# sloisel/MultiGridBarrierMPI.jl

Hardware: AMD Instinct MI355X
Metric: fem2d p-Laplace DoF/s per Newton step (higher is better)
Workload: dtype f64; 1 GPU; fem2d p-Laplace L=7 p=1 (n=57344 rows, N_L=49154 Newton unknowns), amgb main phase, tol=sqrt(eps); parallelism=single GPU

## Files before the change

### include/mgb_hip.h

```cpp
#ifndef MGB_HIP_H
#define MGB_HIP_H

#include <stdint.h>

#ifdef __cplusplus
extern "C" {
#endif

#define MGB_OK 0
#define MGB_E_ARG (-1)
#define MGB_E_HIP (-2)
#define MGB_E_NUMERIC (-3)
#define MGB_E_INTERNAL (-4)

typedef struct mgb_ctx_s* mgb_ctx;
typedef struct mgb_geo_s* mgb_geo;
typedef struct mgb_amg_s* mgb_amg;
typedef struct mgb_vec_s* mgb_vec;
typedef struct mgb_csr_s* mgb_csr;
typedef struct mgb_locator_s* mgb_locator;

const char* mgb_last_error(void);
int mgb_version(void);
int mgb_device_count(void);

int mgb_ctx_create(int device_id, mgb_ctx* out);
int mgb_ctx_destroy(mgb_ctx ctx);
int mgb_ctx_synchronize(mgb_ctx ctx);
typedef int (*mgb_allreduce_fn)(void* user, double* dev_ptr, long long count);
int mgb_ctx_set_comm(mgb_ctx ctx, int rank, int world, mgb_allreduce_fn fn, void* user);
int mgb_rccl_unique_id(char* out128);
int mgb_ctx_set_comm_rccl(mgb_ctx ctx, const char* unique_id128, int rank, int world);
int mgb_ctx_comm_stats(mgb_ctx ctx, long long* calls, double* bytes);
int mgb_shard_rows(int rank, int world, int n, int block, int* r0, int* r1);

int mgb_fem1d_native(int L, mgb_geo* out);
int mgb_fem2d_native(int L, const double* K, int nK_rows, mgb_geo* out);
int mgb_fem3d_native(int L, int k, mgb_geo* out);
int mgb_geo_create(int n, int dim, int L, int block, const double* x, const double* w, mgb_geo* out);
int mgb_geo_set_matrix(mgb_geo g, const char* name, int rows, int cols, const int32_t* rowptr,
                       const int32_t* colidx, const double* vals);
int mgb_geo_destroy(mgb_geo g);
int mgb_geo_dims(mgb_geo g, int* n, int* dim, int* L, int* block);
int mgb_geo_get_xw(mgb_geo g, double* x, double* w);
int mgb_geo_matrix_info(mgb_geo g, const char* name, int* rows, int* cols, int* nnz);
int mgb_geo_matrix_get(mgb_geo g, const char* name, int32_t* rowptr, int32_t* colidx, double* vals);

int mgb_vec_create(mgb_ctx ctx, int n, const double* host_or_null, mgb_vec* out);
int mgb_vec_free(mgb_vec v);
int mgb_vec_len(mgb_vec v, int* n);
int mgb_vec_upload(mgb_vec v, const double* host);
int mgb_vec_download(mgb_vec v, double* host);
int mgb_csr_create(mgb_ctx ctx, int rows, int cols, const int32_t* rowptr, const int32_t* colidx,
                   const double* vals, mgb_csr* out);
int mgb_csr_free(mgb_csr A);
int mgb_csr_dims(mgb_csr A, int* rows, int* cols, int* nnz);
int mgb_csr_get(mgb_csr A, int32_t* rowptr, int32_t* colidx, double* vals);
int mgb_csr_spgemm(mgb_csr A, mgb_csr B, mgb_csr* out);
int mgb_csr_transpose(mgb_csr A, mgb_csr* out);
int mgb_csr_add(mgb_csr A, double alpha, mgb_csr B, mgb_csr* out);
int mgb_csr_hcat(int count, const mgb_csr* mats, mgb_csr* out);
int mgb_csr_blockdiag(int count, const mgb_csr* mats, mgb_csr* out);
int mgb_diag(mgb_ctx ctx, mgb_vec z, int m, int n, mgb_csr* out);
int mgb_spmv(mgb_csr A, mgb_vec x, mgb_vec y);
int mgb_spmv_add(mgb_csr A, mgb_vec x, mgb_vec y0, mgb_vec y);
int mgb_dot(mgb_vec x, mgb_vec y, double* out);
int mgb_norm(mgb_vec x, double* out);
int mgb_sum(mgb_vec x, double* out);
int mgb_col_extract(mgb_vec M, int n, int K, int k, mgb_vec out);
int mgb_map_rows_barrier(int which, int K, int nterms, const int* kind, const int* nq, const int* idx_q, const int* idx_s,
                         const int* idx_s2, const double* p, const double* coef, const double* off, int n, mgb_vec Dz,
                         mgb_vec out);
int mgb_mul(mgb_vec x, mgb_vec y, mgb_vec out);
int mgb_axpy(mgb_vec x, double alpha, mgb_vec y, mgb_vec out);
int mgb_vec_allreduce_sum(mgb_vec x);
int mgb_all_isfinite(mgb_vec x, int* out);

int mgb_amg_create(mgb_ctx ctx, mgb_geo g, int S, const char* const* state_vars, int K, const char* const* D,
                   int nq, const int* idx_q, int idx_s, double p, mgb_amg* out);
int mgb_amg_create_cones(mgb_ctx ctx, mgb_geo g, int S, const char* const* state_vars, int K, const char* const* D,
                         int ncones, const int* nq, const int* idx_q, const int* idx_s, const int* idx_s2,
                         const double* p, mgb_amg* out);
int mgb_amg_create_terms(mgb_ctx ctx, mgb_geo g, int S, const char* const* state_vars, int K, const char* const* D,
                         int nterms, const int* kind, const int* nq, const int* idx_q, const int* idx_s, const int* idx_s2,
                         const double* p, const double* coef, const double* off, mgb_amg* out);
int mgb_amg_set_exponents(mgb_amg a, int term, const double* p_nodes);
int mgb_amg_set_term_mask(mgb_amg a, const unsigned char* mask);
int mgb_amg_destroy(mgb_amg a);
int mgb_amg_dims(mgb_amg a, int* n, int* S, int* K, int* L, int* nY);
int mgb_amg_local_rows(mgb_amg a, int* n_global, int* row0, int* n_local);
int mgb_amg_prepare(mgb_amg a, int level);
int mgb_amg_level_size(mgb_amg a, int level, int* N, int* nnz_lower);
int mgb_amg_f0_f32(mgb_amg a, int level, const float* s, float t, double* f0);
int mgb_amg_f1_f32(mgb_amg a, int level, const float* s, float t, float* g);
int mgb_amg_f2_f32(mgb_amg a, int level, const float* s, float t, float* lower_vals);
int mgb_amg_f1_template_f64(mgb_amg a, int level, const double* s, double t, double* g);
int mgb_amg_f2_template_f64(mgb_amg a, int level, const double* s, double t, double* lower_vals);
int mgb_amg_chol_info(mgb_amg a, int level, int* split_world, double* exchange_doubles, int* launches);
int mgb_amg_chol_schedule(mgb_amg a, int level, int cap, int* nlaunch, int* kind, int* workgroups, int* unknown_node,
                          int* unknown_col);
int mgb_amg_chol_tree(mgb_amg a, int level, int cap, int* nnodes, int* ns, int* nf, int* parent);
int mgb_amg_chol_values_local(mgb_amg a, int level, int* yes);
int mgb_amg_hessian_pattern(mgb_amg a, int level, int32_t* rowptr, int32_t* colidx);
int mgb_amg_set_c(mgb_amg a, const double* c);
int mgb_amg_set_z(mgb_amg a, const double* z);
int mgb_amg_get_z(mgb_amg a, double* z);
int mgb_amg_apply_D(mgb_amg a, int level, const double* s, double* Dz );
int mgb_amg_f0(mgb_amg a, int level, const double* s, double t, double* y, double* parts2);
int mgb_amg_f0_trial(mgb_amg a, int level, const double* s_ref, const double* s, double t, double* y);
int mgb_amg_f1(mgb_amg a, int level, const double* s, double t, double* g);
int mgb_amg_f2(mgb_amg a, int level, const double* s, double t, double* lower_vals);
int mgb_amg_solve_linear(mgb_amg a, int level, const double* lower_vals, const double* g, double* x);
int mgb_amg_solve_linear_gpu(mgb_amg a, int level, const double* lower_vals, const double* g, double* x);
int mgb_amg_set_solver(mgb_amg a, int solver);
int mgb_amg_set_schedule(mgb_amg a, int all_levels);
int mgb_amg_set_stop_rule(mgb_amg a, int upstream);
int mgb_amg_set_centering(mgb_amg a, int exact);
int mgb_amg_solve(mgb_amg a, double tol, double t0, double kappa, int maxit, int max_newton, int verbose);
int mgb_amg_set_early_stop(mgb_amg a, int col);
int mgb_amg_sol_info(mgb_amg a, int* nt, double* t_elapsed, double* time_factor, long long* counts4);
int mgb_amg_sol_get(mgb_amg a, long long* its , double* ts, double* c_dot_Dz);
int mgb_amg_sol_kernels(mgb_amg a, double* ms11, double* bytes11, long long* launches11);
int mgb_amg_time_kernels(mgb_amg a, int level, int reps, int nrot, double* ms8, double* bytes8);

int mgb_hessian_apply(mgb_amg a, int level, const double* s, const double* v, double* Hv, int matrix_free);
int mgb_smooth(mgb_amg a, int level, const double* s, const double* b, double* x, int degree, int sweeps, double lmax,
               int matrix_free, double* lmax_used);
int mgb_prolong(mgb_amg a, int level, const double* xc, double* xf);
int mgb_restrict(mgb_amg a, int level, const double* rf, double* rc);
int mgb_amg_prolongation(mgb_amg a, int level, int* rows, int* cols, int* nnz, int32_t* rowptr, int32_t* colidx, double* vals);
int mgb_amg_pcg_solve_linear(mgb_amg a, int level, const double* s, const double* g, double* x, int* iters, double* relres,
                             int* converged);
int mgb_amg_set_pcg(mgb_amg a, double rtol, int maxit, int degree, int power_its, double lo_frac, double hi_frac, int chunk,
                    int fallback, int assembled_top, int giveup);
int mgb_amg_sol_pcg(mgb_amg a, long long* counts4, double* time_s);
int mgb_amg_time_mg_kernels(mgb_amg a, int level, int reps, int nrot, double* ms6, double* bytes6, double* alg6);
int mgb_amg_mg_info(mgb_amg a, int top, int* coarsest);

int mgb_locator_create(mgb_ctx ctx, mgb_geo g, mgb_locator* out);
int mgb_locator_destroy(mgb_locator loc);
int mgb_interpolate(mgb_locator loc, int m, mgb_vec pts, int S, mgb_vec z, mgb_vec vals, mgb_vec grads_or_null,
                    int32_t* elem_host_or_null);
int mgb_geo_interpolate_host(mgb_geo g, int m, const double* pts, int S, const double* z, double* vals,
                             double* grads_or_null, int32_t* elem_or_null);


typedef struct mgb_plan_s* mgb_plan;
int mgb_plan_create(mgb_geo g, int S, const char* const* state_vars, int K, const char* const* D, int nq,
                    const int* idx_q, int idx_s, int level, mgb_plan* out);
int mgb_reduction_scratch_doubles(int n_local, int max_level_unknowns, long long* out);
int mgb_plan_destroy(mgb_plan p);
int mgb_plan_prolongation(mgb_plan fine, mgb_plan coarse, int* rows, int* cols, int* nnz, int32_t* rowptr, int32_t* colidx,
                          double* vals);
int mgb_plan_sizes(mgb_plan p, int* N, int* nnz_lower, int* nnz_T, int* nnz_B);
int mgb_plan_pattern(mgb_plan p, int32_t* rowptr, int32_t* colidx);
int mgb_plan_eval_host(mgb_plan p, const double* Y , double* lower_vals);
int mgb_plan_shard(mgb_plan p, int S, int K, int rank, int world, int block, mgb_plan* out, int* r0, int* r1);
int mgb_plan_apply_B_host(mgb_plan p, const double* s , double* Bs );
int mgb_plan_apply_BT_host(mgb_plan p, const double* v , double* g );
int mgb_plan_chol_bench(mgb_plan p, const double* Y, int dim, int reps, double* seconds_per_factor,
                        double* seconds_per_solve, double* flops, double* front_doubles, double* residual);
typedef struct mgb_hostchol_s* mgb_hostchol;
int mgb_plan_hostchol_create(mgb_plan p, int dim, mgb_hostchol* out);
int mgb_hostchol_destroy(mgb_hostchol c);
int mgb_hostchol_info(mgb_hostchol c, int* n, int* threads, double* flops);
int mgb_hostchol_factor_solve(mgb_hostchol c, const double* lower_vals, const double* g, double* x);
int mgb_hostchol_partition(mgb_hostchol c, int world, int* split_world, int cap, int* nnodes, int* owner);
int mgb_hostchol_factor_solve_dist(mgb_hostchol c, int rank, int world, mgb_allreduce_fn fn, void* user,
                                   const double* lower_vals, const double* g, double* x);
int mgb_plan_hostchol_create_ranked(mgb_plan p, int dim, int K, int world, int block, mgb_hostchol* out);
int mgb_hostchol_rank_aligned(mgb_hostchol c, int world, int* aligned, int* top_values);
int mgb_hostchol_factor_solve_dist_local(mgb_hostchol c, int rank, int world, mgb_allreduce_fn fn, void* user,
                                         const double* local_lower_vals, const double* g, double* x);
int mgb_plan_chol_tree(mgb_plan p, int dim, int cap, int* nnodes, int* ns, int* nf, int* parent);
int mgb_plan_chol_bwd_fused(mgb_plan p, int dim, int cut, int top_nf, int threads, int* info, int cap_wg, int* wg, int cap_bdry,
                            int* bdry, int* slots, int cap_nodes, int* bofs, int* first);
int mgb_chol_selftest(int nx, int ny, double* max_residual, double* flops, double* seconds);

#ifdef __cplusplus
}
#endif
#endif
```

### multigridbarriermpi.jl_amd/__init__.py

```python
from __future__ import annotations

import math
from dataclasses import dataclass, field
from typing import Callable, Dict, List, Optional, Sequence

import numpy as np
import scipy.sparse as sp

from . import _lib
from ._lib import MGBError, call, dptr, f64, i32, iptr

import ctypes as C

__all__ = [
    "fem1d", "fem2d", "fem3d", "fem1d_mpi", "fem2d_mpi", "fem3d_mpi", "fem1d_mpi_solve", "fem2d_mpi_solve",
    "fem3d_mpi_solve", "parabolic_solve", "ParabolicSOL", "native_to_mpi",
    "mpi_to_native", "amgb", "Geometry", "AMGBSOL", "HPCVector", "HPCMatrix", "HPCSparseMatrix",
    "backend_hip", "amgb_zeros", "amgb_all_isfinite", "amgb_diag", "amgb_blockdiag", "map_rows", "map_rows_gpu",
    "_raw_array", "_to_cpu_array", "MGBError", "device_count", "AMG", "amg", "hcat", "BarrierFn", "barrier_functions",
    "interpolate", "sample_grid",
]


def device_count() -> int:
# ... 533 lines not shown
    call("mgb_geo_create", n, dim, L, int(g_native.discretization.get("block", 1)), dptr(x), dptr(w), C.byref(h))

    def put(name, S):
        S = sp.csr_matrix(S, dtype=np.float64)
        S.sort_indices()
        S.sum_duplicates()
        rp, ci, va = i32(S.indptr), i32(S.indices), f64(S.data)
        call("mgb_geo_set_matrix", h, name.encode(), S.shape[0], S.shape[1], iptr(rp), iptr(ci), dptr(va))
        return HPCSparseMatrix(S, backend)

    try:
        operators = {k: put("op:" + k, g_native.operators[k]) for k in sorted(g_native.operators)}
        subspaces = {k: [put("sub:%s:%d" % (k, l), S) for l, S in enumerate(g_native.subspaces[k])]
                     for k in sorted(g_native.subspaces)}
        refine = [put("refine:%d" % l, S) for l, S in enumerate(g_native.refine)]
        coarsen = [put("coarsen:%d" % l, S) for l, S in enumerate(g_native.coarsen)]
    except Exception:
        call("mgb_geo_destroy", h)
        raise
    return Geometry(dict(g_native.discretization), HPCMatrix(x, backend), HPCVector(w, backend), subspaces,
                    operators, refine, coarsen, _geo=h)


def _mpi_from_native_handle(h, kind, ops, backend: Optional[HPCBackend], extra=None) -> Geometry:
    backend = backend or backend_hip()
    ref = _GeoRef(h)
    n, dim, L, block = C.c_int(), C.c_int(), C.c_int(), C.c_int()
    call("mgb_geo_dims", h, C.byref(n), C.byref(dim), C.byref(L), C.byref(block))
    x = np.empty((n.value, dim.value))
    w = np.empty(n.value)
    call("mgb_geo_get_xw", h, dptr(x), dptr(w))
    lazy = lambda name: _GeoMatrix(ref, name, backend)
    operators = {k: lazy("op:" + k) for k in sorted(ops)}
    subspaces = {k: [lazy("sub:%s:%d" % (k, l)) for l in range(L.value)] for k in ("dirichlet", "full")}
    refine = [lazy("refine:%d" % l) for l in range(L.value)]
    coarsen = [lazy("coarsen:%d" % l) for l in range(L.value)]
    disc = dict(kind=kind, L=L.value, dim=dim.value, block=block.value, **(extra or {}))
    return Geometry(disc, HPCMatrix(x, backend), HPCVector(w, backend), subspaces, operators, refine, coarsen, _geo=h,
                    _geo_ref=ref)


def _check_ti(Ti):
    if np.dtype(Ti) != np.dtype(np.int32):
        raise ValueError("only Ti=Int32 is supported by the HIP path")


def fem1d_mpi(L: int = 4, Ti=np.int32, backend=None) -> Geometry:
    _check_ti(Ti)
    h = C.c_void_p()
    call("mgb_fem1d_native", int(L), C.byref(h))
    return _mpi_from_native_handle(h, "fem1d", ("id", "dx"), backend)


def fem3d(L: int = 2, k: int = 3) -> Geometry:
    h = C.c_void_p()
    call("mgb_fem3d_native", int(L), int(k), C.byref(h))
    try:
        g = _native_from_handle(h, "fem3d", ("id", "dx", "dy", "dz"))
        g.discretization["k"] = int(k)
        return g
    finally:
        call("mgb_geo_destroy", h)


def fem3d_mpi(L: int = 2, k: int = 3, Ti=np.int32, backend=None) -> Geometry:
    _check_ti(Ti)
    h = C.c_void_p()
    call("mgb_fem3d_native", int(L), int(k), C.byref(h))
    return _mpi_from_native_handle(h, "fem3d", ("id", "dx", "dy", "dz"), backend, extra=dict(k=int(k)))


def fem2d_mpi(L: int = 2, K=None, Ti=np.int32, backend=None) -> Geometry:
    _check_ti(Ti)
    h = C.c_void_p()
    if K is None:
        call("mgb_fem2d_native", int(L), None, 0, C.byref(h))
    else:
        Kc = f64(K)
        call("mgb_fem2d_native", int(L), dptr(Kc), int(Kc.shape[0]), C.byref(h))
    return _mpi_from_native_handle(h, "fem2d", ("id", "dx", "dy"), backend)



DEFAULT_STATE = (("u", "dirichlet"), ("s", "full"))
DEFAULT_D = {1: (("u", "id"), ("u", "dx"), ("s", "id")),
             2: (("u", "id"), ("u", "dx"), ("u", "dy"), ("s", "id")),
             3: (("u", "id"), ("u", "dx"), ("u", "dy"), ("u", "dz"), ("s", "id"))}
class _RowFn:

    def __init__(self, row, grid):
        self._row, self.grid = row, grid

    def __call__(self, x):
        return self._row(x)


def _rows(fn, x) -> np.ndarray:
    if hasattr(fn, "grid"):
        return np.ascontiguousarray(fn.grid(x), dtype=np.float64)
    return np.vstack([np.asarray(fn(xi), dtype=np.float64) for xi in x])


def _const_rows(v):
    v = np.asarray(v, dtype=np.float64)
    return _RowFn(lambda x: v.copy(), lambda x: np.tile(v, (x.shape[0], 1)))


DEFAULT_F = {1: _const_rows([0.5, 0.0, 1.0]), 2: _const_rows([0.5, 0.0, 0.0, 1.0]), 3: _const_rows([0.5, 0.0, 0.0, 0.0, 1.0])}
DEFAULT_G = {1: _RowFn(lambda x: np.array([x[0], 2.0]), lambda x: np.column_stack([x[:, 0], np.full(x.shape[0], 2.0)])),
             2: _RowFn(lambda x: np.array([x[0] ** 2 + x[1] ** 2, 100.0]),
                       lambda x: np.column_stack([x[:, 0] ** 2 + x[:, 1] ** 2, np.full(x.shape[0], 100.0)])),
             3: _RowFn(lambda x: np.array([x[0] ** 2 + x[1] ** 2 + x[2] ** 2, 100.0]),
                       lambda x: np.column_stack([x[:, 0] ** 2 + x[:, 1] ** 2 + x[:, 2] ** 2, np.full(x.shape[0], 100.0)]))}


def _encode_terms(cones):
    kind, nq, iq, isl, is2, pp, coef, off = [], [], [], [], [], [], [], []
    for c in cones:
        if c[0] == "linear":
            _, cidx, ccoef, coff = c
            if not 1 <= len(cidx) <= 3 or len(ccoef) != len(cidx):
                raise ValueError("linear barrier term: 1..3 columns with one coefficient each")
            kind.append(1); nq.append(len(cidx)); iq += (list(cidx) + [0, 0, 0])[:3]; isl.append(0); is2.append(-1)
            pp.append(1.0); coef += (list(map(float, ccoef)) + [0.0, 0.0, 0.0])[:3]; off.append(float(coff))
        else:
            kind.append(0); nq.append(len(c[0]) - 1); iq += (list(c[0][:-1]) + [0, 0, 0])[:3]; isl.append(int(c[0][-1]))
            is2.append(int(c[2]) if len(c) > 2 else -1); pp.append(float(c[1])); coef += [0.0, 0.0, 0.0]; off.append(0.0)
    arr_i = lambda v: (C.c_int * len(v))(*v)
    arr_d = lambda v: (C.c_double * len(v))(*v)
    return (len(cones), arr_i(kind), arr_i(nq), arr_i(iq), arr_i(isl), arr_i(is2), arr_d(pp), arr_d(coef), arr_d(off))


class BarrierFn:

    def __init__(self, cones, K: int, which: int):
        self.cones, self.K, self.which = list(cones), int(K), int(which)

    def rows(self, Dz: "HPCMatrix"):
        n, K = Dz.shape
        if K != self.K:
            raise ValueError("BarrierFn: Dz has %d columns, the barrier was built for %d" % (K, self.K))
        width = (1, K, K * K)[self.which]
        out = HPCVector(n * width, Dz.backend)
        call("mgb_map_rows_barrier", self.which, K, *_encode_terms(self.cones), n, Dz._v.handle, out.handle)
        if self.which == 0:
            return out
        M_ = HPCMatrix.__new__(HPCMatrix)
        M_.shape, M_.backend, M_._v = (n, width), Dz.backend, out
        return M_

    def __call__(self, x_row, dz_row):
        r = self.rows(HPCMatrix(np.asarray(dz_row, dtype=np.float64).reshape(1, -1))).to_numpy()
        return float(r[0]) if self.which == 0 else r[0]


def barrier_functions(cones, K: int):
    return tuple(BarrierFn(cones, K, w) for w in (0, 1, 2))


class AMG:

    def __init__(self, geometry: Geometry, state_variables=DEFAULT_STATE, D=None, p: float = 1.0, idx=None,
                 cones=None, select=None):
        if geometry._geo is None:
            raise TypeError("AMG needs an MPI geometry (use native_to_mpi / fem*d_mpi)")
        dim = geometry.discretization["dim"]
        D = DEFAULT_D[dim] if D is None else D
        K = len(D)
        if cones is None:
            if idx is None:
                idx = list(range(K - dim - 1, K))
            cones = [(list(idx), float(p) if np.isscalar(p) else p)]
        self.geometry = geometry
        node_p, cones = {}, list(cones)
        for ti, c in enumerate(cones):
            if c[0] != "linear" and not np.isscalar(c[1]):
                pv = c[1]
                pn = (np.array([float(pv(xi)) for xi in geometry.x.to_numpy()]) if callable(pv) else f64(pv).reshape(-1))
                if pn.size != geometry.x.shape[0] or not np.all(pn >= 1.0):
                    raise ValueError("p(x) must give one value >= 1 per node")
                node_p[ti] = pn
                cones[ti] = (c[0], float(pn[0])) + tuple(c[2:])
        p = float(p) if np.isscalar(p) else (float(node_p[0][0]) if 0 in node_p else 1.0)
        self.p_nodes = node_p.get(0)
        self.state_variables, self.D, self.p, self.cones = tuple(state_variables), tuple(D), float(p), list(cones)
        power = [c for c in cones if c[0] != "linear"]
        self.idx = list(power[0][0]) if power else []
        backend = geometry.x.backend
        h = C.c_void_p()
        call("mgb_amg_create_terms", backend.handle, geometry._geo, len(state_variables), _lib.str_array(state_variables), K,
             _lib.str_array(D), *_encode_terms(cones), C.byref(h))
        self.handle = h
        n, S, K_, L, nY = (C.c_int() for _ in range(5))
        call("mgb_amg_dims", h, C.byref(n), C.byref(S), C.byref(K_), C.byref(L), C.byref(nY))
        self.S, self.K, self.L, self.nY = S.value, K_.value, L.value, nY.value
        ng, r0, nl = C.c_int(), C.c_int(), C.c_int()
        call("mgb_amg_local_rows", h, C.byref(ng), C.byref(r0), C.byref(nl))
        self.n, self.row0, self.n_local = ng.value, r0.value, nl.value
        for ti, pn in node_p.items():
            call("mgb_amg_set_exponents", h, int(ti), dptr(pn))
        if select is not None:
            mask = np.ascontiguousarray([[1 if b else 0 for b in select(xi)] for xi in geometry.x.to_numpy()], dtype=np.uint8)
            if mask.shape != (self.n, len(cones)):
                raise ValueError("select(x) must give one flag per barrier term")
            call("mgb_amg_set_term_mask", h, mask.ctypes.data_as(C.POINTER(C.c_ubyte)))

    def prepare(self, l=-1):
        call("mgb_amg_prepare", self.handle, int(l))

    def level_size(self, l):
        N, nz = C.c_int(), C.c_int()
        call("mgb_amg_level_size", self.handle, l, C.byref(N), C.byref(nz))
        return N.value, nz.value

    def chol_info(self, l=None):
        sw, ex, la = C.c_int(), C.c_double(), C.c_int()
        call("mgb_amg_chol_info", self.handle, self.L - 1 if l is None else int(l), C.byref(sw), C.byref(ex), C.byref(la))
        vl = C.c_int()
        call("mgb_amg_chol_values_local", self.handle, self.L - 1 if l is None else int(l), C.byref(vl))
        return dict(split_world=sw.value, exchange_doubles=ex.value, launches=la.value, values_local=bool(vl.value))

    CHOL_KINDS = ("Leaf", "Single", "SingleNarrow", "SingleDense", "SingleDenseNarrow", "Start", "Step", "Step2", "Panel2",
                  "Update2", "BwdRect", "Bwd256", "Bwd1024", "BwdFused")

    def chol_schedule(self, l=None):
        l = self.L - 1 if l is None else int(l)
        N = self.level_size(l)[0]
        nl = C.c_int()
        call("mgb_amg_chol_schedule", self.handle, l, 0, C.byref(nl), None, None, None, None)
        kind, wg = np.empty(nl.value, dtype=np.int32), np.empty(nl.value, dtype=np.int32)
        node, col = np.empty(N, dtype=np.int32), np.empty(N, dtype=np.int32)
        call("mgb_amg_chol_schedule", self.handle, l, nl.value, C.byref(nl), iptr(kind), iptr(wg), iptr(node), iptr(col))
        nn = C.c_int()
        call("mgb_amg_chol_tree", self.handle, l, 0, C.byref(nn), None, None, None)
        ns, nf, par = (np.empty(nn.value, dtype=np.int32) for _ in range(3))
        call("mgb_amg_chol_tree", self.handle, l, nn.value, C.byref(nn), iptr(ns), iptr(nf), iptr(par))
        height = np.zeros(nn.value, dtype=np.int32)
        for t in range(nn.value):
            if par[t] >= 0:
                height[par[t]] = max(height[par[t]], height[t] + 1)
        return dict(kinds=[self.CHOL_KINDS[k] for k in kind], workgroups=wg, unknown_node=node, unknown_col=col, ns=ns, nf=nf,
                    parent=par, height=height)

    def hessian_pattern(self, l):
        N, nz = self.level_size(l)
        rp = np.empty(N + 1, dtype=np.int32)
        ci = np.empty(nz, dtype=np.int32)
        call("mgb_amg_hessian_pattern", self.handle, l, iptr(rp), iptr(ci))
        return rp, ci

    def set_c(self, c):
        c = f64(c)
        assert c.shape == (self.n, self.K)
        call("mgb_amg_set_c", self.handle, dptr(c))

    def set_z(self, z):
        z = f64(np.asarray(z).reshape(-1))
        assert z.size == self.n * self.S
        call("mgb_amg_set_z", self.handle, dptr(z))

    def get_z(self):
        z = np.empty(self.n * self.S)
        call("mgb_amg_get_z", self.handle, dptr(z))
        return z

    def apply_D(self, l, s):
        s = f64(s)
        out = np.empty((self.n_local, self.K))
        call("mgb_amg_apply_D", self.handle, l, dptr(s), dptr(out))
        return out

    def apply_D_global(self, l, s):
        loc = self.apply_D(l, s)
        backend = self.geometry.x.backend
        if backend.world == 1:
            return loc
        full = np.zeros((self.n, self.K))
        full[self.row0:self.row0 + self.n_local] = loc
        v = HPCVector(full.reshape(-1), backend)
        call("mgb_vec_allreduce_sum", v.handle)
        return v.to_numpy().reshape(self.n, self.K)

    def f0(self, l, s, t, parts=False):
        s = f64(s)
        y = C.c_double()
        pr = np.empty(2)
        call("mgb_amg_f0", self.handle, l, dptr(s), float(t), C.byref(y), dptr(pr))
        return (y.value, pr) if parts else y.value

    def f0_trial(self, l, s_ref, s, t):
        s_ref, s = f64(s_ref), f64(s)
        y = C.c_double()
        call("mgb_amg_f0_trial", self.handle, l, dptr(s_ref), dptr(s), float(t), C.byref(y))
        return y.value

    def f1(self, l, s, t):
        s = f64(s)
        g = np.empty(self.level_size(l)[0])
        call("mgb_amg_f1", self.handle, l, dptr(s), float(t), dptr(g))
        return g

    def f2(self, l, s, t):
        s = f64(s)
        N, nz = self.level_size(l)
        vals = np.empty(nz)
        call("mgb_amg_f2", self.handle, l, dptr(s), float(t), dptr(vals))
# ... 531 lines not shown
```

### multigridbarriermpi.jl_amd/_lib.py

```python
from __future__ import annotations

import ctypes as C
import os

import numpy as np

_HERE = os.path.dirname(os.path.abspath(__file__))
LIB_PATH = os.path.join(_HERE, "lib", "libmgb_hip.so")

c_int_p = C.POINTER(C.c_int)
c_i32_p = C.POINTER(C.c_int32)
c_dbl_p = C.POINTER(C.c_double)
c_flt_p = C.POINTER(C.c_float)
c_ll_p = C.POINTER(C.c_longlong)
c_str_arr = C.POINTER(C.c_char_p)
H = C.c_void_p
ALLREDUCE_FN = C.CFUNCTYPE(C.c_int, C.c_void_p, C.c_void_p, C.c_longlong)


class MGBError(RuntimeError):
    def __init__(self, code, msg):
        super().__init__("mgb error %d: %s" % (code, msg))
        self.code = code


PROTOTYPES = {
    "mgb_ctx_create": [C.c_int, C.POINTER(H)],
    "mgb_ctx_destroy": [H],
    "mgb_ctx_synchronize": [H],
    "mgb_ctx_set_comm": [H, C.c_int, C.c_int, ALLREDUCE_FN, C.c_void_p],
    "mgb_rccl_unique_id": [C.c_char_p],
    "mgb_ctx_set_comm_rccl": [H, C.c_char_p, C.c_int, C.c_int],
    "mgb_ctx_comm_stats": [H, c_ll_p, c_dbl_p],
    "mgb_shard_rows": [C.c_int, C.c_int, C.c_int, C.c_int, c_int_p, c_int_p],
    "mgb_fem1d_native": [C.c_int, C.POINTER(H)],
    "mgb_fem2d_native": [C.c_int, c_dbl_p, C.c_int, C.POINTER(H)],
    "mgb_fem3d_native": [C.c_int, C.c_int, C.POINTER(H)],
    "mgb_geo_create": [C.c_int, C.c_int, C.c_int, C.c_int, c_dbl_p, c_dbl_p, C.POINTER(H)],
    "mgb_geo_set_matrix": [H, C.c_char_p, C.c_int, C.c_int, c_i32_p, c_i32_p, c_dbl_p],
    "mgb_geo_destroy": [H],
    "mgb_geo_dims": [H, c_int_p, c_int_p, c_int_p, c_int_p],
    "mgb_geo_get_xw": [H, c_dbl_p, c_dbl_p],
    "mgb_geo_matrix_info": [H, C.c_char_p, c_int_p, c_int_p, c_int_p],
    "mgb_geo_matrix_get": [H, C.c_char_p, c_i32_p, c_i32_p, c_dbl_p],
    "mgb_vec_create": [H, C.c_int, c_dbl_p, C.POINTER(H)],
    "mgb_vec_free": [H],
    "mgb_vec_len": [H, c_int_p],
    "mgb_vec_upload": [H, c_dbl_p],
    "mgb_vec_download": [H, c_dbl_p],
    "mgb_csr_create": [H, C.c_int, C.c_int, c_i32_p, c_i32_p, c_dbl_p, C.POINTER(H)],
    "mgb_csr_free": [H],
    "mgb_csr_dims": [H, c_int_p, c_int_p, c_int_p],
    "mgb_csr_get": [H, c_i32_p, c_i32_p, c_dbl_p],
    "mgb_csr_spgemm": [H, H, C.POINTER(H)],
    "mgb_csr_transpose": [H, C.POINTER(H)],
    "mgb_csr_add": [H, C.c_double, H, C.POINTER(H)],
    "mgb_csr_hcat": [C.c_int, C.POINTER(H), C.POINTER(H)],
    "mgb_csr_blockdiag": [C.c_int, C.POINTER(H), C.POINTER(H)],
    "mgb_diag": [H, H, C.c_int, C.c_int, C.POINTER(H)],
    "mgb_spmv": [H, H, H],
    "mgb_spmv_add": [H, H, H, H],
    "mgb_dot": [H, H, c_dbl_p],
    "mgb_norm": [H, c_dbl_p],
    "mgb_sum": [H, c_dbl_p],
    "mgb_col_extract": [H, C.c_int, C.c_int, C.c_int, H],
    "mgb_map_rows_barrier": [C.c_int, C.c_int, C.c_int, c_int_p, c_int_p, c_int_p, c_int_p, c_int_p, c_dbl_p, c_dbl_p, c_dbl_p,
                             C.c_int, H, H],
    "mgb_mul": [H, H, H],
    "mgb_axpy": [H, C.c_double, H, H],
    "mgb_vec_allreduce_sum": [H],
    "mgb_all_isfinite": [H, c_int_p],
    "mgb_amg_create": [H, H, C.c_int, c_str_arr, C.c_int, c_str_arr, C.c_int, c_int_p, C.c_int, C.c_double,
                       C.POINTER(H)],
    "mgb_amg_create_cones": [H, H, C.c_int, c_str_arr, C.c_int, c_str_arr, C.c_int, c_int_p, c_int_p, c_int_p, c_int_p,
                             c_dbl_p, C.POINTER(H)],
    "mgb_amg_create_terms": [H, H, C.c_int, c_str_arr, C.c_int, c_str_arr, C.c_int, c_int_p, c_int_p, c_int_p, c_int_p, c_int_p,
                             c_dbl_p, c_dbl_p, c_dbl_p, C.POINTER(H)],
    "mgb_amg_set_exponents": [H, C.c_int, c_dbl_p],
    "mgb_amg_set_term_mask": [H, C.POINTER(C.c_ubyte)],
    "mgb_amg_destroy": [H],
    "mgb_amg_dims": [H, c_int_p, c_int_p, c_int_p, c_int_p, c_int_p],
    "mgb_amg_local_rows": [H, c_int_p, c_int_p, c_int_p],
    "mgb_amg_prepare": [H, C.c_int],
    "mgb_amg_chol_info": [H, C.c_int, c_int_p, c_dbl_p, c_int_p],
    "mgb_amg_chol_schedule": [H, C.c_int, C.c_int, c_int_p, c_int_p, c_int_p, c_int_p, c_int_p],
    "mgb_amg_chol_tree": [H, C.c_int, C.c_int, c_int_p, c_int_p, c_int_p, c_int_p],
    "mgb_amg_chol_values_local": [H, C.c_int, c_int_p],
    "mgb_amg_level_size": [H, C.c_int, c_int_p, c_int_p],
    "mgb_amg_hessian_pattern": [H, C.c_int, c_i32_p, c_i32_p],
    "mgb_amg_set_c": [H, c_dbl_p],
    "mgb_amg_set_z": [H, c_dbl_p],
    "mgb_amg_get_z": [H, c_dbl_p],
    "mgb_amg_apply_D": [H, C.c_int, c_dbl_p, c_dbl_p],
    "mgb_amg_f0": [H, C.c_int, c_dbl_p, C.c_double, c_dbl_p, c_dbl_p],
    "mgb_amg_f0_trial": [H, C.c_int, c_dbl_p, c_dbl_p, C.c_double, c_dbl_p],
    "mgb_amg_f1": [H, C.c_int, c_dbl_p, C.c_double, c_dbl_p],
    "mgb_amg_f2": [H, C.c_int, c_dbl_p, C.c_double, c_dbl_p],
    "mgb_amg_set_early_stop": [H, C.c_int],
    "mgb_amg_f0_f32": [H, C.c_int, c_flt_p, C.c_float, c_dbl_p],
    "mgb_amg_f1_f32": [H, C.c_int, c_flt_p, C.c_float, c_flt_p],
    "mgb_amg_f2_f32": [H, C.c_int, c_flt_p, C.c_float, c_flt_p],
    "mgb_amg_f1_template_f64": [H, C.c_int, c_dbl_p, C.c_double, c_dbl_p],
    "mgb_amg_f2_template_f64": [H, C.c_int, c_dbl_p, C.c_double, c_dbl_p],
    "mgb_amg_solve_linear": [H, C.c_int, c_dbl_p, c_dbl_p, c_dbl_p],
    "mgb_amg_solve_linear_gpu": [H, C.c_int, c_dbl_p, c_dbl_p, c_dbl_p],
    "mgb_amg_set_solver": [H, C.c_int],
    "mgb_amg_set_schedule": [H, C.c_int],
    "mgb_amg_set_stop_rule": [H, C.c_int],
    "mgb_amg_set_centering": [H, C.c_int],
    "mgb_amg_set_pcg": [H, C.c_double, C.c_int, C.c_int, C.c_int, C.c_double, C.c_double, C.c_int, C.c_int, C.c_int, C.c_int],
    "mgb_amg_sol_pcg": [H, c_ll_p, c_dbl_p],
    "mgb_hessian_apply": [H, C.c_int, c_dbl_p, c_dbl_p, c_dbl_p, C.c_int],
    "mgb_smooth": [H, C.c_int, c_dbl_p, c_dbl_p, c_dbl_p, C.c_int, C.c_int, C.c_double, C.c_int, c_dbl_p],
    "mgb_prolong": [H, C.c_int, c_dbl_p, c_dbl_p],
    "mgb_restrict": [H, C.c_int, c_dbl_p, c_dbl_p],
    "mgb_amg_prolongation": [H, C.c_int, c_int_p, c_int_p, c_int_p, c_i32_p, c_i32_p, c_dbl_p],
    "mgb_amg_pcg_solve_linear": [H, C.c_int, c_dbl_p, c_dbl_p, c_dbl_p, c_int_p, c_dbl_p, c_int_p],
    "mgb_amg_mg_info": [H, C.c_int, c_int_p],
    "mgb_amg_time_mg_kernels": [H, C.c_int, C.c_int, C.c_int, c_dbl_p, c_dbl_p, c_dbl_p],
    "mgb_locator_create": [H, H, C.POINTER(H)],
    "mgb_locator_destroy": [H],
    "mgb_interpolate": [H, C.c_int, H, C.c_int, H, H, H, c_i32_p],
    "mgb_geo_interpolate_host": [H, C.c_int, c_dbl_p, C.c_int, c_dbl_p, c_dbl_p, c_dbl_p, c_i32_p],
    "mgb_plan_prolongation": [H, H, c_int_p, c_int_p, c_int_p, c_i32_p, c_i32_p, c_dbl_p],
    "mgb_amg_solve": [H, C.c_double, C.c_double, C.c_double, C.c_int, C.c_int, C.c_int],
    "mgb_amg_sol_info": [H, c_int_p, c_dbl_p, c_dbl_p, c_ll_p],
    "mgb_amg_sol_get": [H, c_ll_p, c_dbl_p, c_dbl_p],
    "mgb_amg_sol_kernels": [H, c_dbl_p, c_dbl_p, c_ll_p],
    "mgb_amg_time_kernels": [H, C.c_int, C.c_int, C.c_int, c_dbl_p, c_dbl_p],
    "mgb_plan_create": [H, C.c_int, c_str_arr, C.c_int, c_str_arr, C.c_int, c_int_p, C.c_int, C.c_int,
                        C.POINTER(H)],
    "mgb_reduction_scratch_doubles": [C.c_int, C.c_int, c_ll_p],
    "mgb_plan_destroy": [H],
    "mgb_plan_sizes": [H, c_int_p, c_int_p, c_int_p, c_int_p],
    "mgb_plan_pattern": [H, c_i32_p, c_i32_p],
    "mgb_plan_eval_host": [H, c_dbl_p, c_dbl_p],
    "mgb_plan_shard": [H, C.c_int, C.c_int, C.c_int, C.c_int, C.c_int, C.POINTER(C.c_void_p), c_int_p, c_int_p],
    "mgb_plan_apply_B_host": [H, c_dbl_p, c_dbl_p],
    "mgb_plan_apply_BT_host": [H, c_dbl_p, c_dbl_p],
    "mgb_plan_chol_bench": [H, c_dbl_p, C.c_int, C.c_int, c_dbl_p, c_dbl_p, c_dbl_p, c_dbl_p, c_dbl_p],
    "mgb_plan_hostchol_create": [H, C.c_int, C.POINTER(H)],
    "mgb_hostchol_destroy": [H],
    "mgb_hostchol_info": [H, c_int_p, c_int_p, c_dbl_p],
    "mgb_hostchol_factor_solve": [H, c_dbl_p, c_dbl_p, c_dbl_p],
    "mgb_hostchol_partition": [H, C.c_int, c_int_p, C.c_int, c_int_p, c_int_p],
    "mgb_hostchol_factor_solve_dist": [H, C.c_int, C.c_int, ALLREDUCE_FN, C.c_void_p, c_dbl_p, c_dbl_p, c_dbl_p],
    "mgb_plan_hostchol_create_ranked": [H, C.c_int, C.c_int, C.c_int, C.c_int, C.POINTER(H)],
    "mgb_hostchol_rank_aligned": [H, C.c_int, c_int_p, c_int_p],
    "mgb_hostchol_factor_solve_dist_local": [H, C.c_int, C.c_int, ALLREDUCE_FN, C.c_void_p, c_dbl_p, c_dbl_p, c_dbl_p],
    "mgb_plan_chol_tree": [H, C.c_int, C.c_int, c_int_p, c_int_p, c_int_p, c_int_p],
    "mgb_plan_chol_bwd_fused": [H, C.c_int, C.c_int, C.c_int, C.c_int, c_int_p, C.c_int, c_int_p, C.c_int, c_int_p, c_int_p, C.c_int,
                                c_int_p, c_int_p],
    "mgb_chol_selftest": [C.c_int, C.c_int, c_dbl_p, c_dbl_p, c_dbl_p],
}
_SPECIAL = {"mgb_last_error": ([], C.c_char_p), "mgb_version": ([], C.c_int), "mgb_device_count": ([], C.c_int)}

_lib = None


def load():
    global _lib
    if _lib is not None:
        return _lib
    if not os.path.exists(LIB_PATH):
        raise ImportError("libmgb_hip.so not built: run `python -c 'import __graft_entry__ as g; g.build()'` "
                          "or multigridbarriermpi.jl_amd/csrc/build.sh (expected at %s)" % LIB_PATH)
    lib = C.CDLL(LIB_PATH)
    for name, args in PROTOTYPES.items():
        fn = getattr(lib, name)
        fn.argtypes = args
        fn.restype = C.c_int
    for name, (args, res) in _SPECIAL.items():
        fn = getattr(lib, name)
        fn.argtypes = args
        fn.restype = res
    _lib = lib
    return lib


def call(name, *args):
    lib = load()
    rc = getattr(lib, name)(*args)
    if rc != 0:
        raise MGBError(rc, lib.mgb_last_error().decode("utf-8", "replace"))
    return rc


def dptr(a):
    return None if a is None else a.ctypes.data_as(c_dbl_p)


def iptr(a):
    return None if a is None else a.ctypes.data_as(c_i32_p)


def f64(a):
    return np.ascontiguousarray(a, dtype=np.float64)


def i32(a):
    return np.ascontiguousarray(a, dtype=np.int32)


def str_array(pairs):
    flat = []
    for a, b in pairs:
        flat += [str(a).encode(), str(b).encode()]
    return (C.c_char_p * len(flat))(*flat)
```

### multigridbarriermpi.jl_amd/csrc/amg.cpp

```cpp
#include "amg.hpp"


#include <chrono>
#include <cmath>
#include <thread>
#include <string>
#include <cstdlib>
#include <cstdio>

namespace mgb {

void hip_check(hipError_t e, const char* what) {
  if (e != hipSuccess) throw HipError(std::string("HIP error in ") + what + ": " + hipGetErrorString(e));
}

static inline void cpu_relax() {
#if defined(__x86_64__) || defined(__i386__)
  __builtin_ia32_pause();
#elif defined(__aarch64__)
  asm volatile("yield" ::: "memory");
#else
  std::this_thread::yield();
#endif
}
// ... 309 lines not shown
  const int K = P.K, nY = P.nY();
  auto gather = [&](int q, const ConeSpec& S, RowU& u) { gather_row(pl.B, K, q, S, u); };
  auto structural = [&](const RowU& u, int nc, int a, int b, int i, int j) { return structural_pair(u, nc, a, b, i, j); };
  const int nthr = std::max(1, std::min(MfChol::threads(), n / 2048));
  auto chunks = [&](auto&& fn) { node_chunks(n, nthr, fn); };
  auto phase = [](const char*) {};
  auto entry = [&](int r, int c) {
    const int* b0 = pl.Apat.colidx.data() + pl.Apat.rowptr[r];
    const int* e0 = pl.Apat.colidx.data() + pl.Apat.rowptr[r + 1];
    return (int)(std::lower_bound(b0, e0, c) - pl.Apat.colidx.data());
  };
  const int nnzA = pl.Apat.nnz();
  pl.T = Csr(nnzA, n * nY);
  struct Term {
    int e, col;
    double coef;
  };
  std::vector<std::vector<Term>> tterms(nthr);
  std::vector<std::vector<int>> tcnt(nthr);
  chunks([&](int q0, int q1, int tI) {
    std::vector<Term>& terms = tterms[tI];
    std::vector<int>& cnt = tcnt[tI];
    cnt.assign(nnzA, 0);
    terms.reserve((size_t)(q1 - q0) * 80);
    RowU u;
    for (int q = q0; q < q1; ++q) {
      int base = 0;
      for (int ci = 0; ci < P.ncones; ++ci) {
        const ConeSpec& S = P.cone[ci];
        const int nact = S.nact();
        gather(q, S, u);
        const int nc = (int)u.cols.size();
        for (int i = 0; i < nc; ++i)
          for (int j = 0; j <= i; ++j) {
            int e = -1;
            int slot = base;
            for (int a = 0; a < nact; ++a)
              for (int b = a; b < nact; ++b, ++slot) {
                if (!structural(u, nc, a, b, i, j)) continue;
                if (e < 0) e = entry(u.cols[i], u.cols[j]);
                double coef = u.val[(size_t)a * nc + i] * u.val[(size_t)b * nc + j];
                if (a != b) coef += u.val[(size_t)b * nc + i] * u.val[(size_t)a * nc + j];
                terms.push_back({e, q * nY + slot, coef});
                cnt[e]++;
              }
          }
        base += S.nY();
      }
    }
  });
  phase("list terms");
  {
    long long tot = 0;
    for (int e = 0; e < nnzA; ++e) {
      pl.T.rowptr[e] = (int)tot;
      for (int t = 0; t < nthr; ++t) {
        const int c0 = tcnt[t][e];
        tcnt[t][e] = (int)tot;
        tot += c0;
      }
      if (tot > 2000000000LL) throw ArgError("amg: Hessian plan exceeds Int32 indexing");
    }
    pl.T.rowptr[nnzA] = (int)tot;
    pl.T.colidx.resize((size_t)tot);
    pl.T.vals.resize((size_t)tot);
  }
  chunks([&](int, int, int tI) {
    std::vector<int>& pos = tcnt[tI];
    for (const Term& tm : tterms[tI]) {
      const int pp = pos[tm.e]++;
      pl.T.colidx[pp] = tm.col;
      pl.T.vals[pp] = tm.coef;
    }
    std::vector<Term>().swap(tterms[tI]);
  });
  phase("fill terms");
}


Amg::Amg(Ctx& ctx, const GeometryHost& g, const AmgSpec& spec, const BarrierParams& P)
    : ctx_(ctx), n_(g.n), S_((int)spec.state_variables.size()), P_(P), spec_(spec) {
  hip_check(hipSetDevice(ctx_.device), "hipSetDevice");
  if (const char* e = std::getenv("MGB_FUSED_TRIAL_ROWS")) fused_trial_rows_ = std::atoi(e);
  if (P.K != (int)spec.D.size()) throw ArgError("amg: barrier K != number of D rows");
  if (P.ncones < 1 || P.ncones > kMaxCones) throw ArgError("amg: barrier supports 1 to 3 terms");
  if (P.K > 8) throw ArgError("amg: the barrier kernels support at most 8 rows of D");
  for (int ci = 0; ci < P.ncones; ++ci) {
    const ConeSpec& S = P.cone[ci];
    if (S.kind != 0 && S.kind != 1) throw ArgError("amg: unknown barrier term kind");
    if (S.nq < 1 || S.nq > 3) throw ArgError("amg: barrier supports 1..3 gradient components");
    for (int a = 0; a < S.nact(); ++a)
      if (S.col(a) < 0 || S.col(a) >= P.K) throw ArgError("amg: barrier index out of range");
  }
  if ((int)g.w.size() != n_ || (int)g.x.size() != n_ * g.dim) throw ArgError("amg: geometry x/w size mismatch");
  ng_ = g.n;
  Csr Dstack = build_dstack(g, spec);
  w_min_ = *std::min_element(g.w.begin(), g.w.end());
  if (ctx_.world > 1) {
    int r1 = 0;
    shard_rows(ctx_.rank, ctx_.world, ng_, g.block, &r0_, &r1);
    n_ = r1 - r0_;
    Dstack_.upload(shard_dstack(Dstack, ng_, S_, P.K, r0_, r1));
  } else {
    Dstack_.upload(Dstack);
  }
  w_.upload(g.w.data() + r0_, n_);
  const int K = P.K, nY = P.nY();
  c_.alloc((size_t)n_ * K);
  z_.alloc((size_t)n_ * S_);
  z_save_.alloc((size_t)n_ * S_);
  Dz0_.alloc((size_t)n_ * K);
  Dz0_save_.alloc((size_t)n_ * K);
  Dz_.alloc((size_t)n_ * K);
  DzA_.alloc((size_t)n_ * K);
  DzB_.alloc((size_t)n_ * K);
  DzC_.alloc((size_t)n_ * K);
  v_.alloc((size_t)n_ * K);
  Y_.alloc((size_t)n_ * nY);
  phi_cur_.alloc((size_t)n_ * P.ncones);
  phi_trial_.alloc((size_t)n_ * P.ncones);
  phi_trial2_.alloc((size_t)n_ * P.ncones);
  phi_trial3_.alloc((size_t)n_ * P.ncones);
  h_flag_.alloc(4);
  scal_.alloc(12);
  h_scal_.alloc(12);
  seq_dev_.alloc(1);
  hip_check(hipMemset(seq_dev_.p, 0, sizeof(unsigned long long)), "memset seq");
  h_seq_.alloc(1);
  h_seq_.p[0] = 0;
  hip_check(hipMemsetAsync(c_.p, 0, c_.n * sizeof(double), ctx_.stream), "memset");
  hip_check(hipMemsetAsync(z_.p, 0, z_.n * sizeof(double), ctx_.stream), "memset");
  hip_check(hipStreamSynchronize(ctx_.stream), "sync");
  geo_ = g;
  dstack_host_ = std::move(Dstack);
  for (int l = 0; l < g.L; ++l) {
    levels_.emplace_back(new Level);
    int N = 0;
    for (auto& sv : spec.state_variables) {
      if (sv.second == "fixed") continue;
      auto it = g.subspaces.find(sv.second);
      if (it == g.subspaces.end() || l >= (int)it->second.size())
        throw ArgError("amg: unknown subspace '" + sv.second + "'");
      N += it->second[l].cols;
    }
    levels_[l]->plan.N = N;
  }
  int maxN = 0;
  for (auto& lv : levels_) maxN = std::max(maxN, lv->plan.N);
  partials_.alloc(reduction_scratch_doubles(n_, maxN));
  hip_check(hipMemset(partials_.p, 0, partials_.n * sizeof(double)), "memset scratch");
}

size_t reduction_scratch_doubles(int n_local, int max_level_unknowns) {
  return (size_t)6 * std::max(f0_blocks(n_local), f0_blocks(max_level_unknowns)) + 8 + kReductionHeader;
}

int Amg::level_index(const Level& lv) const {
  for (size_t l = 0; l < levels_.size(); ++l)
    if (levels_[l].get() == &lv) return (int)l;
  throw InternalError("amg: level not found");
}

Amg::Level& Amg::level(int l) {
  Level& lv = *levels_.at(l);
  if (lv.built) return lv;
  if (lv.chol_analysis.joinable()) lv.chol_analysis.join();
  lv.chol_analyzed = false;
  lv.chol_analysis_error = nullptr;
  hip_check(hipSetDevice(ctx_.device), "hipSetDevice");
  static const bool use_elasm = !(std::getenv("MGB_ASSEMBLE") && std::string(std::getenv("MGB_ASSEMBLE")) == "plan");
  const bool try_elasm = use_elasm && ctx_.world == 1 && geo_.block > 1 && n_ % geo_.block == 0;
  lv.plan = build_level_plan(geo_, spec_, dstack_host_, l, P_, !try_elasm);
  lv.T_built = !try_elasm;
  if (ctx_.world > 1) {
    std::vector<unsigned long long> mask = dof_rank_masks(lv.plan.B, ng_, P_.K, ctx_.world, geo_.block);
    lv.plan = shard_level_plan(lv.plan, ng_, S_, P_.K, P_.nY(), r0_, r0_ + n_);
    lv.plan.rank_mask = std::move(mask);
  }
  if (!pcg_ && lv.plan.N > 0) {
    lv.chol_analysis = std::thread([this, &lv] {
      try {
        analyze_chol(lv);
      } catch (...) {
        lv.chol_analysis_error = std::current_exception();
      }
    });
  }
  const double t_up = now_s();
  lv.R.upload(lv.plan.R);
  lv.B.upload(lv.plan.B);
  if (n_ > fused_trial_rows_ && geo_.block > 1 && n_ % geo_.block == 0) lv.Bel.build(lv.plan.B, geo_.block * P_.K);
  lv.BT.upload(lv.plan.BT);
  if (lv.T_built) lv.T.upload(lv.plan.T);
  if (try_elasm && lv.plan.N > 0) {
    mg_of(lv);
    if (mg_ensure_elop(lv)) lv.elasm.build(lv.mg->elop, lv.plan.Apat, P_);
    if (!lv.elasm.view.valid()) ensure_T(lv);
  }
  const int N = lv.plan.N, nnzA = lv.plan.Apat.nnz();
  lv.s.alloc(N);
  lv.s_trial.alloc(N);
  lv.s_trial2.alloc(N);
  lv.s_trial3.alloc(N);
  lv.g_trial.alloc(N);
  lv.g.alloc(N);
  lv.nstep.alloc(N);
  lv.avals.alloc(nnzA);
  lv.h_avals.alloc(nnzA);
  lv.h_g.alloc(N);
  lv.h_n.alloc(N);
  lv.h_s.alloc(N);
  if (std::getenv("MGB_VERBOSE_SETUP")) std::fprintf(stderr, "[mgb setup] level upload + buffers       %.3f s\n", now_s() - t_up);
  lv.built = true;
  return lv;
}

void Amg::analyze_chol(Level& lv) {
  static const bool aligned_on = !(std::getenv("MGB_RANK_ALIGNED") && std::atoi(std::getenv("MGB_RANK_ALIGNED")) == 0);
  const bool ranked = aligned_on && ctx_.world > 1 && (int)lv.plan.rank_mask.size() == lv.plan.N;
  lv.chol.analyze(lv.plan.Apat, lv.plan.coords.data(), geo_.dim, 64, ranked ? lv.plan.rank_mask.data() : nullptr, ctx_.world);
  lv.chol_analyzed = true;
}

void Amg::ensure_chol(Level& lv) {
  if (lv.chol_built) return;
  hip_check(hipSetDevice(ctx_.device), "hipSetDevice");
  static const bool vt = std::getenv("MGB_VERBOSE_SETUP") != nullptr;
  double t0 = now_s();
  if (lv.chol_analysis.joinable()) lv.chol_analysis.join();
  if (lv.chol_analysis_error) {
    std::exception_ptr e = lv.chol_analysis_error;
    lv.chol_analysis_error = nullptr;
    std::rethrow_exception(e);
  }
  if (!lv.chol_analyzed) analyze_chol(lv);
  if (vt) std::fprintf(stderr, "[mgb setup] chol analyze (rest)         %.3f s\n", now_s() - t0);
  t0 = now_s();
  lv.gchol.build(lv.chol, &ctx_);
  if (vt) std::fprintf(stderr, "[mgb setup] gpuchol build + upload      %.3f s\n", now_s() - t0);
  lv.chol_built = true;
}

static double csr_bytes(const DevCsr& A, bool y0);

void Amg::ensure_T(Level& lv) {
  if (!lv.T_built) {
    build_plan_terms(lv.plan, ng_, P_);
    lv.T_built = true;
  }
  if (lv.T.view.rows == 0 && lv.plan.T.rows > 0) {
    hip_check(hipSetDevice(ctx_.device), "hipSetDevice");
    lv.T.upload(lv.plan.T);
  }
}

double Amg::assemble_bytes(Level& lv) {
  if (!lv.elasm.view.valid()) return csr_bytes(lv.T.view, false);
  const DevElOp& E = lv.mg->elop.view;
  return (double)lv.B.view.nnz * 8 + (double)n_ * P_.nY() * 8 + E.nel * 4.0 + 2.0 * E.nel * lv.elasm.view.npm * 8 +
         (double)E.nel * lv.elasm.view.npm * 4 + lv.plan.Apat.nnz() * 12.0;
}

void Amg::assemble_values(Level& lv) {
  if (lv.elasm.view.valid()) {
    launch_elop_assemble(ctx_.stream, lv.mg->elop.view, lv.elasm.view, P_, Y_.p, lv.elasm.elmat.p, lv.avals.p);
    return;
  }
  ensure_T(lv);
  launch_spmv(ctx_.stream, lv.T.view, Y_.p, nullptr, lv.avals.p);
}

const LevelPlan& Amg::plan(int l) { return level(l).plan; }

void Amg::chol_info(int l, int* split_world, double* exchange_doubles, int* launches) {
  Level& lv = level(l);
  ensure_chol(lv);
  if (split_world) *split_world = lv.gchol.split() ? ctx_.world : 1;
  if (exchange_doubles) *exchange_doubles = lv.gchol.split() ? lv.gchol.exchange_doubles() : 0.0;
  if (launches) *launches = lv.gchol.launches_per_solve();
}

void Amg::chol_schedule(int l, int cap, int* nlaunch, int* kind, int* workgroups, int* unknown_node, int* unknown_col) {
  Level& lv = level(l);
  ensure_chol(lv);
  lv.gchol.schedule_info(cap, nlaunch, kind, workgroups);
  GpuChol::unknown_columns(lv.chol, unknown_node, unknown_col);
}

void Amg::chol_tree(int l, int cap, int* nnodes, int* ns, int* nf, int* parent) {
  Level& lv = level(l);
  ensure_chol(lv);
  std::vector<int> a, b, c;
  lv.chol.tree(a, b, c);
  if (nnodes) *nnodes = (int)a.size();
  const size_t m = std::min<size_t>(std::max(cap, 0), a.size());
  if (ns) std::copy(a.begin(), a.begin() + m, ns);
  if (nf) std::copy(b.begin(), b.begin() + m, nf);
  if (parent) std::copy(c.begin(), c.begin() + m, parent);
}

void Amg::prepare(int l) {
  const int L = (int)levels_.size();
  for (int J = (l >= 0 ? l : (schedule_all_ ? 0 : L - 1)); J <= (l >= 0 ? l : L - 1); ++J) {
    Level& lv = level(J);
    if (lv.plan.N == 0) continue;
    if (pcg_) mg_prepare(J);
    else ensure_chol(lv);
// ... 55 lines not shown
  hip_check(hipStreamSynchronize(ctx_.stream), "sync");
  if (ctx_.world <= 1) {
    z_.download(z_host, (size_t)n_ * S_);
    return;
  }
  DevBuf<double> zg;
  zg.alloc((size_t)ng_ * S_);
  hip_check(hipMemsetAsync(zg.p, 0, zg.n * sizeof(double), ctx_.stream), "memset zg");
  for (int sv = 0; sv < S_; ++sv)
    hip_check(hipMemcpyAsync(zg.p + (size_t)sv * ng_ + r0_, z_.p + (size_t)sv * n_, (size_t)n_ * sizeof(double),
                             hipMemcpyDeviceToDevice, ctx_.stream), "D2D z");
  ctx_.allreduce_sum(zg.p, (long long)zg.n);
  hip_check(hipStreamSynchronize(ctx_.stream), "sync");
  zg.download(z_host, zg.n);
}

static double csr_bytes(const DevCsr& A, bool y0) {
  return (double)A.nnz * 12.0 + (A.rows + 1) * 4.0 + A.cols * 8.0 + A.rows * 8.0 * (y0 ? 2 : 1);
}

KernelTimer::~KernelTimer() {
  for (auto* v : {&free_, &pending_})
    for (auto& p : *v) {
      (void)hipEventDestroy(p.a);
      (void)hipEventDestroy(p.b);
    }
}

void KernelTimer::begin(hipStream_t st, int cls, double bytes) {
  if (!on_ || !sampling_) return;
  if (free_.empty()) {
    Pair p{};
    hip_check(hipEventCreate(&p.a), "hipEventCreate");
    hip_check(hipEventCreate(&p.b), "hipEventCreate");
    free_.push_back(p);
  }
  cur_ = free_.back();
  free_.pop_back();
  cur_.cls = cls;
  cur_.bytes = bytes;
  hip_check(hipEventRecord(cur_.a, st), "hipEventRecord");
  open_ = true;
}

void KernelTimer::end(hipStream_t st) {
  if (!on_ || !open_) return;
  hip_check(hipEventRecord(cur_.b, st), "hipEventRecord");
  pending_.push_back(cur_);
  open_ = false;
}

void KernelTimer::collect(SolveStats& st) {
  for (auto& p : pending_) {
    float ms = 0;
    if (hipEventElapsedTime(&ms, p.a, p.b) == hipSuccess) {
      st.kern_ms[p.cls] += ms;
      st.kern_bytes[p.cls] += p.bytes;
      st.kern_launches[p.cls]++;
    }
    free_.push_back(p);
  }
  pending_.clear();
}

void Amg::sync_collect(const char* what) {
  hip_check(hipStreamSynchronize(ctx_.stream), what);
  if (live_) timer_.collect(*live_);
}

void Amg::resync_signals() {
  hip_check(hipStreamSynchronize(ctx_.stream), "resync signals");
  seq_expected_ = *h_seq_.p;
}

HostSignal Amg::next_signal() {
  HostSignal sig;
  if (ctx_.world != 1) return sig;
  sig.seq_dev = seq_dev_.p;
  sig.seq_host = h_seq_.p;
  ++seq_expected_;
  return sig;
}

void Amg::wait_signal(const char* what) {
  if (ctx_.world != 1 || host_solve_ || (live_ && timer_.sampling())) {
    sync_collect(what);
    return;
  }
  const volatile unsigned long long* q = h_seq_.p;
  const double t0 = now_s();
  for (unsigned long spins = 0; __atomic_load_n(q, __ATOMIC_ACQUIRE) < seq_expected_; ++spins) {
    cpu_relax();
    if ((spins & 0xfffff) == 0xfffff && now_s() - t0 > 10.0) {
      hip_check(hipStreamSynchronize(ctx_.stream), what);
      if (__atomic_load_n(q, __ATOMIC_ACQUIRE) < seq_expected_) throw InternalError(std::string("mgb: completion signal lost in ") + what);
    }
  }
}

void Amg::refresh_dz0() { launch_spmv(ctx_.stream, Dstack_.view, z_.p, nullptr, Dz0_.p); }

void Amg::dev_apply(Level& lv, const double* s_dev, double* dz) {
  timer_.begin(ctx_.stream, KC_APPLY, csr_bytes(lv.B.view, true));
  if (lv.Bel.view.valid()) launch_spmv_el(ctx_.stream, lv.B.view, lv.Bel.view, s_dev, Dz0_.p, dz);
  else launch_spmv(ctx_.stream, lv.B.view, s_dev, Dz0_.p, dz);
  timer_.end(ctx_.stream);
}

double Amg::trial_bytes(const Level& lv, bool with_ref) const {
  return csr_bytes(lv.B.view, true) + (double)n_ * (P_.K + 1 + P_.ncones * (with_ref ? 2 : 1)) * 8;
}

void Amg::enqueue_f0(Level& lv, const double* s_dev, double alpha, const double* nstep, double* s_out, double* dz,
                     const double* phi_ref, double* phi_out, double* out2, HostSignal sig) {
  if (n_ <= fused_trial_rows_) {
    timer_.begin(ctx_.stream, KC_F0, trial_bytes(lv, phi_ref != nullptr));
    launch_trial_f0(ctx_.stream, lv.B.view, n_, P_, s_dev, alpha, nstep, s_out, Dz0_.p, dz, w_.p, c_.p, phi_ref,
                    kFracToBoundary, phi_out, partials_.p, out2, host_scal(out2), sig);
    timer_.end(ctx_.stream);
    return;
  }
  const double* x = s_dev;
  if (nstep) {
    launch_waxpby(ctx_.stream, lv.plan.N, s_dev, alpha, nstep, s_out);
    x = s_out;
  }
  dev_apply(lv, x, dz);
  timer_.begin(ctx_.stream, KC_F0, (double)n_ * (2 * P_.K + 2 + (phi_ref ? 1 : 0)) * 8);
  launch_barrier_f0(ctx_.stream, n_, P_, dz, w_.p, c_.p, phi_ref, kFracToBoundary, phi_out, partials_.p, out2, host_scal(out2), sig);
  timer_.end(ctx_.stream);
}

double Amg::dev_f0(Level& lv, const double* s_dev, double t, double* parts, const double* phi_ref, double* phi_out,
                   double* dz, double alpha, const double* nstep, double* s_out) {
  enqueue_f0(lv, s_dev, alpha, nstep, s_out, dz, phi_ref, phi_out, scal_.p, next_signal());
  if (ctx_.world > 1) {
    ctx_.allreduce_sum(scal_.p, 2);
    hip_check(hipMemcpyAsync(h_scal_.p, scal_.p, 2 * sizeof(double), hipMemcpyDeviceToHost, ctx_.stream), "D2H scal");
  }
  wait_signal("sync f0");
  if (parts) {
    parts[0] = h_scal_.p[0];
    parts[1] = h_scal_.p[1];
  }
  return h_scal_.p[0] + t * h_scal_.p[1];
}

bool Amg::values_stay_local(Level& lv) {
  if (ctx_.world <= 1 || host_solve_) return false;
  ensure_chol(lv);
  return lv.gchol.values_local();
}

void Amg::enqueue_f2_assemble(Level& lv, const double* dz, SolveStats& st) {
  timer_.begin(ctx_.stream, KC_F2, (double)n_ * (P_.K + 1 + P_.nY()) * 8);
  launch_barrier_f2(ctx_.stream, n_, P_, dz, w_.p, Y_.p);
  timer_.end(ctx_.stream);
  if (pcg_) {
    mg_values(level_index(lv));
    st.n_f2++;
    return;
  }
  timer_.begin(ctx_.stream, KC_ASSEMBLE, assemble_bytes(lv));
  assemble_values(lv);
  timer_.end(ctx_.stream);
  if (!values_stay_local(lv)) ctx_.allreduce_sum(lv.avals.p, lv.plan.Apat.nnz());
  st.n_f2++;
}

double Amg::dev_f1(Level& lv, const double* dz, double t, double* g_out, SolveStats* st, const double** pre) {
  timer_.begin(ctx_.stream, KC_F1, (double)n_ * (3 * P_.K + 1) * 8);
  launch_barrier_f1(ctx_.stream, n_, P_, dz, w_.p, c_.p, t, v_.p);
  timer_.end(ctx_.stream);
  timer_.begin(ctx_.stream, KC_RESTRICT, csr_bytes(lv.BT.view, false));
  launch_spmv(ctx_.stream, lv.BT.view, v_.p, nullptr, g_out);
  timer_.end(ctx_.stream);
  if (owner_local(lv)) {
    const int ntop = lv.gchol.ntop_unknowns();
    if (gtop_.n < (size_t)ntop + 1) gtop_.alloc((size_t)ntop + 1);
    launch_gather_top(ctx_.stream, ntop, lv.gchol.top_unknowns(), g_out, gtop_.p);
    launch_dot_owned(ctx_.stream, lv.plan.N, g_out, g_out, lv.gchol.unknown_kind(), 0, partials_.p, gtop_.p + ntop);
    ctx_.allreduce_sum(gtop_.p, ntop + 1);
    launch_scatter_top_norm(ctx_.stream, ntop, lv.gchol.top_unknowns(), gtop_.p, g_out, scal_.p + 2);
  } else {
    ctx_.allreduce_sum(g_out, lv.plan.N);
    launch_dot(ctx_.stream, lv.plan.N, g_out, g_out, partials_.p, scal_.p + 2, host_scal(scal_.p + 2), nullptr, nullptr, next_signal());
  }
  if (ctx_.world > 1)
    hip_check(hipMemcpyAsync(h_scal_.p + 2, scal_.p + 2, sizeof(double), hipMemcpyDeviceToHost, ctx_.stream), "D2H gg");
  if (host_solve_)
    hip_check(hipMemcpyAsync(lv.h_g.p, g_out, (size_t)lv.plan.N * sizeof(double), hipMemcpyDeviceToHost, ctx_.stream),
              "D2H g");
  if (pre && st && !host_solve_) {
    if (!pcg_) ensure_chol(lv);
    if (ctx_.world > 1) {
      if (!ev_f1_) hip_check(hipEventCreateWithFlags(&ev_f1_, hipEventDisableTiming), "event");
      hip_check(hipEventRecord(ev_f1_, ctx_.stream), "record f1");
    }
    enqueue_f2_assemble(lv, dz, *st);
    *pre = dz;
    if (ctx_.world == 1) wait_signal("sync f1");
    else hip_check(hipEventSynchronize(ev_f1_), "sync f1 event");
  } else {
    wait_signal("sync f1");
  }
  return std::sqrt(h_scal_.p[2]);
}

static const double kBeta = 0.5, kArmijo = 0.1, kMinStep = 1e-8;

void Amg::enqueue_trial(Level& lv, Trial& T, double step, int slot, HostSignal sig) {
  double* out = scal_.p + 4 + 2 * slot;
  enqueue_f0(lv, lv.s.p, -step, lv.nstep.p, T.s, T.dz, phi_cur_.p, T.phi, out, sig);
  T.step = step;
}

static const double kSpecSteps[3] = {1.0, kBeta, kBeta * kBeta};

void Amg::enqueue_spec_trials(Level& lv, Trial* spec, HostSignal sig) {
  const int ns = spec_count();
  if (ns == 3) {
    TrialSet T;
    T.na = 3;
    for (int q = 0; q < 3; ++q) {
      T.alpha[q] = -kSpecSteps[q];
      T.s_out[q] = spec[q].s;
      T.dz[q] = spec[q].dz;
      T.phi_out[q] = spec[q].phi;
      spec[q].step = kSpecSteps[q];
    }
    T.out_dev = scal_.p + 4;
    T.out_host = host_scal(scal_.p + 4);
    timer_.begin(ctx_.stream, KC_F0, trial_bytes(lv, true) + 2.0 * n_ * (P_.K + P_.ncones) * 8);
    launch_trial_set(ctx_.stream, lv.B.view, n_, P_, lv.s.p, lv.nstep.p, T, Dz0_.p, w_.p, c_.p, phi_cur_.p, kFracToBoundary,
                     partials_.p, sig);
    timer_.end(ctx_.stream);
  } else {
    enqueue_trial(lv, spec[0], kSpecSteps[0], 0);
    enqueue_trial(lv, spec[1], kSpecSteps[1], 1, sig);
  }
}

void Amg::launch_step_graph(Level& lv, Trial* spec) {
  const void* key[15] = {lv.avals.p, lv.g.p, lv.nstep.p, lv.s.p, spec[0].s, spec[0].phi, spec[0].dz, spec[1].s, spec[1].phi,
                         spec[1].dz, spec[2].s,  spec[2].phi, spec[2].dz, phi_cur_.p, Dz0_.p};
  for (const auto& g : lv.step_graphs)
    if (std::equal(key, key + 15, g.key)) {
      hip_check(hipGraphLaunch(g.exec, ctx_.stream), "hipGraphLaunch");
      ++seq_expected_;
      for (int q = 0; q < spec_count(); ++q) spec[q].step = kSpecSteps[q];
      return;
    }
  hipGraph_t graph = nullptr;
  hip_check(hipStreamBeginCapture(ctx_.stream, hipStreamCaptureModeThreadLocal), "hipStreamBeginCapture");
  try {
    lv.gchol.enqueue_chain(ctx_.stream, lv.avals.p, lv.g.p, lv.nstep.p);
    launch_dot(ctx_.stream, lv.plan.N, lv.g.p, lv.nstep.p, partials_.p, scal_.p + 3, host_scal(scal_.p + 3), lv.gchol.fail_flag(),
               h_flag_.p);
    HostSignal sig;
    sig.seq_dev = seq_dev_.p;
    sig.seq_host = h_seq_.p;
    enqueue_spec_trials(lv, spec, sig);
  } catch (...) {
    (void)hipStreamEndCapture(ctx_.stream, &graph);
    if (graph) (void)hipGraphDestroy(graph);
    throw;
  }
  hip_check(hipStreamEndCapture(ctx_.stream, &graph), "hipStreamEndCapture");
  Level::StepGraph sg{};
  std::copy(key, key + 15, sg.key);
  hipError_t e = hipGraphInstantiate(&sg.exec, graph, nullptr, nullptr, 0);
  (void)hipGraphDestroy(graph);
  hip_check(e, "hipGraphInstantiate");
  lv.step_graphs.push_back(sg);
  hip_check(hipGraphLaunch(sg.exec, ctx_.stream), "hipGraphLaunch");
  ++seq_expected_;
}

bool Amg::dev_f2_solve(Level& lv, const double* dz, double t, SolveStats& st, double* inc, Trial* spec,
                       const double* pre_assembled) {
  const int N = lv.plan.N, nnzA = lv.plan.Apat.nnz();
  if (!pcg_) ensure_chol(lv);
  if (pre_assembled != dz) enqueue_f2_assemble(lv, dz, st);
  st.n_factor++;
  timer_.sample((st.n_factor % 8) == 1);
  if (pcg_) {
    const int top = level_index(lv);
    bool ok = pcg_run(lv, top, lv.g.p, lv.nstep.p, &st, nullptr, nullptr);
    if (!ok && pcg_last_code_ == 2.0) {
      for (int l = mg_coarsest(top); l <= top; ++l)
        if (level(l).mg) level(l).mg->ev_warm = false;
      mg_values(top);
      ok = pcg_run(lv, top, lv.g.p, lv.nstep.p, &st, nullptr, nullptr);
    }
    h_flag_.p[0] = 0;
    if (ok) pcg_bad_streak_ = 0;
    if (!ok) {
      if (!pcg_opt.fallback) return false;
      st.pcg_fallbacks++;
      if (pcg_opt.giveup > 0 && ++pcg_bad_streak_ >= pcg_opt.giveup) {
        pcg_ = false;
        st.pcg_gaveup_at = st.n_factor;
      }
      ensure_chol(lv);
      assemble_values(lv);
      lv.gchol.factor_solve(ctx_.stream, lv.avals.p, lv.g.p, lv.nstep.p, nullptr, false);
      lv.flag_armed = false;
      hip_check(hipMemcpyAsync(h_flag_.p, lv.gchol.fail_flag(), sizeof(int), hipMemcpyDeviceToHost, ctx_.stream), "D2H flag");
    }
    launch_dot(ctx_.stream, N, lv.g.p, lv.nstep.p, partials_.p, scal_.p + 3, host_scal(scal_.p + 3), nullptr, nullptr,
               spec ? HostSignal() : next_signal());
    if (spec) {
      enqueue_spec_trials(lv, spec, next_signal());
      st.n_f0 += spec_count();
    }
    wait_signal("sync pcg solve");
    if (!ok) hip_check(hipStreamSynchronize(ctx_.stream), "sync fallback flag");
    if (spec)
      for (int q = 0; q < spec_count(); ++q) {
        spec[q].y = h_scal_.p[4 + 2 * q] + t * h_scal_.p[5 + 2 * q];
        spec[q].valid = true;
      }
    *inc = h_scal_.p[3];
    return h_flag_.p[0] == 0;
  }
  if (!host_solve_) {
    const bool use_graph = GpuChol::knobs().graph;
    KernelTimer* tm = (live_ && timer_.sampling()) ? &timer_ : nullptr;
    const bool flag_rides = ctx_.world == 1;
    hipEvent_t e0 = nullptr, e1 = nullptr;
    const bool time_chain = live_ && timer_.enabled() && (st.n_factor % 8) == 5;
    if (flag_rides && spec && !tm && !time_chain && use_graph && lv.flag_armed) {
      launch_step_graph(lv, spec);
      st.n_f0 += spec_count();
    } else {
      if (time_chain) {
        hip_check(hipEventCreate(&e0), "event");
        hip_check(hipEventCreate(&e1), "event");
        hip_check(hipEventRecord(e0, ctx_.stream), "record");
      }
      const bool olocal = owner_local(lv);
      lv.gchol.factor_solve(ctx_.stream, lv.avals.p, lv.g.p, lv.nstep.p, tm, flag_rides && lv.flag_armed, false, olocal);
      if (time_chain) hip_check(hipEventRecord(e1, ctx_.stream), "record");
      if (olocal) {
        launch_dot_owned(ctx_.stream, N, lv.g.p, lv.nstep.p, lv.gchol.unknown_kind(), ctx_.rank == 0, partials_.p, scal_.p + 3);
        launch_flag_to_double(ctx_.stream, lv.gchol.fail_flag(), scal_.p + 10);
      } else if (flag_rides) {
        launch_dot(ctx_.stream, N, lv.g.p, lv.nstep.p, partials_.p, scal_.p + 3, host_scal(scal_.p + 3), lv.gchol.fail_flag(),
                   h_flag_.p, spec ? HostSignal() : next_signal());
        lv.flag_armed = true;
      } else {
        launch_dot(ctx_.stream, N, lv.g.p, lv.nstep.p, partials_.p, scal_.p + 3);
        hip_check(hipMemcpyAsync(h_flag_.p, lv.gchol.fail_flag(), sizeof(int), hipMemcpyDeviceToHost, ctx_.stream), "D2H flag");
      }
      if (spec) {
        enqueue_spec_trials(lv, spec, next_signal());
        if (!olocal) ctx_.allreduce_sum(scal_.p + 4, 2 * spec_count());
        st.n_f0 += spec_count();
      }
      if (olocal) {
        if (!spec) hip_check(hipMemsetAsync(scal_.p + 4, 0, 6 * sizeof(double), ctx_.stream), "zero trial slots");
        ctx_.allreduce_sum(scal_.p + 3, 8);
        hip_check(hipMemcpyAsync(h_scal_.p + 3, scal_.p + 3, 8 * sizeof(double), hipMemcpyDeviceToHost, ctx_.stream), "D2H inc + trials + flag");
      } else if (ctx_.world > 1)
        hip_check(hipMemcpyAsync(h_scal_.p + 3, scal_.p + 3, (spec ? 1 + 2 * spec_count() : 1) * sizeof(double),
                                 hipMemcpyDeviceToHost, ctx_.stream), "D2H inc + trials");
    }
    wait_signal("sync solve");
    if (owner_local(lv)) h_flag_.p[0] = h_scal_.p[10] != 0.0 ? 1 : 0;
    if (spec)
      for (int q = 0; q < spec_count(); ++q) {
        spec[q].y = h_scal_.p[4 + 2 * q] + t * h_scal_.p[5 + 2 * q];
        spec[q].valid = true;
      }
    if (e0) {
      float ms = 0;
      hip_check(hipEventSynchronize(e1), "sync chain event");
      if (hipEventElapsedTime(&ms, e0, e1) == hipSuccess) st.time_factor += 8.0 * ms * 1e-3;
      (void)hipEventDestroy(e0);
      (void)hipEventDestroy(e1);
    }
    *inc = h_scal_.p[3];
    if (h_flag_.p[0] != 0 && h_flag_.p[0] != 1)
      throw InternalError("gpuchol: pivot flag holds " + std::to_string(h_flag_.p[0]) + " (only 0 / 1 are ever written)");
    return h_flag_.p[0] == 0;
  }
  hip_check(hipMemcpyAsync(lv.h_avals.p, lv.avals.p, (size_t)nnzA * sizeof(double), hipMemcpyDeviceToHost, ctx_.stream),
            "D2H avals");
  sync_collect("sync f2");
  const double t0 = now_s();
  bool ok = lv.chol.factor(lv.h_avals.p);
  double acc = 0;
  if (ok) {
    std::copy(lv.h_g.p, lv.h_g.p + N, lv.h_n.p);
    lv.chol.solve(lv.h_n.p);
    for (int i = 0; i < N; ++i) acc += lv.h_g.p[i] * lv.h_n.p[i];
    hip_check(hipMemcpyAsync(lv.nstep.p, lv.h_n.p, (size_t)N * sizeof(double), hipMemcpyHostToDevice, ctx_.stream),
              "H2D n");
  }
  st.time_factor += now_s() - t0;
  *inc = acc;
  return ok;
}


Amg::NewtonResult Amg::newton(int l, double t, bool finest, bool final, double lam_tol, int maxit, SolveStats& st, int verbose) {
  Level& lv = level(l);
  const int N = lv.plan.N;
  NewtonResult res;
  if (N == 0) {
    res.converged = true;
    return res;
  }
  hip_check(hipMemsetAsync(lv.s.p, 0, (size_t)N * sizeof(double), ctx_.stream), "memset s");
  double y = dev_f0(lv, lv.s.p, t, nullptr, nullptr, phi_cur_.p, Dz_.p);
  st.n_f0++;
  if (!std::isfinite(y)) {
    std::vector<double> hdz((size_t)n_ * P_.K);
    Dz_.download(hdz.data(), hdz.size());
    int bad = 0, worst = -1;
    double minphi = INFINITY;
    for (int q = 0; q < n_; ++q) {
      const double* d = hdz.data() + (size_t)q * P_.K;
      double phi = INFINITY, sv = INFINITY;
      for (int ci = 0; ci < P_.ncones; ++ci) {
        const ConeSpec& S = P_.cone[ci];
        if (S.kind == 1) {
          double ph = S.off;
          for (int i = 0; i < S.nq; ++i) ph += S.coef[i] * d[S.iq[i]];
          phi = std::min(phi, ph);
          continue;
        }
        double qq = 0;
        for (int i = 0; i < S.nq; ++i) qq += d[S.iq[i]] * d[S.iq[i]];
        const double sc = d[S.is] + (S.is2 >= 0 ? d[S.is2] : 0.0);
        phi = std::min(phi, (sc > 0 ? std::pow(sc, S.a) : -1.0) - qq);
        sv = std::min(sv, sc);
      }
      if (!(phi > 0) || !(sv > 0)) bad++;
      if (!(phi >= minphi)) {
        minphi = phi;
        worst = q;
      }
    }
    char buf[256];
    snprintf(buf, sizeof buf, "newton: infeasible start (level %d, t=%g, %d of %d rows outside the cone, min phi=%g at row %d, y=%g)",
             l, t, bad, n_, minphi, worst, y);
    throw NumericError(buf);
  }
  double gnorm = dev_f1(lv, Dz_.p, t, lv.g.p);
  st.n_f1++;
  double ymin = y, gmin = gnorm, incmin = INFINITY;
  const double theta = finest ? 0.1 : 0.5;
  Trial T[3];
  T[0].s = lv.s_trial.p;
  T[0].phi = phi_trial_.p;
  T[1].s = lv.s_trial2.p;
  T[1].phi = phi_trial2_.p;
  T[2].s = lv.s_trial3.p;
  T[2].phi = phi_trial3_.p;
  T[0].dz = DzA_.p;
  T[1].dz = DzB_.p;
  T[2].dz = DzC_.p;
  auto eval = [&](int pos, double step) {
    if (!(T[pos].valid && T[pos].step == step))
      for (int q = 0; q < 3; ++q)
        if (q != pos && T[q].valid && T[q].step == step) {
          std::swap(T[pos], T[q]);
          break;
        }
    Trial& X = T[pos];
    if (X.valid && X.step == step) return X.y;
    X.y = dev_f0(lv, lv.s.p, t, nullptr, phi_cur_.p, X.phi, X.dz, -step, lv.nstep.p, X.s);
    st.n_f0++;
    X.step = step;
    X.valid = true;
    return X.y;
  };
  const double* pre = nullptr;
  const bool speculate = !host_solve_;
  while (res.k < maxit && !res.converged) {
    res.k++;
    double inc = 0;
    T[0].valid = T[1].valid = T[2].valid = false;
    const double* have = pre;
    pre = nullptr;
    if (!dev_f2_solve(lv, Dz_.p, t, st, &inc, speculate ? T : nullptr, have)) {
      if (verbose > 1) fprintf(stderr, "    [mgb] level %d k=%d: Hessian not numerically SPD (pivot flag %d)\n", l, res.k, h_flag_.p[0]);
      break;
    }
    if (!std::isfinite(inc)) {
      if (verbose > 1) fprintf(stderr, "    [mgb] level %d k=%d: non-finite Newton decrement\n", l, res.k);
      break;
    }
    if (inc <= 0) {
      res.converged = true;
      break;
    }
    double step = 1.0, ynext = y, gnext = gnorm;
    bool accepted = false;
    while (step >= kMinStep) {
      double yA = eval(0, step);
      if (std::isfinite(yA) && yA <= y - kArmijo * step * inc) {
        while (step * kBeta >= kMinStep) {
          const double yB = eval(1, step * kBeta);
          if (!(std::isfinite(yB) && yB < yA)) break;
          std::swap(T[0], T[1]);
          yA = yB;
          step *= kBeta;
// ... 445 lines not shown
```

### multigridbarriermpi.jl_amd/csrc/amg.hpp

```cpp
#pragma once
#include <memory>
#include <string>
#include <utility>
#include <thread>
#include <exception>
#include <vector>

#include "geometry.hpp"
#include "gpuchol.hpp"
#include "kernels.hpp"
#include "mfchol.hpp"
#include "mg.hpp"

namespace mgb {

void hip_check(hipError_t e, const char* what);

typedef int (*AllreduceFn)(void* user, double* dev_ptr, long long count);

struct Ctx {
  int device = 0;
  hipStream_t stream = nullptr;
  int rank = 0, world = 1;
  AllreduceFn allreduce = nullptr;
// ... 149 lines not shown
  bool schedule_all = false;
  bool time_kernels = true;
  bool upstream_stop = false;
  bool exact_centering = true;
  double tol = 1.4901161193847656e-08;
  double t0 = 0.1;
  double kappa = 10.0;
  int maxit = 10000;
  int max_newton = 48;
  int verbose = 0;
};

struct SolveStats {
  int L = 0;
  std::vector<long long> its;
  std::vector<double> ts, c_dot_Dz;
  double t_elapsed = 0, t_setup = 0;
  double time_factor = 0, time_device = 0;
  long long n_factor = 0, n_f0 = 0, n_f1 = 0, n_f2 = 0;
  long long pcg_solves = 0, pcg_iters = 0, pcg_fallbacks = 0;
  long long pcg_gaveup_at = -1;
  double time_pcg = 0;
  double kern_ms[KC_COUNT] = {};
  double kern_bytes[KC_COUNT] = {};
  long long kern_launches[KC_COUNT] = {};
};

class KernelTimer {
 public:
  ~KernelTimer();
  void enable(bool on) { on_ = on; sampling_ = true; }
  void sample(bool now) { sampling_ = now; }
  bool sampling() const { return on_ && sampling_; }
  bool enabled() const { return on_; }
  void begin(hipStream_t st, int cls, double bytes);
  void end(hipStream_t st);
  void collect(SolveStats& st);
 private:
  struct Pair {
    hipEvent_t a, b;
    int cls;
    double bytes;
  };
  std::vector<Pair> free_, pending_;
  Pair cur_{};
  bool on_ = false, open_ = false, sampling_ = true;
};

class Amg {
 public:
  Amg(Ctx& ctx, const GeometryHost& g, const AmgSpec& spec, const BarrierParams& P);
  int n() const { return n_; }
  int n_global() const { return ng_; }
  int row0() const { return r0_; }
  int S() const { return S_; }
  int K() const { return P_.K; }
  int L() const { return (int)levels_.size(); }
  int level_size(int l) const { return levels_[l]->plan.N; }
  const LevelPlan& plan(int l);
  void prepare(int l);
  const BarrierParams& params() const { return P_; }
  void chol_info(int l, int* split_world, double* exchange_doubles, int* launches);
  void chol_schedule(int l, int cap, int* nlaunch, int* kind, int* workgroups, int* unknown_node, int* unknown_col);
  void chol_tree(int l, int cap, int* nnodes, int* ns, int* nf, int* parent);
  bool chol_values_local(int l) { return values_stay_local(level(l)); }
  void set_early_stop(int col) { early_stop_col_ = col; }
  void set_exponents(int term, const double* p_nodes_global);
  void set_term_mask(const unsigned char* mask_global);
  void set_pcg(bool on) { pcg_ = on; }

  void set_c(const double* c_host);
  void set_z(const double* z_host);
  void get_z(double* z_host);

  double f0(int l, const double* s_host, double t, double* parts);
  double f0_trial(int l, const double* s_ref_host, const double* s_host, double t);
  void f1(int l, const double* s_host, double t, double* g_host);
  void f2(int l, const double* s_host, double t, double* avals_host);
  double f0_f32(int l, const float* s_host, float t);
  void f1_f32(int l, const float* s_host, float t, float* g_host);
  void f2_f32(int l, const float* s_host, float t, float* avals_host);
  void f1_tpl64(int l, const double* s_host, double t, double* g_host);
  void f2_tpl64(int l, const double* s_host, double t, double* avals_host);
  void apply_D(int l, const double* s_host, double* Dz_host);
  bool solve_host(int l, const double* avals, const double* g, double* nstep);
  bool solve_device(int l, const double* avals, const double* g, double* nstep);

  void solve(const SolveOptions& opt, SolveStats& st);

  struct KernelTimes {
    double apply_ms, f2_ms, assemble_ms, f1_ms, restrict_ms, f0_ms, trial_ms, apply_csr_ms, apply_el;
    double apply_bytes, f2_bytes, assemble_bytes, f1_bytes, restrict_bytes, f0_bytes, trial_bytes;
  };
  KernelTimes time_kernels(int l, int reps, int nrot = 1);

 private:
  struct Level {
    bool built = false, chol_built = false, T_built = false;
    DevElAsmOwned elasm;
    bool flag_armed = false;
    struct StepGraph {
      const void* key[15];
      hipGraphExec_t exec;
    };
    std::vector<StepGraph> step_graphs;
    std::thread chol_analysis;
    std::exception_ptr chol_analysis_error;
    bool chol_analyzed = false;
    ~Level() {
      if (chol_analysis.joinable()) chol_analysis.join();
      for (auto& g : step_graphs) (void)hipGraphExecDestroy(g.exec);
    }
    LevelPlan plan;
    DevCsrOwned R, B, BT, T;
    DevElCsrOwned Bel;
    DevBuf<float> B32, BT32, T32, s32, g32, avals32;
    bool f32_built = false;
    MfChol chol;
    GpuChol gchol;
    DevBuf<double> s, s_trial, s_trial2, s_trial3, g, g_trial, nstep, avals;
    PinnedBuf<double> h_avals, h_g, h_n, h_s;
    struct Mg {
      bool elop_tried = false, assembled = false, transfer = false, vectors = false;
      DevElOpOwned elop;
      DevBuf<double> elbuf;
      DevCsrOwned A;
      DevBuf<int> amap, diagpos, lo_rowptr, lo_colidx;
      DevCsrOwned P, PT;
      DevBuf<double> dinv, x, b, r, d0, d1, ev0, ev1, coef, Ainv;
      bool ev_warm = false;
    };
    std::unique_ptr<Mg> mg;
  };
  struct NewtonResult {
    int k = 0;
    bool converged = false;
  };
  Level& level(int l);
  int level_index(const Level& lv) const;
  void ensure_chol(Level& lv);
  void analyze_chol(Level& lv);
  void ensure_T(Level& lv);
  void assemble_values(Level& lv);
  double assemble_bytes(Level& lv);
  void refresh_dz0();
  void dev_apply(Level& lv, const double* s_dev, double* dz);
  double dev_f0(Level& lv, const double* s_dev, double t, double* parts, const double* phi_ref, double* phi_out,
                double* dz, double alpha = 0.0, const double* nstep = nullptr, double* s_out = nullptr);
  double trial_bytes(const Level& lv, bool with_ref) const;
  int fused_trial_rows_ = 64 * 2048;
  void enqueue_f0(Level& lv, const double* s_dev, double alpha, const double* nstep, double* s_out, double* dz,
                  const double* phi_ref, double* phi_out, double* out2, HostSignal sig = HostSignal());
  double dev_f1(Level& lv, const double* dz, double t, double* g_out, SolveStats* st = nullptr, const double** pre = nullptr);
  void enqueue_f2_assemble(Level& lv, const double* dz, SolveStats& st);
  bool values_stay_local(Level& lv);
  bool owner_local(Level& lv) { return in_solve_ && values_stay_local(lv); }
  bool in_solve_ = false;
  DevBuf<double> gtop_;
  struct EventHolder {
    hipEvent_t e = nullptr;
    ~EventHolder() {
      if (e) (void)hipEventDestroy(e);
    }
  } ev_f1_holder_;
  hipEvent_t& ev_f1_ = ev_f1_holder_.e;
  struct Trial {
    double* s = nullptr;
    double* phi = nullptr;
    double* dz = nullptr;
    double step = 0, y = 0;
    bool valid = false;
  };
  bool dev_f2_solve(Level& lv, const double* dz, double t, SolveStats& st, double* inc, Trial* spec = nullptr,
                    const double* pre_assembled = nullptr);
  void enqueue_trial(Level& lv, Trial& T, double step, int slot, HostSignal sig = HostSignal());
  int spec_count() const { return n_ <= fused_trial_rows_ ? 3 : 2; }
  void enqueue_spec_trials(Level& lv, Trial* spec, HostSignal sig);
  void launch_step_graph(Level& lv, Trial* spec);
  NewtonResult newton(int l, double t, bool finest, bool final, double lam_tol, int maxit, SolveStats& st, int verbose);
  bool amgb_step(double t, bool final, double lam_tol, int max_newton, std::vector<long long>& its, SolveStats& st, int verbose);
  double c_dot_dz();

 public:
  PcgOptions pcg_opt;
  void hessian_apply(int l, const double* s_host, const double* v_host, double* out_host, bool matrix_free);
  double mg_smooth(int l, const double* s_host, const double* b_host, double* x_host, int degree, int sweeps, double lmax,
                   bool matrix_free);
  void mg_prolong(int l, const double* xc_host, double* xf_host);
  void mg_restrict(int l, const double* rf_host, double* rc_host);
  int mg_coarsest(int top);
  bool pcg_solve_linear(int l, const double* s_host, const double* g_host, double* x_host, int* iters, double* relres);
  const Csr& prolongation_host(int l);
  struct MgKernelTimes {
    double ms[6], bytes[6], alg[6];
  };
  MgKernelTimes time_mg_kernels(int l, int reps, int nrot);

 private:
  Level::Mg& mg_of(Level& lv);
  void mg_ensure_vectors(Level& lv);
  bool mg_ensure_elop(Level& lv);
  void mg_ensure_assembled(Level& lv);
  void mg_ensure_transfer(int l);
  void mg_prepare(int top);
  bool mg_top_matrix_free(int top);
  void mg_values(int top);
  void mg_level_values(Level& lv, bool mf);
  void mg_estimate(Level& lv, bool mf, double lmax_given);
  void mg_apply(Level& lv, bool mf, const MgEpi& epi);
  void mg_smooth_pre(Level& lv, bool mf, const double* b, double* x, double* r, int degree, const double* done);
  void mg_smooth_post(Level& lv, bool mf, const double* b, double* x, double* r, int degree, const double* done);
  void mg_vcycle(int top, int l, const double* b, double* x, const double* done);
  bool pcg_run(Level& lv, int top, const double* g, double* x, SolveStats* st, int* iters, double* relres);
  void eval_Y_at(Level& lv, const double* s_host);
  std::vector<Csr> P_host_;
  DevBuf<double> mg_scal_, mg_scratch_, pcg_r_, pcg_z_, pcg_p_, pcg_Ap_;
  PinnedBuf<double> h_pcg_;
  DevBuf<int> mg_fail_;
  bool mg_inited_ = false;
  bool pcg_ = false;
  double pcg_last_code_ = 0;
  int pcg_bad_streak_ = 0;

  Ctx& ctx_;
  int n_ = 0, S_ = 0;
  int ng_ = 0, r0_ = 0;
  int early_stop_col_ = -1;
  bool slack_negative();
  DevBuf<float> w32_, c32_, Dz0_32_, Dz32_, v32_, Y32_;
  DevBuf<double> rowF_, rowC_, a_node_, mu_node_;
  DevBuf<unsigned char> term_mask_;
  void ensure_f32(Level& lv);
  BarrierParams P_;
  AmgSpec spec_;
  GeometryHost geo_;
  Csr dstack_host_;
  DevCsrOwned Dstack_;
  std::vector<std::unique_ptr<Level>> levels_;
  DevBuf<double> w_, c_, z_, z_save_, Dz0_, Dz0_save_, Dz_, DzA_, DzB_, DzC_, v_, Y_, partials_, scal_, phi_cur_, phi_trial_, phi_trial2_,
      phi_trial3_;
  PinnedBuf<int> h_flag_;
  bool host_solve_ = false;
  PinnedBuf<double> h_scal_;
  double w_min_ = 0;
  bool schedule_all_ = false;
  KernelTimer timer_;
  SolveStats* live_ = nullptr;
  void sync_collect(const char* what);
  DevBuf<unsigned long long> seq_dev_;
  PinnedBuf<unsigned long long> h_seq_;
  unsigned long long seq_expected_ = 0;
  void resync_signals();
  HostSignal next_signal();
  void wait_signal(const char* what);
  double* host_scal(double* dev_slot) const { return ctx_.world == 1 ? h_scal_.p + (dev_slot - scal_.p) : nullptr; }
};

}
```

### multigridbarriermpi.jl_amd/csrc/capi.cpp

```cpp
#include "../../include/mgb_hip.h"

#include <chrono>
#include <cmath>
#include <cstdlib>
#include <string>
#include <thread>

#include "amg.hpp"
#include "interp.hpp"

using namespace mgb;

struct mgb_ctx_s {
  Ctx ctx;
  explicit mgb_ctx_s(int dev) : ctx(dev) {}
};
struct mgb_geo_s {
  GeometryHost g;
};
struct mgb_vec_s {
  mgb_ctx_s* ctx;
  DevBuf<double> buf;
  int n;
};
// ... 442 lines not shown
  return guard([&] {
    need(ctx && out, "null argument");
    hip_check(hipSetDevice(ctx->ctx.device), "hipSetDevice");
    Csr A = make_csr(rows, cols, rowptr, colidx, vals, "mgb_csr_create");
    *out = new_csr(ctx, std::move(A));
  });
}
int mgb_csr_free(mgb_csr A) {
  return guard([&] { delete A; });
}
int mgb_csr_dims(mgb_csr A, int* rows, int* cols, int* nnz) {
  return guard([&] {
    need(A, "null argument");
    if (rows) *rows = A->host.rows;
    if (cols) *cols = A->host.cols;
    if (nnz) *nnz = A->host.nnz();
  });
}
int mgb_csr_get(mgb_csr A, int32_t* rowptr, int32_t* colidx, double* vals) {
  return guard([&] {
    need(A, "null argument");
    if (rowptr) std::copy(A->host.rowptr.begin(), A->host.rowptr.end(), rowptr);
    if (colidx) std::copy(A->host.colidx.begin(), A->host.colidx.end(), colidx);
    if (vals) std::copy(A->host.vals.begin(), A->host.vals.end(), vals);
  });
}
int mgb_csr_spgemm(mgb_csr A, mgb_csr B, mgb_csr* out) {
  return guard([&] {
    need(A && B && out, "null argument");
    *out = new_csr(A->ctx, spgemm(A->host, B->host));
  });
}
int mgb_csr_transpose(mgb_csr A, mgb_csr* out) {
  return guard([&] {
    need(A && out, "null argument");
    *out = new_csr(A->ctx, transpose(A->host));
  });
}
int mgb_csr_add(mgb_csr A, double alpha, mgb_csr B, mgb_csr* out) {
  return guard([&] {
    need(A && B && out, "null argument");
    *out = new_csr(A->ctx, add(A->host, alpha, B->host));
  });
}
static std::vector<const Csr*> host_list(int count, const mgb_csr* mats) {
  need(count >= 1 && mats, "empty matrix list");
  std::vector<const Csr*> v;
  for (int i = 0; i < count; ++i) {
    need(mats[i] != nullptr, "null matrix in list");
    v.push_back(&mats[i]->host);
  }
  return v;
}
int mgb_csr_hcat(int count, const mgb_csr* mats, mgb_csr* out) {
  return guard([&] {
    need(out, "null argument");
    auto v = host_list(count, mats);
    *out = new_csr(mats[0]->ctx, hcat(v));
  });
}
int mgb_csr_blockdiag(int count, const mgb_csr* mats, mgb_csr* out) {
  return guard([&] {
    need(out, "null argument");
    auto v = host_list(count, mats);
    *out = new_csr(mats[0]->ctx, blockdiag(v));
  });
}
int mgb_diag(mgb_ctx ctx, mgb_vec z, int m, int n, mgb_csr* out) {
  return guard([&] {
    need(ctx && z && out && m >= 0 && n >= 0, "diag: bad arguments");
    const int d = std::min(std::min(m, n), z->n);
    std::vector<double> h(z->n);
    hip_check(hipStreamSynchronize(ctx->ctx.stream), "sync");
    z->buf.download(h.data(), z->n);
    Csr A(m, n);
    for (int i = 0; i < m; ++i) {
      if (i < d) {
        A.colidx.push_back(i);
        A.vals.push_back(h[i]);
      }
      A.rowptr[i + 1] = (int)A.colidx.size();
    }
    *out = new_csr(ctx, std::move(A));
  });
}
int mgb_spmv_add(mgb_csr A, mgb_vec x, mgb_vec y0, mgb_vec y) {
  return guard([&] {
    need(A && x && y, "null argument");
    need(A->A.view.cols == x->n && A->A.view.rows == y->n && (!y0 || y0->n == y->n), "spmv: shape mismatch");
    launch_spmv(A->ctx->ctx.stream, A->A.view, x->buf.p, y0 ? y0->buf.p : nullptr, y->buf.p);
    hip_check(hipGetLastError(), "spmv launch");
  });
}
int mgb_spmv(mgb_csr A, mgb_vec x, mgb_vec y) { return mgb_spmv_add(A, x, nullptr, y); }
int mgb_dot(mgb_vec x, mgb_vec y, double* out) {
  return guard([&] {
    need(x && y && out && x->n == y->n, "dot: shape mismatch");
    *out = reduce_scalar(x, [&](hipStream_t st, double* parts, double* res) { launch_dot(st, x->n, x->buf.p, y->buf.p, parts, res); });
  });
}
int mgb_norm(mgb_vec x, double* out) {
  return guard([&] {
    need(x && out, "null argument");
    *out = std::sqrt(reduce_scalar(x, [&](hipStream_t st, double* parts, double* res) { launch_dot(st, x->n, x->buf.p, x->buf.p, parts, res); }));
  });
}
int mgb_sum(mgb_vec x, double* out) {
  return guard([&] {
    need(x && out, "null argument");
    *out = reduce_scalar(x, [&](hipStream_t st, double* parts, double* res) { launch_sum(st, x->n, x->buf.p, parts, res); });
  });
}
int mgb_col_extract(mgb_vec M, int n, int K, int k, mgb_vec out) {
  return guard([&] {
    need(M && out && n >= 0 && K >= 1 && k >= 0 && k < K, "col_extract: bad arguments");
    need((long long)n * K == M->n && out->n == n, "col_extract: shape mismatch");
    launch_col_extract(M->ctx->ctx.stream, n, K, k, M->buf.p, out->buf.p);
    hip_check(hipGetLastError(), "col_extract launch");
  });
}
int mgb_map_rows_barrier(int which, int K, int nterms, const int* kind, const int* nq, const int* idx_q, const int* idx_s,
                         const int* idx_s2, const double* p, const double* coef, const double* off, int n, mgb_vec Dz,
                         mgb_vec out) {
  return guard([&] {
    need(Dz && out && n >= 0 && K >= 1 && K <= 8 && which >= 0 && which <= 2, "map_rows_barrier: bad arguments");
    BarrierParams P = make_params_terms(K, nterms, kind, nq, idx_q, idx_s, idx_s2, p, coef, off);
    const long long want = which == 0 ? n : (which == 1 ? (long long)n * K : (long long)n * K * K);
    need((long long)n * K == Dz->n && out->n == want, "map_rows_barrier: shape mismatch");
    hipStream_t st = Dz->ctx->ctx.stream;
    hip_check(hipSetDevice(Dz->ctx->ctx.device), "hipSetDevice");
    if (which == 0) {
      launch_barrier_rows_F(st, n, P, Dz->buf.p, out->buf.p);
    } else {
      std::vector<double> ones((size_t)std::max(n, 1), 1.0);
      DevBuf<double> w;
      w.upload(ones.data(), ones.size());
      if (which == 1) {
        DevBuf<double> c;
        c.alloc((size_t)std::max(n, 1) * K);
        hip_check(hipMemsetAsync(c.p, 0, c.n * sizeof(double), st), "memset");
        if (n) launch_barrier_f1(st, n, P, Dz->buf.p, w.p, c.p, 0.0, out->buf.p);
        hip_check(hipStreamSynchronize(st), "sync");
      } else {
        DevBuf<double> Y;
        Y.alloc((size_t)std::max(n, 1) * P.nY());
        if (n) launch_barrier_f2(st, n, P, Dz->buf.p, w.p, Y.p);
        launch_expand_hessian_rows(st, n, P, Y.p, out->buf.p);
        hip_check(hipStreamSynchronize(st), "sync");
      }
    }
    hip_check(hipGetLastError(), "map_rows_barrier launch");
  });
}
int mgb_mul(mgb_vec x, mgb_vec y, mgb_vec out) {
  return guard([&] {
    need(x && y && out && x->n == y->n && x->n == out->n, "mul: shape mismatch");
    launch_mul(x->ctx->ctx.stream, x->n, x->buf.p, y->buf.p, out->buf.p);
  });
}
int mgb_axpy(mgb_vec x, double alpha, mgb_vec y, mgb_vec out) {
  return guard([&] {
    need(x && y && out && x->n == y->n && x->n == out->n, "axpy: shape mismatch");
    launch_waxpby(x->ctx->ctx.stream, x->n, x->buf.p, alpha, y->buf.p, out->buf.p);
  });
}
int mgb_vec_allreduce_sum(mgb_vec x) {
  return guard([&] {
    need(x, "null argument");
    x->ctx->ctx.allreduce_sum(x->buf.p, x->n, true);
    hip_check(hipStreamSynchronize(x->ctx->ctx.stream), "sync allreduce");
  });
}
int mgb_all_isfinite(mgb_vec x, int* out) {
  return guard([&] {
    need(x && out, "null argument");
    hipStream_t st = x->ctx->ctx.stream;
    DevBuf<int> flag;
    flag.alloc(1);
    launch_all_isfinite(st, x->n, x->buf.p, flag.p);
    hip_check(hipStreamSynchronize(st), "sync");
    int h = 0;
    flag.download(&h, 1);
    *out = h != 0;
  });
}

int mgb_amg_create(mgb_ctx ctx, mgb_geo g, int S, const char* const* state_vars, int K, const char* const* D, int nq,
                   const int* idx_q, int idx_s, double p, mgb_amg* out) {
  return guard([&] {
    need(ctx && g && out, "null argument");
    AmgSpec spec = make_spec(S, state_vars, K, D);
    BarrierParams P = make_params(K, nq, idx_q, idx_s, p);
    auto* a = new mgb_amg_s{ctx, nullptr, {}};
    try {
      const auto t0 = std::chrono::steady_clock::now();
      a->amg.reset(new Amg(ctx->ctx, g->g, spec, P));
      a->stats.t_setup = std::chrono::duration<double>(std::chrono::steady_clock::now() - t0).count();
    } catch (...) {
      delete a;
      throw;
    }
    *out = a;
  });
}
int mgb_amg_create_cones(mgb_ctx ctx, mgb_geo g, int S, const char* const* state_vars, int K, const char* const* D,
                         int ncones, const int* nq, const int* idx_q, const int* idx_s, const int* idx_s2,
                         const double* p, mgb_amg* out) {
  return guard([&] {
    need(ctx && g && out, "null argument");
    AmgSpec spec = make_spec(S, state_vars, K, D);
    BarrierParams P = make_params_cones(K, ncones, nq, idx_q, idx_s, idx_s2, p);
    auto* a = new mgb_amg_s{ctx, nullptr, {}};
    try {
      const auto t0 = std::chrono::steady_clock::now();
      a->amg.reset(new Amg(ctx->ctx, g->g, spec, P));
      a->stats.t_setup = std::chrono::duration<double>(std::chrono::steady_clock::now() - t0).count();
    } catch (...) {
      delete a;
      throw;
    }
    *out = a;
  });
}
int mgb_amg_create_terms(mgb_ctx ctx, mgb_geo g, int S, const char* const* state_vars, int K, const char* const* D, int nterms,
                         const int* kind, const int* nq, const int* idx_q, const int* idx_s, const int* idx_s2, const double* p,
                         const double* coef, const double* off, mgb_amg* out) {
  return guard([&] {
    need(ctx && g && out, "null argument");
    AmgSpec spec = make_spec(S, state_vars, K, D);
    BarrierParams P = make_params_terms(K, nterms, kind, nq, idx_q, idx_s, idx_s2, p, coef, off);
    auto* a = new mgb_amg_s{ctx, nullptr, {}};
    try {
      const auto t0 = std::chrono::steady_clock::now();
      a->amg.reset(new Amg(ctx->ctx, g->g, spec, P));
      a->stats.t_setup = std::chrono::duration<double>(std::chrono::steady_clock::now() - t0).count();
    } catch (...) {
      delete a;
      throw;
    }
    *out = a;
  });
}
int mgb_amg_destroy(mgb_amg a) {
  return guard([&] { delete a; });
}
int mgb_amg_dims(mgb_amg a, int* n, int* S, int* K, int* L, int* nY) {
  return guard([&] {
    need(a, "null amg");
    if (n) *n = a->amg->n();
    if (S) *S = a->amg->S();
    if (K) *K = a->amg->K();
    if (L) *L = a->amg->L();
    if (nY) *nY = a->amg->params().nY();
  });
}
int mgb_amg_local_rows(mgb_amg a, int* n_global, int* row0, int* n_local) {
  return guard([&] {
    need(a, "null amg");
    if (n_global) *n_global = a->amg->n_global();
    if (row0) *row0 = a->amg->row0();
    if (n_local) *n_local = a->amg->n();
  });
}
int mgb_amg_prepare(mgb_amg a, int level) {
  return guard([&] {
    need(a && level >= -1 && level < a->amg->L(), "level out of range");
    a->amg->prepare(level);
  });
}
int mgb_amg_set_exponents(mgb_amg a, int term, const double* p_nodes) {
  return guard([&] {
    need(a && p_nodes, "set_exponents: null argument");
    a->amg->set_exponents(term, p_nodes);
  });
}
int mgb_amg_set_term_mask(mgb_amg a, const unsigned char* mask) {
  return guard([&] {
    need(a && mask, "set_term_mask: null argument");
    a->amg->set_term_mask(mask);
  });
}
int mgb_amg_set_early_stop(mgb_amg a, int col) {
  return guard([&] {
    need(a && col >= -1, "set_early_stop: bad arguments");
    a->amg->set_early_stop(col);
  });
}
int mgb_amg_f0_f32(mgb_amg a, int level, const float* s, float t, double* f0) {
  return guard([&] {
    need(a && s && f0 && level >= 0 && level < a->amg->L(), "f0_f32: bad arguments");
    *f0 = a->amg->f0_f32(level, s, t);
  });
}
int mgb_amg_f1_f32(mgb_amg a, int level, const float* s, float t, float* g) {
  return guard([&] {
    need(a && s && g && level >= 0 && level < a->amg->L(), "f1_f32: bad arguments");
    a->amg->f1_f32(level, s, t, g);
  });
}
int mgb_amg_f2_f32(mgb_amg a, int level, const float* s, float t, float* lower_vals) {
  return guard([&] {
    need(a && s && lower_vals && level >= 0 && level < a->amg->L(), "f2_f32: bad arguments");
    a->amg->f2_f32(level, s, t, lower_vals);
  });
}
int mgb_amg_f1_template_f64(mgb_amg a, int level, const double* s, double t, double* g) {
// ... 675 lines not shown
```

### multigridbarriermpi.jl_amd/csrc/devutil.hpp

```cpp
#pragma once
#include <hip/hip_runtime.h>

#include "kernels.hpp"

namespace mgb {
namespace {

constexpr int kBlock = 256;
constexpr int kMaxBlocks = 2048;

inline int grid_for(long long work_items) {
  long long b = (work_items + kBlock - 1) / kBlock;
  if (b < 1) b = 1;
  if (b > kMaxBlocks) b = kMaxBlocks;
  return (int)b;
}

__device__ inline unsigned xcd_block(unsigned b, unsigned nb) {
  if (nb < 16u) return b;
  const unsigned per = nb >> 3, main = per << 3;
  return b < main ? (b & 7u) * per + (b >> 3) : b;
}

__device__ inline double wave_sum(double v) {
#pragma unroll
  for (int o = 32; o > 0; o >>= 1) v += __shfl_down(v, o, 64);
  return v;
}

__device__ inline double block_sum(double v, double* lds) {
  v = wave_sum(v);
  const int wave = threadIdx.x >> 6;
  if ((threadIdx.x & 63) == 0) lds[wave] = v;
  __syncthreads();
  double r = 0.0;
  if (threadIdx.x == 0)
    for (int i = 0; i < kBlock / 64; ++i) r += lds[i];
  __syncthreads();
  return r;
}

template <int N>
__device__ inline void block_sum_n(const double (&v)[N], double (&out)[N]) {
  __shared__ double red[N][kBlock / 64];
  const int wave = threadIdx.x >> 6;
#pragma unroll
  for (int o = 0; o < N; ++o) {
    const double w = wave_sum(v[o]);
    if ((threadIdx.x & 63) == 0) red[o][wave] = w;
  }
  __syncthreads();
#pragma unroll
  for (int o = 0; o < N; ++o) {
    double r = 0.0;
    if (threadIdx.x == 0)
      for (int i = 0; i < kBlock / 64; ++i) r += red[o][i];
    out[o] = r;
  }
  __syncthreads();
}

constexpr int kTicketDoubles = kReductionHeader;
constexpr int kTicketStride = 32;
static_assert(kReductionHeader * sizeof(double) >= 9 * kTicketStride * sizeof(unsigned), "ticket words");
template <int NOUT>
__device__ inline void grid_finish(const double (&r)[NOUT] , double* scratch, double* out_dev,
                                   double* out_host, double* lds, HostSignal sig = HostSignal(), unsigned slot = 0xffffffffu) {
  if (slot == 0xffffffffu) slot = blockIdx.x;
  __shared__ int is_last;
  unsigned* ticket = reinterpret_cast<unsigned*>(scratch);
  double* partials = scratch + kTicketDoubles;
  if (threadIdx.x == 0) {
#pragma unroll
    for (int o = 0; o < NOUT; ++o)
      __hip_atomic_store(&partials[(size_t)slot * NOUT + o], r[o], __ATOMIC_RELAXED, __HIP_MEMORY_SCOPE_AGENT);
    asm volatile("s_waitcnt vmcnt(0)" ::: "memory");
    const unsigned shard = blockIdx.x & 7u, nshards = gridDim.x < 8u ? gridDim.x : 8u;
    const unsigned in_shard = (gridDim.x - shard + 7u) / 8u;
    bool last = false;
    if (__hip_atomic_fetch_add(&ticket[kTicketStride * shard], 1u, __ATOMIC_RELAXED, __HIP_MEMORY_SCOPE_AGENT) == in_shard - 1) {
      __hip_atomic_store(&ticket[kTicketStride * shard], 0u, __ATOMIC_RELAXED, __HIP_MEMORY_SCOPE_AGENT);
      last = __hip_atomic_fetch_add(&ticket[kTicketStride * 8], 1u, __ATOMIC_RELAXED, __HIP_MEMORY_SCOPE_AGENT) == nshards - 1;
      if (last) __hip_atomic_store(&ticket[kTicketStride * 8], 0u, __ATOMIC_RELAXED, __HIP_MEMORY_SCOPE_AGENT);
    }
    is_last = last;
  }
  __syncthreads();
  if (!is_last) return;
  double acc[NOUT];
#pragma unroll
  for (int o = 0; o < NOUT; ++o) acc[o] = 0.0;
  for (int i0 = threadIdx.x; i0 < (int)gridDim.x; i0 += 4 * kBlock) {
    double v[4][NOUT];
#pragma unroll
    for (int u = 0; u < 4; ++u) {
      const int i = min(i0 + u * kBlock, (int)gridDim.x - 1);
#pragma unroll
      for (int o = 0; o < NOUT; ++o) v[u][o] = __hip_atomic_load(&partials[(size_t)i * NOUT + o], __ATOMIC_RELAXED, __HIP_MEMORY_SCOPE_AGENT);
    }
#pragma unroll
    for (int u = 0; u < 4; ++u)
#pragma unroll
      for (int o = 0; o < NOUT; ++o) acc[o] = (i0 + u * kBlock < (int)gridDim.x) ? acc[o] + v[u][o] : acc[o];
  }
  double tot[NOUT];
  block_sum_n<NOUT>(acc, tot);
  (void)lds;
  if (threadIdx.x == 0) {
#pragma unroll
    for (int o = 0; o < NOUT; ++o) {
      if (out_dev) out_dev[o] = tot[o];
      if (out_host) __hip_atomic_store(&out_host[o], tot[o], __ATOMIC_RELAXED, __HIP_MEMORY_SCOPE_SYSTEM);
    }
  }
  if (sig.seq_host && threadIdx.x == 0) {
    asm volatile("s_waitcnt vmcnt(0)" ::: "memory");
    const unsigned long long q = __hip_atomic_load(sig.seq_dev, __ATOMIC_RELAXED, __HIP_MEMORY_SCOPE_AGENT) + 1;
    __hip_atomic_store(sig.seq_dev, q, __ATOMIC_RELAXED, __HIP_MEMORY_SCOPE_AGENT);
    __hip_atomic_store(sig.seq_host, q, __ATOMIC_RELEASE, __HIP_MEMORY_SCOPE_SYSTEM);
  }
}
template <int NOUT, class Fn>
__device__ inline void grid_finish_fn(const double (&r)[NOUT] , double* scratch, double* lds, Fn&& fn) {
  __shared__ int is_last_fn;
  unsigned* ticket = reinterpret_cast<unsigned*>(scratch);
  double* partials = scratch + kTicketDoubles;
  if (threadIdx.x == 0) {
#pragma unroll
    for (int o = 0; o < NOUT; ++o)
      __hip_atomic_store(&partials[(size_t)blockIdx.x * NOUT + o], r[o], __ATOMIC_RELAXED, __HIP_MEMORY_SCOPE_AGENT);
    asm volatile("s_waitcnt vmcnt(0)" ::: "memory");
    const unsigned shard = blockIdx.x & 7u, nshards = gridDim.x < 8u ? gridDim.x : 8u;
    const unsigned in_shard = (gridDim.x - shard + 7u) / 8u;
    bool last = false;
    if (__hip_atomic_fetch_add(&ticket[kTicketStride * shard], 1u, __ATOMIC_RELAXED, __HIP_MEMORY_SCOPE_AGENT) == in_shard - 1) {
      __hip_atomic_store(&ticket[kTicketStride * shard], 0u, __ATOMIC_RELAXED, __HIP_MEMORY_SCOPE_AGENT);
      last = __hip_atomic_fetch_add(&ticket[kTicketStride * 8], 1u, __ATOMIC_RELAXED, __HIP_MEMORY_SCOPE_AGENT) == nshards - 1;
      if (last) __hip_atomic_store(&ticket[kTicketStride * 8], 0u, __ATOMIC_RELAXED, __HIP_MEMORY_SCOPE_AGENT);
    }
    is_last_fn = last;
  }
  __syncthreads();
  if (!is_last_fn) return;
  double tot[NOUT], acc[NOUT];
#pragma unroll
  for (int o = 0; o < NOUT; ++o) acc[o] = 0.0;
  for (int i0 = threadIdx.x; i0 < (int)gridDim.x; i0 += 4 * kBlock) {
    double v[4][NOUT];
#pragma unroll
    for (int u = 0; u < 4; ++u) {
      const int i = min(i0 + u * kBlock, (int)gridDim.x - 1);
#pragma unroll
      for (int o = 0; o < NOUT; ++o) v[u][o] = __hip_atomic_load(&partials[(size_t)i * NOUT + o], __ATOMIC_RELAXED, __HIP_MEMORY_SCOPE_AGENT);
    }
#pragma unroll
    for (int u = 0; u < 4; ++u)
#pragma unroll
      for (int o = 0; o < NOUT; ++o) acc[o] = (i0 + u * kBlock < (int)gridDim.x) ? acc[o] + v[u][o] : acc[o];
  }
  block_sum_n<NOUT>(acc, tot);
  (void)lds;
  if (threadIdx.x == 0) fn(tot);
}

}
}
```

### multigridbarriermpi.jl_amd/csrc/kernels.hip

```cpp
#include "kernels.hpp"
#include "kernels_tpl.hpp"

#include <algorithm>
#include <cmath>

namespace mgb {

namespace {


template <int G>
void spmv_launch(hipStream_t st, const DevCsr& A, const double* x, const double* y0, double* y) {
  const int grid = grid_for((long long)A.rows * G);
  hipLaunchKernelGGL((spmv_kernel_t<G, double>), dim3(grid), dim3(kBlock), 0, st, A.rows, A.rowptr, A.colidx, A.vals, x, y0, y);
}

template <int G>
__global__ __launch_bounds__(kBlock) void spmv_el_kernel(int rows, DevElCsr E, const int* __restrict__ rowptr,
                                                          const double* __restrict__ vals, const double* __restrict__ x,
                                                          const double* y0, double* y) {
  extern __shared__ double xs[];
  const int lane = threadIdx.x % G, grp = threadIdx.x / G;
  constexpr int GR = kBlock / G;
  const int rpe = E.rows_per_el;
  const int els = max(1, min(E.nel, (kBlock * 4) / rpe));
  const int npass = (E.nel + els - 1) / els;
  for (int ps = xcd_block(blockIdx.x, gridDim.x); ps < npass; ps += gridDim.x) {
    const int e0 = ps * els, ne = min(els, E.nel - e0);
    __syncthreads();
    for (int idx = threadIdx.x; idx < ne * E.cmax; idx += kBlock) xs[idx] = x[E.ecols[(long long)e0 * E.cmax + idx]];
    __syncthreads();
    const long long r0 = (long long)e0 * rpe;
    const int nrows = (int)min((long long)ne * rpe, (long long)rows - r0);
    for (int rr0 = grp; rr0 < nrows; rr0 += kSpmvU * GR) {
      int b[kSpmvU], e[kSpmvU];
      double acc[kSpmvU], base[kSpmvU];
#pragma unroll
      for (int u = 0; u < kSpmvU; ++u) {
        const int rr = rr0 + u * GR;
        const bool ok = rr < nrows;
        b[u] = ok ? rowptr[r0 + rr] : 0;
        e[u] = ok ? rowptr[r0 + rr + 1] : 0;
        base[u] = (ok && y0 && lane == 0) ? y0[r0 + rr] : 0.0;
      }
#pragma unroll
      for (int u = 0; u < kSpmvU; ++u) {
        const int rr = rr0 + u * GR;
        const double* xe = xs + (rr / rpe) * E.cmax;
        const int k = b[u] + lane;
        acc[u] = (k < e[u]) ? vals[k] * xe[E.lcol[k]] : 0.0;
        for (int kk = k + G; kk < e[u]; kk += G) acc[u] += vals[kk] * xe[E.lcol[kk]];
      }
#pragma unroll
      for (int u = 0; u < kSpmvU; ++u) {
        double a = acc[u];
#pragma unroll
        for (int o = G / 2; o > 0; o >>= 1) a += __shfl_down(a, o, G);
        const int rr = rr0 + u * GR;
        if (lane == 0 && rr < nrows) y[r0 + rr] = base[u] + a;
      }
    }
  }
}

template <int G>
void spmv_el_launch(hipStream_t st, const DevCsr& A, const DevElCsr& E, const double* x, const double* y0, double* y) {
  const int els = std::max(1, std::min(E.nel, (kBlock * 4) / E.rows_per_el));
  const int npass = (E.nel + els - 1) / els;
  const int grid = std::max(1, std::min(npass, kMaxBlocks * 4));
  hipLaunchKernelGGL(spmv_el_kernel<G>, dim3(grid), dim3(kBlock), (size_t)els * E.cmax * sizeof(double), st, A.rows, E, A.rowptr,
                     A.vals, x, y0, y);
}


using Cone = ConeT<double>;

__global__ __launch_bounds__(kBlock) void barrier_f0_kernel(int n, BarrierParams P, const double* __restrict__ Dz,
                                                             const double* __restrict__ w,
                                                             const double* __restrict__ c,
                                                             const double* __restrict__ phi_ref, double frac,
                                                             double* __restrict__ phi_out, double* scratch,
                                                             double* out_dev, double* out_host, HostSignal sig) {
  __shared__ double lds[kBlock / 64];
  double accF = 0.0, accL = 0.0;
  for (long long q = (long long)blockIdx.x * kBlock + threadIdx.x; q < n; q += (long long)gridDim.x * kBlock) {
    const double* dz = Dz + q * P.K;
    const double* cq = c + q * P.K;
    const double wq = w[q];
    double F = 0.0;
    for (int ci = 0; ci < P.ncones; ++ci) {
      if (!P.active(ci, q)) {
        if (phi_out) phi_out[q * P.ncones + ci] = INFINITY;
        continue;
      }
      const ConeAM<double> am = cone_am<double>(P, ci, q);
      Cone k = load_cone<double>(P.cone[ci], dz, am.a);
      if (phi_ref && !(k.phi >= frac * phi_ref[q * P.ncones + ci])) k.ok = false;
      if (phi_out) phi_out[q * P.ncones + ci] = k.phi;
      F += k.ok ? (-log(k.phi) - am.mu * log(k.s)) : INFINITY;
    }
    accF += wq * F;
    double lin = 0.0;
    for (int j = 0; j < P.K; ++j) lin += cq[j] * dz[j];
    accL += wq * lin;
  }
  const double r[2] = {block_sum(accF, lds), block_sum(accL, lds)};
  grid_finish<2>(r, scratch, out_dev, out_host, lds, sig);
}


constexpr int kTrialNodes = 64;
template <int G, int NA>
__global__ __launch_bounds__(kBlock) void trial_f0_kernel(int n, int N, BarrierParams P, const int* __restrict__ rowptr,
                                                           const int* __restrict__ colidx, const double* __restrict__ vals,
                                                           const double* __restrict__ s, const double* __restrict__ nstep,
                                                           TrialSet T, const double* __restrict__ Dz0,
                                                           const double* __restrict__ w, const double* __restrict__ c,
                                                           const double* __restrict__ phi_ref, double frac, double* scratch,
                                                           HostSignal sig) {
  __shared__ double lds[kBlock / 64];
  __shared__ double dzs[NA][kTrialNodes * kMaxK];
  constexpr int GR = kBlock / G;
  const int K = P.K, lane = threadIdx.x % G, grp = threadIdx.x / G;
#pragma unroll
  for (int a = 0; a < NA; ++a)
    if (T.s_out[a])
      for (long long i = (long long)blockIdx.x * kBlock + threadIdx.x; i < N; i += (long long)gridDim.x * kBlock)
        T.s_out[a][i] = s[i] + T.alpha[a] * nstep[i];
  auto xval = [&](int j, int a) { return nstep ? s[j] + T.alpha[a] * nstep[j] : s[j]; };
  double accF = 0.0, accL = 0.0;
  const int pa = threadIdx.x >> 6, pnode = threadIdx.x & 63;
  const int nchunks = (n + kTrialNodes - 1) / kTrialNodes;
  for (int ch = xcd_block(blockIdx.x, gridDim.x); ch < nchunks; ch += gridDim.x) {
    const int q0 = ch * kTrialNodes, nq = min(kTrialNodes, n - q0), nrows = nq * K;
    const long long r0 = (long long)q0 * K;
    for (int rr0 = grp; rr0 < nrows; rr0 += kSpmvU * GR) {
      int b[kSpmvU], e[kSpmvU], ci[kSpmvU];
      double acc[NA][kSpmvU], base[kSpmvU], va[kSpmvU];
#pragma unroll
      for (int u = 0; u < kSpmvU; ++u) {
        const int rr = rr0 + u * GR;
        const bool ok = rr < nrows;
        b[u] = ok ? rowptr[r0 + rr] : 0;
        e[u] = ok ? rowptr[r0 + rr + 1] : 0;
        base[u] = (ok && lane == 0) ? Dz0[r0 + rr] : 0.0;
      }
#pragma unroll
      for (int u = 0; u < kSpmvU; ++u) {
        const int k = b[u] + lane;
        const bool in = k < e[u];
        ci[u] = in ? colidx[k] : -1;
        va[u] = in ? vals[k] : 0.0;
      }
#pragma unroll
      for (int a = 0; a < NA; ++a)
#pragma unroll
        for (int u = 0; u < kSpmvU; ++u) acc[a][u] = (ci[u] >= 0) ? va[u] * xval(ci[u], a) : 0.0;
#pragma unroll
      for (int u = 0; u < kSpmvU; ++u)
        for (int k = b[u] + lane + G; k < e[u]; k += G) {
          const double vk = vals[k];
          const int ck = colidx[k];
#pragma unroll
          for (int a = 0; a < NA; ++a) acc[a][u] += vk * xval(ck, a);
        }
#pragma unroll
      for (int a = 0; a < NA; ++a)
#pragma unroll
        for (int u = 0; u < kSpmvU; ++u) {
          double t = acc[a][u];
#pragma unroll
          for (int o = G / 2; o > 0; o >>= 1) t += __shfl_down(t, o, G);
          const int rr = rr0 + u * GR;
          if (lane == 0 && rr < nrows) {
            const double v = base[u] + t;
            T.dz[a][r0 + rr] = v;
            dzs[a][rr] = v;
          }
        }
    }
    __syncthreads();
    if (pa < NA && pnode < nq) {
      const long long q = q0 + pnode;
      const double* dz = dzs[pa] + pnode * K;
      const double* cq = c + q * K;
      const double wq = w[q];
      double* phi_out = T.phi_out[pa];
      double F = 0.0;
      for (int ci2 = 0; ci2 < P.ncones; ++ci2) {
        if (!P.active(ci2, q)) {
          if (phi_out) phi_out[q * P.ncones + ci2] = INFINITY;
          continue;
        }
        const ConeAM<double> am = cone_am<double>(P, ci2, q);
        Cone k = load_cone<double>(P.cone[ci2], dz, am.a);
        if (phi_ref && !(k.phi >= frac * phi_ref[q * P.ncones + ci2])) k.ok = false;
        if (phi_out) phi_out[q * P.ncones + ci2] = k.phi;
        F += k.ok ? (-log(k.phi) - am.mu * log(k.s)) : INFINITY;
      }
      accF += wq * F;
      double lin = 0.0;
      for (int j = 0; j < K; ++j) lin += cq[j] * dz[j];
      accL += wq * lin;
    }
    __syncthreads();
  }
  double r[2 * NA], mine[2 * NA];
#pragma unroll
  for (int a = 0; a < NA; ++a) {
    mine[2 * a] = pa == a ? accF : 0.0;
    mine[2 * a + 1] = pa == a ? accL : 0.0;
  }
  block_sum_n<2 * NA>(mine, r);
  grid_finish<2 * NA>(r, scratch, T.out_dev, T.out_host, lds, sig, xcd_block(blockIdx.x, gridDim.x));
}

inline int trial_grid(int n) {
  const int b = (n + kTrialNodes - 1) / kTrialNodes;
  return b < 1 ? 1 : (b > kMaxBlocks ? kMaxBlocks : b);
}

template <int G>
void trial_launch(hipStream_t st, const DevCsr& B, int n, const BarrierParams& P, const double* s, const double* nstep,
                  const TrialSet& T, const double* Dz0, const double* w, const double* c, const double* phi_ref, double frac,
                  double* scratch, HostSignal sig) {
#define MGB_TRIAL_NA(NA)                                                                                                    \
  hipLaunchKernelGGL((trial_f0_kernel<G, NA>), dim3(trial_grid(n)), dim3(kBlock), 0, st, n, B.cols, P, B.rowptr, B.colidx,   \
                     B.vals, s, nstep, T, Dz0, w, c, phi_ref, frac, scratch, sig)
  switch (T.na) {
    case 1: MGB_TRIAL_NA(1); break;
    case 2: MGB_TRIAL_NA(2); break;
    default: MGB_TRIAL_NA(3); break;
  }
#undef MGB_TRIAL_NA
}

__global__ __launch_bounds__(kBlock) void barrier_rows_F_kernel(int n, BarrierParams P, const double* __restrict__ Dz,
                                                                 double* __restrict__ out) {
  for (long long q = (long long)blockIdx.x * kBlock + threadIdx.x; q < n; q += (long long)gridDim.x * kBlock) {
    const double* dz = Dz + q * P.K;
    double F = 0.0;
    for (int ci = 0; ci < P.ncones; ++ci) {
      if (!P.active(ci, q)) continue;
      const ConeAM<double> am = cone_am<double>(P, ci, q);
      Cone k = load_cone<double>(P.cone[ci], dz, am.a);
      F += k.ok ? (-log(k.phi) - am.mu * log(k.s)) : INFINITY;
    }
    out[q] = F;
  }
}

__global__ __launch_bounds__(kBlock) void expand_hessian_rows_kernel(int n, BarrierParams P, const double* __restrict__ Y,
                                                                      double* __restrict__ out) {
  const int K = P.K, nY = P.nY();
  for (long long q = (long long)blockIdx.x * kBlock + threadIdx.x; q < n; q += (long long)gridDim.x * kBlock) {
    double* o = out + q * K * K;
    for (int e = 0; e < K * K; ++e) o[e] = 0.0;
    const double* yq = Y + q * nY;
    int slot = 0;
    for (int ci = 0; ci < P.ncones; ++ci) {
      const ConeSpec& S = P.cone[ci];
      const int nact = S.nact();
      for (int a = 0; a < nact; ++a)
        for (int b = a; b < nact; ++b, ++slot) {
          const int ra = S.col(a), rb = S.col(b);
          o[ra * K + rb] += yq[slot];
          if (ra != rb) o[rb * K + ra] += yq[slot];
        }
    }
  }
}

__global__ __launch_bounds__(kBlock) void waxpby_kernel(int n, const double* __restrict__ x, double alpha,
                                                         const double* __restrict__ y, double* out) {
  for (long long i = (long long)blockIdx.x * kBlock + threadIdx.x; i < n; i += (long long)gridDim.x * kBlock)
    out[i] = x[i] + alpha * y[i];
}

__global__ __launch_bounds__(kBlock) void mul_kernel(int n, const double* __restrict__ x, const double* __restrict__ y,
                                                      double* out) {
  for (long long i = (long long)blockIdx.x * kBlock + threadIdx.x; i < n; i += (long long)gridDim.x * kBlock)
    out[i] = x[i] * y[i];
}

__global__ __launch_bounds__(kBlock) void col_extract_kernel(int n, int K, int k, const double* __restrict__ M,
                                                              double* out) {
  for (long long i = (long long)blockIdx.x * kBlock + threadIdx.x; i < n; i += (long long)gridDim.x * kBlock)
    out[i] = M[i * K + k];
}

__global__ __launch_bounds__(kBlock) void dot_kernel(int n, const double* __restrict__ x, const double* __restrict__ y,
                                                      double* scratch, double* out_dev, double* out_host, int* flag_dev,
                                                      int* flag_host, HostSignal sig) {
  __shared__ double lds[kBlock / 64];
  if (flag_dev && blockIdx.x == 0 && threadIdx.x == 0) {
    const int f = __hip_atomic_load(flag_dev, __ATOMIC_RELAXED, __HIP_MEMORY_SCOPE_AGENT);
    __hip_atomic_store(flag_host, f, __ATOMIC_RELAXED, __HIP_MEMORY_SCOPE_SYSTEM);
    __hip_atomic_store(flag_dev, 0, __ATOMIC_RELAXED, __HIP_MEMORY_SCOPE_AGENT);
  }
  double acc = 0.0;
  for (long long i = (long long)blockIdx.x * kBlock + threadIdx.x; i < n; i += (long long)gridDim.x * kBlock)
    acc += x[i] * y[i];
  const double r[1] = {block_sum(acc, lds)};
  grid_finish<1>(r, scratch, out_dev, out_host, lds, sig);
}

__global__ __launch_bounds__(kBlock) void dot_owned_kernel(int n, const double* __restrict__ x, const double* __restrict__ y,
                                                            const int* __restrict__ kind, int count_top, double* scratch,
                                                            double* out_dev) {
  __shared__ double lds[kBlock / 64];
  double acc = 0.0;
  for (long long i = (long long)blockIdx.x * kBlock + threadIdx.x; i < n; i += (long long)gridDim.x * kBlock) {
    const int k = kind[i];
    if (k == 1 || (k == 2 && count_top)) acc += x[i] * y[i];
  }
  const double r[1] = {block_sum(acc, lds)};
  grid_finish<1>(r, scratch, out_dev, nullptr, lds);
}

__global__ __launch_bounds__(kBlock) void gather_top_kernel(int ntop, const int* __restrict__ top, const double* __restrict__ g,
                                                             double* __restrict__ buf) {
  for (long long i = (long long)blockIdx.x * kBlock + threadIdx.x; i < ntop; i += (long long)gridDim.x * kBlock) buf[i] = g[top[i]];
}

__global__ __launch_bounds__(kBlock) void scatter_top_norm_kernel(int ntop, const int* __restrict__ top, const double* __restrict__ buf,
                                                                   double* __restrict__ g, double* out) {
  __shared__ double lds[kBlock / 64];
  double acc = 0.0;
  for (int i = threadIdx.x; i < ntop; i += kBlock) {
    const double v = buf[i];
    g[top[i]] = v;
    acc += v * v;
  }
  const double tot = block_sum(acc, lds);
  if (threadIdx.x == 0) out[0] = buf[ntop] + tot;
}

__global__ void flag_to_double_kernel(const int* flag_dev, double* out) {
  if (threadIdx.x == 0 && blockIdx.x == 0) out[0] = *flag_dev != 0 ? 1.0 : 0.0;
}

__global__ __launch_bounds__(kBlock) void sum_kernel(int n, const double* __restrict__ x, double* scratch, double* out_dev,
                                                      double* out_host) {
  __shared__ double lds[kBlock / 64];
  double acc = 0.0;
  for (long long i = (long long)blockIdx.x * kBlock + threadIdx.x; i < n; i += (long long)gridDim.x * kBlock) acc += x[i];
  const double r[1] = {block_sum(acc, lds)};
  grid_finish<1>(r, scratch, out_dev, out_host, lds);
}

__global__ __launch_bounds__(kBlock) void isfinite_kernel(int n, const double* __restrict__ x, int* flag) {
  int bad = 0;
  for (long long i = (long long)blockIdx.x * kBlock + threadIdx.x; i < n; i += (long long)gridDim.x * kBlock)
    bad |= !isfinite(x[i]);
  if (__any(bad) && (threadIdx.x & 63) == 0) atomicAnd(flag, 0);
}

}

void launch_spmv(hipStream_t st, const DevCsr& A, const double* x, const double* y0, double* y) {
  if (A.rows == 0) return;
  switch (A.group) {
    case 1: spmv_launch<1>(st, A, x, y0, y); break;
    case 2: spmv_launch<2>(st, A, x, y0, y); break;
    case 4: spmv_launch<4>(st, A, x, y0, y); break;
    case 8: spmv_launch<8>(st, A, x, y0, y); break;
    case 16: spmv_launch<16>(st, A, x, y0, y); break;
    case 32: spmv_launch<32>(st, A, x, y0, y); break;
    default: spmv_launch<64>(st, A, x, y0, y); break;
  }
}

void launch_spmv_el(hipStream_t st, const DevCsr& A, const DevElCsr& E, const double* x, const double* y0, double* y) {
  if (A.rows == 0) return;
  switch (A.group) {
    case 1: spmv_el_launch<1>(st, A, E, x, y0, y); break;
    case 2: spmv_el_launch<2>(st, A, E, x, y0, y); break;
    case 4: spmv_el_launch<4>(st, A, E, x, y0, y); break;
    case 8: spmv_el_launch<8>(st, A, E, x, y0, y); break;
    case 16: spmv_el_launch<16>(st, A, E, x, y0, y); break;
    case 32: spmv_el_launch<32>(st, A, E, x, y0, y); break;
    default: spmv_el_launch<64>(st, A, E, x, y0, y); break;
  }
}

void launch_waxpby(hipStream_t st, int n, const double* x, double alpha, const double* y, double* out) {
  if (n == 0) return;
  hipLaunchKernelGGL(waxpby_kernel, dim3(grid_for(n)), dim3(kBlock), 0, st, n, x, alpha, y, out);
}

int f0_blocks(int n) { return std::max(grid_for(n), trial_grid(n)); }

void launch_trial_set(hipStream_t st, const DevCsr& B, int n, BarrierParams P, const double* s, const double* nstep,
                      const TrialSet& T, const double* Dz0, const double* w, const double* c, const double* phi_ref, double frac,
                      double* scratch, HostSignal sig) {
#define MGB_TRIAL(G) trial_launch<G>(st, B, n, P, s, nstep, T, Dz0, w, c, phi_ref, frac, scratch, sig)
  switch (B.group) {
    case 1: MGB_TRIAL(1); break;
    case 2: MGB_TRIAL(2); break;
    case 4: MGB_TRIAL(4); break;
    case 8: MGB_TRIAL(8); break;
    case 16: MGB_TRIAL(16); break;
    case 32: MGB_TRIAL(32); break;
    default: MGB_TRIAL(64); break;
  }
#undef MGB_TRIAL
}

void launch_trial_f0(hipStream_t st, const DevCsr& B, int n, BarrierParams P, const double* s, double alpha,
                     const double* nstep, double* s_out, const double* Dz0, double* Dz, const double* w, const double* c,
                     const double* phi_ref, double frac, double* phi_out, double* scratch, double* out2, double* out2_host,
                     HostSignal sig) {
  TrialSet T;
  T.na = 1;
  T.alpha[0] = alpha;
  T.s_out[0] = s_out;
  T.dz[0] = Dz;
  T.phi_out[0] = phi_out;
  T.out_dev = out2;
  T.out_host = out2_host;
  launch_trial_set(st, B, n, P, s, nstep, T, Dz0, w, c, phi_ref, frac, scratch, sig);
}

void launch_barrier_f0(hipStream_t st, int n, BarrierParams P, const double* Dz, const double* w, const double* c,
                       const double* phi_ref, double frac, double* phi_out, double* scratch, double* out2, double* out2_host,
                       HostSignal sig) {
  hipLaunchKernelGGL(barrier_f0_kernel, dim3(grid_for(n)), dim3(kBlock), 0, st, n, P, Dz, w, c, phi_ref, frac, phi_out, scratch,
                     out2, out2_host, sig);
}

void launch_barrier_f1(hipStream_t st, int n, BarrierParams P, const double* Dz, const double* w, const double* c,
                       double t, double* v) {
  hipLaunchKernelGGL(barrier_f1_kernel_t<double>, dim3(grid_for(n)), dim3(kBlock), 0, st, n, P, Dz, w, c, t, v);
}

void launch_barrier_f2(hipStream_t st, int n, BarrierParams P, const double* Dz, const double* w, double* Y) {
  hipLaunchKernelGGL(barrier_f2_kernel_t<double>, dim3(grid_for(n)), dim3(kBlock), 0, st, n, P, Dz, w, Y);
}

void launch_barrier_rows_F(hipStream_t st, int n, BarrierParams P, const double* Dz, double* out) {
  if (n == 0) return;
  hipLaunchKernelGGL(barrier_rows_F_kernel, dim3(grid_for(n)), dim3(kBlock), 0, st, n, P, Dz, out);
}

void launch_expand_hessian_rows(hipStream_t st, int n, BarrierParams P, const double* Y, double* out) {
  if (n == 0) return;
  hipLaunchKernelGGL(expand_hessian_rows_kernel, dim3(grid_for(n)), dim3(kBlock), 0, st, n, P, Y, out);
}

void launch_dot(hipStream_t st, int n, const double* x, const double* y, double* scratch, double* out, double* out_host,
                int* flag_dev, int* flag_host, HostSignal sig) {
  hipLaunchKernelGGL(dot_kernel, dim3(grid_for(n)), dim3(kBlock), 0, st, n, x, y, scratch, out, out_host, flag_dev, flag_host, sig);
}

void launch_dot_owned(hipStream_t st, int n, const double* x, const double* y, const int* kind, int count_top, double* scratch,
                      double* out) {
  hipLaunchKernelGGL(dot_owned_kernel, dim3(grid_for(n)), dim3(kBlock), 0, st, n, x, y, kind, count_top, scratch, out);
}

void launch_gather_top(hipStream_t st, int ntop, const int* top, const double* g, double* buf) {
  if (ntop > 0) hipLaunchKernelGGL(gather_top_kernel, dim3(grid_for(ntop)), dim3(kBlock), 0, st, ntop, top, g, buf);
}

void launch_scatter_top_norm(hipStream_t st, int ntop, const int* top, const double* buf, double* g, double* out) {
  hipLaunchKernelGGL(scatter_top_norm_kernel, dim3(1), dim3(kBlock), 0, st, ntop, top, buf, g, out);
}

void launch_flag_to_double(hipStream_t st, const int* flag_dev, double* out) {
  hipLaunchKernelGGL(flag_to_double_kernel, dim3(1), dim3(64), 0, st, flag_dev, out);
}

void launch_sum(hipStream_t st, int n, const double* x, double* scratch, double* out, double* out_host) {
  hipLaunchKernelGGL(sum_kernel, dim3(grid_for(n)), dim3(kBlock), 0, st, n, x, scratch, out, out_host);
}

void launch_all_isfinite(hipStream_t st, int n, const double* x, int* flag) {
  (void)hipMemsetAsync(flag, 0xFF, sizeof(int), st);
  if (n == 0) return;
  hipLaunchKernelGGL(isfinite_kernel, dim3(grid_for(n)), dim3(kBlock), 0, st, n, x, flag);
}

void launch_mul(hipStream_t st, int n, const double* x, const double* y, double* out) {
  if (n == 0) return;
  hipLaunchKernelGGL(mul_kernel, dim3(grid_for(n)), dim3(kBlock), 0, st, n, x, y, out);
}

void launch_col_extract(hipStream_t st, int n, int K, int k, const double* M, double* out) {
  if (n == 0) return;
  hipLaunchKernelGGL(col_extract_kernel, dim3(grid_for(n)), dim3(kBlock), 0, st, n, K, k, M, out);
}

}
```

### multigridbarriermpi.jl_amd/csrc/kernels.hpp

```cpp
#pragma once
#include <hip/hip_runtime.h>

namespace mgb {

struct DevCsr {
  int rows = 0, cols = 0, nnz = 0, group = 1;
  int* rowptr = nullptr;
  int* colidx = nullptr;
  double* vals = nullptr;
};

struct DevElCsr {
  int rows_per_el = 0, cmax = 0, nel = 0;
  const int* ecols = nullptr;
  const unsigned char* lcol = nullptr;
  bool valid() const { return nel > 0; }
};

struct ConeSpec {
  int kind = 0;
  int nq = 0;
  int iq[3] = {0, 0, 0};
  int is = 0;
  int is2 = -1;
  double a = 2.0;
  double mu = 1.0;
  double coef[3] = {0.0, 0.0, 0.0};
  double off = 0.0;
  __host__ __device__ int nact() const { return kind == 1 ? nq : nq + 1 + (is2 >= 0 ? 1 : 0); }
  __host__ __device__ int nY() const { return nact() * (nact() + 1) / 2; }
  __host__ __device__ int col(int a) const { return a < nq ? iq[a] : (a == nq ? is : is2); }
};

constexpr int kMaxCones = 3;
struct BarrierParams {
  int K = 0;
  int ncones = 1;
  ConeSpec cone[kMaxCones];
  const double* a_node = nullptr;
  const double* mu_node = nullptr;
  const unsigned char* term_mask = nullptr;
  __host__ __device__ bool active(int ci, long long q) const { return !term_mask || term_mask[q * ncones + ci]; }
  __host__ __device__ int nY() const {
    int s = 0;
    for (int c = 0; c < ncones; ++c) s += cone[c].nY();
    return s;
  }
};

void launch_spmv(hipStream_t st, const DevCsr& A, const double* x, const double* y0, double* y);
void launch_spmv_el(hipStream_t st, const DevCsr& A, const DevElCsr& E, const double* x, const double* y0, double* y);
void launch_spmv_f32(hipStream_t st, const DevCsr& A, const float* vals, const float* x, const float* y0, float* y);
void launch_barrier_f0_rows_f32(hipStream_t st, int n, BarrierParams P, const float* Dz, const float* w, const float* c,
                                double* outF, double* outC);
void launch_barrier_f1_f32(hipStream_t st, int n, BarrierParams P, const float* Dz, const float* w, const float* c, float t, float* v);
void launch_barrier_f2_f32(hipStream_t st, int n, BarrierParams P, const float* Dz, const float* w, float* Y);
void launch_to_f32(hipStream_t st, long long n, const double* in, float* out);
void launch_spmv_tpl_f64(hipStream_t st, const DevCsr& A, const double* x, const double* y0, double* y);
void launch_barrier_f1_tpl_f64(hipStream_t st, int n, BarrierParams P, const double* Dz, const double* w, const double* c, double t,
                               double* v);
void launch_barrier_f2_tpl_f64(hipStream_t st, int n, BarrierParams P, const double* Dz, const double* w, double* Y);
void launch_waxpby(hipStream_t st, int n, const double* x, double alpha, const double* y, double* out);
constexpr int kReductionHeader = 144;
struct HostSignal {
  unsigned long long* seq_dev = nullptr;
  unsigned long long* seq_host = nullptr;
};
int f0_blocks(int n);
void launch_barrier_f0(hipStream_t st, int n, BarrierParams P, const double* Dz, const double* w, const double* c,
                       const double* phi_ref, double frac, double* phi_out, double* scratch, double* out2,
                       double* out2_host = nullptr, HostSignal sig = HostSignal());
void launch_trial_f0(hipStream_t st, const DevCsr& B, int n, BarrierParams P, const double* s, double alpha,
                     const double* nstep, double* s_out, const double* Dz0, double* Dz, const double* w, const double* c,
                     const double* phi_ref, double frac, double* phi_out, double* scratch, double* out2,
                     double* out2_host = nullptr, HostSignal sig = HostSignal());
struct TrialSet {
  int na = 0;
  double alpha[3] = {0.0, 0.0, 0.0};
  double* s_out[3] = {nullptr, nullptr, nullptr};
  double* dz[3] = {nullptr, nullptr, nullptr};
  double* phi_out[3] = {nullptr, nullptr, nullptr};
  double* out_dev = nullptr;
  double* out_host = nullptr;
};
void launch_trial_set(hipStream_t st, const DevCsr& B, int n, BarrierParams P, const double* s, const double* nstep,
                      const TrialSet& T, const double* Dz0, const double* w, const double* c, const double* phi_ref, double frac,
                      double* scratch, HostSignal sig = HostSignal());
void launch_barrier_f1(hipStream_t st, int n, BarrierParams P, const double* Dz, const double* w, const double* c,
                       double t, double* v);
void launch_barrier_f2(hipStream_t st, int n, BarrierParams P, const double* Dz, const double* w, double* Y);
void launch_barrier_rows_F(hipStream_t st, int n, BarrierParams P, const double* Dz, double* out);
void launch_expand_hessian_rows(hipStream_t st, int n, BarrierParams P, const double* Y, double* out);
void launch_dot(hipStream_t st, int n, const double* x, const double* y, double* scratch, double* out, double* out_host = nullptr,
                int* flag_dev = nullptr, int* flag_host = nullptr, HostSignal sig = HostSignal());
void launch_dot_owned(hipStream_t st, int n, const double* x, const double* y, const int* kind, int count_top, double* scratch,
                      double* out);
void launch_gather_top(hipStream_t st, int ntop, const int* top, const double* g, double* buf);
void launch_scatter_top_norm(hipStream_t st, int ntop, const int* top, const double* buf, double* g, double* out);
void launch_flag_to_double(hipStream_t st, const int* flag_dev, double* out);
void launch_sum(hipStream_t st, int n, const double* x, double* scratch, double* out, double* out_host = nullptr);
void launch_all_isfinite(hipStream_t st, int n, const double* x, int* flag);
void launch_mul(hipStream_t st, int n, const double* x, const double* y, double* out);
void launch_col_extract(hipStream_t st, int n, int K, int k, const double* M, double* out);

}
```

### multigridbarriermpi.jl_amd/csrc/kernels_tpl.hpp

```cpp
#pragma once
#include "devutil.hpp"

namespace mgb {
namespace {

constexpr int kMaxK = 8;

constexpr int kSpmvU = 2;
template <int G, class T>
__global__ __launch_bounds__(kBlock) void spmv_kernel_t(int rows, const int* __restrict__ rowptr, const int* __restrict__ colidx,
                                                         const T* __restrict__ vals, const T* __restrict__ x, const T* y0, T* y) {
  const int lane = threadIdx.x % G;
  const long long stride = (long long)gridDim.x * (kBlock / G);
  for (long long row0 = (long long)xcd_block(blockIdx.x, gridDim.x) * (kBlock / G) + threadIdx.x / G; row0 < rows;
       row0 += kSpmvU * stride) {
    int b[kSpmvU], e[kSpmvU];
    T acc[kSpmvU], base[kSpmvU];
#pragma unroll
    for (int u = 0; u < kSpmvU; ++u) {
      const long long row = row0 + u * stride;
      const bool ok = row < rows;
      b[u] = ok ? rowptr[row] : 0;
      e[u] = ok ? rowptr[row + 1] : 0;
      base[u] = (ok && y0 && lane == 0) ? y0[row] : T(0);
      acc[u] = T(0);
    }
    int ci[kSpmvU];
    T va[kSpmvU];
#pragma unroll
    for (int u = 0; u < kSpmvU; ++u) {
      const int k = b[u] + lane;
      const bool in = k < e[u];
      ci[u] = in ? colidx[k] : -1;
      va[u] = in ? vals[k] : T(0);
    }
#pragma unroll
    for (int u = 0; u < kSpmvU; ++u) acc[u] = (ci[u] >= 0) ? va[u] * x[ci[u]] : T(0);
#pragma unroll
    for (int u = 0; u < kSpmvU; ++u)
      for (int k = b[u] + lane + G; k < e[u]; k += G) acc[u] += vals[k] * x[colidx[k]];
#pragma unroll
    for (int u = 0; u < kSpmvU; ++u) {
      T a = acc[u];
#pragma unroll
      for (int o = G / 2; o > 0; o >>= 1) a += __shfl_down(a, o, G);
      const long long row = row0 + u * stride;
      if (lane == 0 && row < rows) y[row] = base[u] + a;
    }
  }
}

template <class T>
struct ConeT {
  T q[3];
  T s, phi, sa;
  bool ok;
};

template <class T>
__device__ inline T pow_a(T s, T a) {
  if (a == T(2)) return s * s;
  if (a == T(1)) return s;
  return pow(s, a);
}

template <class T>
struct ConeAM {
  T a, mu;
};
template <class T>
__device__ inline ConeAM<T> cone_am(const BarrierParams& P, int ci, long long q) {
  ConeAM<T> r;
  r.a = P.a_node ? T(P.a_node[q * P.ncones + ci]) : T(P.cone[ci].a);
  r.mu = P.mu_node ? T(P.mu_node[q * P.ncones + ci]) : T(P.cone[ci].mu);
  return r;
}

template <class T>
__device__ inline ConeT<T> load_cone(const ConeSpec& P, const T* dz, T a) {
  ConeT<T> c;
  if (P.kind == 1) {
    T phi = T(P.off);
#pragma unroll
    for (int i = 0; i < 3; ++i) {
      c.q[i] = (i < P.nq) ? dz[P.iq[i]] : T(0);
      phi += (i < P.nq) ? T(P.coef[i]) * c.q[i] : T(0);
    }
    c.s = T(1);
    c.sa = T(1);
    c.phi = phi;
    c.ok = phi > T(0);
    return c;
  }
  T qq = T(0);
#pragma unroll
  for (int i = 0; i < 3; ++i) {
    c.q[i] = (i < P.nq) ? dz[P.iq[i]] : T(0);
    qq += c.q[i] * c.q[i];
  }
  c.s = dz[P.is] + (P.is2 >= 0 ? dz[P.is2] : T(0));
  c.ok = c.s > T(0);
  c.sa = c.ok ? pow_a<T>(c.s, a) : T(-1);
  c.phi = c.sa - qq;
  c.ok = c.ok && (c.phi > T(0));
  return c;
}

template <class T>
__device__ inline T pick3(const T (&q)[3], int i) {
  return i == 0 ? q[0] : (i == 1 ? q[1] : q[2]);
}

template <class T>
__global__ __launch_bounds__(kBlock) void barrier_f0_rows_kernel_t(int n, BarrierParams P, const T* __restrict__ Dz,
                                                                    const T* __restrict__ w, const T* __restrict__ c,
                                                                    double* __restrict__ outF, double* __restrict__ outC) {
  for (long long q = (long long)blockIdx.x * kBlock + threadIdx.x; q < n; q += (long long)gridDim.x * kBlock) {
    const T* dz = Dz + q * P.K;
    T F = T(0);
    for (int ci = 0; ci < P.ncones; ++ci) {
      if (!P.active(ci, q)) continue;
      const ConeAM<T> am = cone_am<T>(P, ci, q);
      const ConeT<T> k = load_cone<T>(P.cone[ci], dz, am.a);
      F += k.ok ? (-log(k.phi) - am.mu * log(k.s)) : T(INFINITY);
    }
    T cd = T(0);
#pragma unroll
    for (int j = 0; j < kMaxK; ++j) cd += (j < P.K) ? c[q * P.K + j] * dz[j] : T(0);
    outF[q] = (double)(w[q] * F);
    outC[q] = (double)(w[q] * cd);
  }
}

template <class T>
__global__ __launch_bounds__(kBlock) void barrier_f1_kernel_t(int n, BarrierParams P, const T* __restrict__ Dz,
                                                               const T* __restrict__ w, const T* __restrict__ c, T t,
                                                               T* __restrict__ v) {
  for (long long q = (long long)blockIdx.x * kBlock + threadIdx.x; q < n; q += (long long)gridDim.x * kBlock) {
    const T* dz = Dz + q * P.K;
    const T* cq = c + q * P.K;
    const T wq = w[q];
    T vr[kMaxK];
#pragma unroll
    for (int j = 0; j < kMaxK; ++j) vr[j] = (j < P.K) ? wq * (t * cq[j]) : T(0);
    for (int ci = 0; ci < P.ncones; ++ci) {
      const ConeSpec& S = P.cone[ci];
      if (!P.active(ci, q)) continue;
      const ConeAM<T> am = cone_am<T>(P, ci, q);
      const ConeT<T> k = load_cone<T>(S, dz, am.a);
      if (S.kind == 1) {
#pragma unroll
        for (int j = 0; j < kMaxK; ++j) {
          T add = T(0);
#pragma unroll
          for (int i = 0; i < 3; ++i) add += (i < S.nq && S.iq[i] == j) ? -wq * (T(S.coef[i]) / k.phi) : T(0);
          vr[j] += add;
        }
        continue;
      }
      const T ds = am.a * pow_a<T>(k.s, am.a - T(1));
      const T gs = wq * (-ds / k.phi - am.mu / k.s);
#pragma unroll
      for (int j = 0; j < kMaxK; ++j) {
        T add = T(0);
#pragma unroll
        for (int i = 0; i < 3; ++i) add += (i < S.nq && S.iq[i] == j) ? wq * (T(2) * k.q[i] / k.phi) : T(0);
        add += (S.is == j) ? gs : T(0);
        add += (S.is2 == j) ? gs : T(0);
        vr[j] += add;
      }
    }
    T* vq = v + q * P.K;
#pragma unroll
    for (int j = 0; j < kMaxK; ++j)
      if (j < P.K) vq[j] = vr[j];
  }
}

template <class T>
__global__ __launch_bounds__(kBlock) void barrier_f2_kernel_t(int n, BarrierParams P, const T* __restrict__ Dz,
                                                               const T* __restrict__ w, T* __restrict__ Y) {
  const int nY = P.nY();
  for (long long q = (long long)blockIdx.x * kBlock + threadIdx.x; q < n; q += (long long)gridDim.x * kBlock) {
    const T* dz = Dz + q * P.K;
    T* yq = Y + q * nY;
    const T wq = w[q];
    int slot = 0;
    for (int ci = 0; ci < P.ncones; ++ci) {
      const ConeSpec& S = P.cone[ci];
      if (!P.active(ci, q)) {
        const int ns = S.nY();
        for (int i = 0; i < ns; ++i) yq[slot++] = T(0);
        continue;
      }
      const ConeAM<T> am = cone_am<T>(P, ci, q);
      const ConeT<T> k = load_cone<T>(S, dz, am.a);
      if (S.kind == 1) {
        const T ip2l = T(1) / (k.phi * k.phi);
#pragma unroll
        for (int i = 0; i < 3; ++i)
#pragma unroll
          for (int j = 0; j < 3; ++j)
            if (i < S.nq && j >= i && j < S.nq) yq[slot++] = wq * (T(S.coef[i]) * T(S.coef[j]) * ip2l);
        continue;
      }
      const T a = am.a;
      const T ds = a * pow_a<T>(k.s, a - T(1));
      const T dds = (a == T(1)) ? T(0) : a * (a - T(1)) * pow_a<T>(k.s, a - T(2));
      const T ip = T(1) / k.phi, ip2 = ip * ip;
      const T hss = -dds * ip + ds * ds * ip2 + am.mu / (k.s * k.s);
      const int nq = S.nq, nact = S.nact();
#pragma unroll
      for (int i = 0; i < 5; ++i)
#pragma unroll
        for (int j = 0; j < 5; ++j) {
          if (i < nact && j >= i && j < nact) {
            const int ai = min(i, nq), aj = min(j, nq);
            T h;
            if (aj < nq) h = T(4) * pick3<T>(k.q, ai) * pick3<T>(k.q, aj) * ip2 + (ai == aj ? T(2) * ip : T(0));
            else if (ai < nq) h = T(-2) * pick3<T>(k.q, ai) * ds * ip2;
            else h = hss;
            yq[slot++] = wq * h;
          }
        }
    }
  }
}


}
}
```

Measured before the change: 88.91 million DoF/s per Newton step.

## Fuse barrier f1/f2 kernels, SpMV with norm, and step dot into trial set

Adds three fusions, each switchable through an MGB_STEP_FUSE env mask that is all-on by default. The barrier gradient and Hessian rows are computed in one kernel so Dz and w are read once. The restriction SpMV also reduces the gradient norm, removing a separate dot pass. The Newton-step dot product is folded into the three-point trial-set kernel. The goal is fewer launches and fewer memory passes per Newton step, at the cost of more complex kernels that may use more registers, with each fusion applying only on a single rank under size limits.

Result: slower. 85.48 million DoF/s per Newton step (-3.9%).

```diff
diff --git a/include/mgb_hip.h b/include/mgb_hip.h
--- a/include/mgb_hip.h
+++ b/include/mgb_hip.h
@@ -71,6 +71,14 @@
 int mgb_map_rows_barrier(int which, int K, int nterms, const int* kind, const int* nq, const int* idx_q, const int* idx_s,
                          const int* idx_s2, const double* p, const double* coef, const double* off, int n, mgb_vec Dz,
                          mgb_vec out);
+int mgb_spmv_norm(mgb_csr A, mgb_vec x, mgb_vec y, double* out);
+int mgb_trial_dot(mgb_csr B, int K, int nterms, const int* kind, const int* nq, const int* idx_q, const int* idx_s,
+                  const int* idx_s2, const double* p, const double* coef, const double* off, int n, mgb_vec s, mgb_vec nstep,
+                  const double* alpha3, mgb_vec Dz0, mgb_vec w, mgb_vec c, mgb_vec g, int flag_in, int fused, mgb_vec out,
+                  double* sums7, int* flag_host, int* flag_dev, int* rode);
+int mgb_barrier_f12(int K, int nterms, const int* kind, const int* nq, const int* idx_q, const int* idx_s, const int* idx_s2,
+                    const double* p, const double* coef, const double* off, int n, mgb_vec Dz, mgb_vec w, mgb_vec c, double t,
+                    const double* a_node, const double* mu_node, const unsigned char* mask, int fused, mgb_vec v, mgb_vec Y);
 int mgb_mul(mgb_vec x, mgb_vec y, mgb_vec out);
 int mgb_axpy(mgb_vec x, double alpha, mgb_vec y, mgb_vec out);
 int mgb_vec_allreduce_sum(mgb_vec x);
diff --git a/multigridbarriermpi.jl_amd/__init__.py b/multigridbarriermpi.jl_amd/__init__.py
--- a/multigridbarriermpi.jl_amd/__init__.py
+++ b/multigridbarriermpi.jl_amd/__init__.py
@@ -709,6 +709,47 @@
     def __call__(self, x_row, dz_row):
         r = self.rows(HPCMatrix(np.asarray(dz_row, dtype=np.float64).reshape(1, -1))).to_numpy()
         return float(r[0]) if self.which == 0 else r[0]
+
+
+def spmv_norm(A: "HPCSparseMatrix", x: "HPCVector"):
+    y = HPCVector(A.shape[0], A.backend)
+    out = C.c_double()
+    call("mgb_spmv_norm", A.handle, x.handle, y.handle, C.byref(out))
+    return y, out.value
+
+
+def trial_dot(B: "HPCSparseMatrix", cones, K: int, s, nstep, alphas, Dz0, w, c, g, flag: int = 0, fused: bool = True):
+    n, N = B.shape[0] // K, B.shape[1]
+    nt = len(cones)
+    be = B.backend
+    vec = lambda a: HPCVector(np.asarray(a, dtype=np.float64), be)
+    per = N + n * K + n * nt
+    out = HPCVector(3 * per, be)
+    sums = np.zeros(7)
+    al = f64(np.asarray(alphas, dtype=np.float64))
+    fh, fd, rode = C.c_int(), C.c_int(), C.c_int()
+    hs, hn, hz, hw, hc, hg = vec(s), vec(nstep), vec(Dz0), vec(w), vec(c), vec(g)
+    call("mgb_trial_dot", B.handle, K, *_encode_terms(cones), n, hs.handle, hn.handle, dptr(al), hz.handle, hw.handle, hc.handle,
+         hg.handle, int(flag), int(bool(fused)), out.handle, dptr(sums), C.byref(fh), C.byref(fd), C.byref(rode))
+    o = out.to_numpy().reshape(3, per)
+    return dict(dot=sums[0], sums=sums[1:].reshape(3, 2), x=o[:, :N], dz=o[:, N:N + n * K].reshape(3, n, K),
+                phi=o[:, N + n * K:].reshape(3, n, nt), flag_host=fh.value, flag_dev=fd.value, rode=bool(rode.value))
+
+
+def barrier_f12(cones, K: int, Dz, w, c, t: float, a_node=None, mu_node=None, mask=None, fused: bool = True):
+    Dz = np.asarray(Dz, dtype=np.float64)
+    n = Dz.shape[0]
+    be = backend_hip()
+    nt, kind, nq, iq, isl, is2, pp, coef, off = _encode_terms(cones)
+    nY = sum((m * (m + 1)) // 2 for m in ((nq[i] if kind[i] == 1 else nq[i] + 1 + (1 if is2[i] >= 0 else 0)) for i in range(nt)))
+    hD, hw, hc = HPCVector(Dz, be), HPCVector(np.asarray(w, dtype=np.float64), be), HPCVector(np.asarray(c, dtype=np.float64), be)
+    v, Y = HPCVector(n * K, be), HPCVector(n * nY, be)
+    an = None if a_node is None else f64(np.asarray(a_node, dtype=np.float64).reshape(n, nt))
+    mn = None if mu_node is None else f64(np.asarray(mu_node, dtype=np.float64).reshape(n, nt))
+    mk = None if mask is None else np.ascontiguousarray(np.asarray(mask).reshape(n, nt), dtype=np.uint8)
+    call("mgb_barrier_f12", K, nt, kind, nq, iq, isl, is2, pp, coef, off, n, hD.handle, hw.handle, hc.handle, float(t), dptr(an),
+         dptr(mn), None if mk is None else mk.ctypes.data_as(C.POINTER(C.c_ubyte)), int(bool(fused)), v.handle, Y.handle)
+    return v.to_numpy().reshape(n, K), Y.to_numpy().reshape(n, nY)
 
 
 def barrier_functions(cones, K: int):
diff --git a/multigridbarriermpi.jl_amd/_lib.py b/multigridbarriermpi.jl_amd/_lib.py
--- a/multigridbarriermpi.jl_amd/_lib.py
+++ b/multigridbarriermpi.jl_amd/_lib.py
@@ -66,6 +66,11 @@
     "mgb_col_extract": [H, C.c_int, C.c_int, C.c_int, H],
     "mgb_map_rows_barrier": [C.c_int, C.c_int, C.c_int, c_int_p, c_int_p, c_int_p, c_int_p, c_int_p, c_dbl_p, c_dbl_p, c_dbl_p,
                              C.c_int, H, H],
+    "mgb_spmv_norm": [H, H, H, c_dbl_p],
+    "mgb_trial_dot": [H, C.c_int, C.c_int, c_int_p, c_int_p, c_int_p, c_int_p, c_int_p, c_dbl_p, c_dbl_p, c_dbl_p, C.c_int, H, H,
+                      c_dbl_p, H, H, H, H, C.c_int, C.c_int, H, c_dbl_p, c_int_p, c_int_p, c_int_p],
+    "mgb_barrier_f12": [C.c_int, C.c_int, c_int_p, c_int_p, c_int_p, c_int_p, c_int_p, c_dbl_p, c_dbl_p, c_dbl_p, C.c_int, H, H, H,
+                        C.c_double, c_dbl_p, c_dbl_p, C.POINTER(C.c_ubyte), C.c_int, H, H],
     "mgb_mul": [H, H, H],
     "mgb_axpy": [H, C.c_double, H, H],
     "mgb_vec_allreduce_sum": [H],
diff --git a/multigridbarriermpi.jl_amd/csrc/amg.cpp b/multigridbarriermpi.jl_amd/csrc/amg.cpp
--- a/multigridbarriermpi.jl_amd/csrc/amg.cpp
+++ b/multigridbarriermpi.jl_amd/csrc/amg.cpp
@@ -485,7 +485,7 @@
 }
 
 size_t reduction_scratch_doubles(int n_local, int max_level_unknowns) {
-  return (size_t)6 * std::max(f0_blocks(n_local), f0_blocks(max_level_unknowns)) + 8 + kReductionHeader;
+  return (size_t)7 * std::max(f0_blocks(n_local), f0_blocks(max_level_unknowns)) + 8 + kReductionHeader;
 }
 
 int Amg::level_index(const Level& lv) const {
@@ -847,10 +847,21 @@
   return lv.gchol.values_local();
 }
 
-void Amg::enqueue_f2_assemble(Level& lv, const double* dz, SolveStats& st) {
-  timer_.begin(ctx_.stream, KC_F2, (double)n_ * (P_.K + 1 + P_.nY()) * 8);
-  launch_barrier_f2(ctx_.stream, n_, P_, dz, w_.p, Y_.p);
-  timer_.end(ctx_.stream);
+enum { kFuseDot = 1, kFuseNorm = 2, kFuseF12 = 4 };
+static int step_fuse() {
+  static const int mask = [] {
+    const char* e = std::getenv("MGB_STEP_FUSE");
+    return e ? std::atoi(e) & 7 : 7;
+  }();
+  return mask;
+}
+
+void Amg::enqueue_f2_assemble(Level& lv, const double* dz, SolveStats& st, bool have_Y) {
+  if (!have_Y) {
+    timer_.begin(ctx_.stream, KC_F2, (double)n_ * (P_.K + 1 + P_.nY()) * 8);
+    launch_barrier_f2(ctx_.stream, n_, P_, dz, w_.p, Y_.p);
+    timer_.end(ctx_.stream);
+  }
   if (pcg_) {
     mg_values(level_index(lv));
     st.n_f2++;
@@ -864,11 +875,21 @@
 }
 
 double Amg::dev_f1(Level& lv, const double* dz, double t, double* g_out, SolveStats* st, const double** pre) {
-  timer_.begin(ctx_.stream, KC_F1, (double)n_ * (3 * P_.K + 1) * 8);
-  launch_barrier_f1(ctx_.stream, n_, P_, dz, w_.p, c_.p, t, v_.p);
+  const bool with_f2 = (step_fuse() & kFuseF12) && pre && st && !host_solve_ && !pcg_;
+  if (with_f2) {
+    timer_.begin(ctx_.stream, KC_F1, (double)n_ * (3 * P_.K + 1 + P_.nY()) * 8);
+    launch_barrier_f12(ctx_.stream, n_, P_, dz, w_.p, c_.p, t, v_.p, Y_.p);
+  } else {
+    timer_.begin(ctx_.stream, KC_F1, (double)n_ * (3 * P_.K + 1) * 8);
+    launch_barrier_f1(ctx_.stream, n_, P_, dz, w_.p, c_.p, t, v_.p);
+  }
   timer_.end(ctx_.stream);
+  const bool norm_rides = ctx_.world == 1 && (step_fuse() & kFuseNorm) && spmv_norm_fits(lv.BT.view.rows);
   timer_.begin(ctx_.stream, KC_RESTRICT, csr_bytes(lv.BT.view, false));
-  launch_spmv(ctx_.stream, lv.BT.view, v_.p, nullptr, g_out);
+  if (norm_rides)
+    launch_spmv_norm(ctx_.stream, lv.BT.view, v_.p, nullptr, g_out, partials_.p, scal_.p + 2, host_scal(scal_.p + 2), next_signal());
+  else
+    launch_spmv(ctx_.stream, lv.BT.view, v_.p, nullptr, g_out);
   timer_.end(ctx_.stream);
   if (owner_local(lv)) {
     const int ntop = lv.gchol.ntop_unknowns();
@@ -877,7 +898,7 @@
     launch_dot_owned(ctx_.stream, lv.plan.N, g_out, g_out, lv.gchol.unknown_kind(), 0, partials_.p, gtop_.p + ntop);
     ctx_.allreduce_sum(gtop_.p, ntop + 1);
     launch_scatter_top_norm(ctx_.stream, ntop, lv.gchol.top_unknowns(), gtop_.p, g_out, scal_.p + 2);
-  } else {
+  } else if (!norm_rides) {
     ctx_.allreduce_sum(g_out, lv.plan.N);
     launch_dot(ctx_.stream, lv.plan.N, g_out, g_out, partials_.p, scal_.p + 2, host_scal(scal_.p + 2), nullptr, nullptr, next_signal());
   }
@@ -892,7 +913,7 @@
       if (!ev_f1_) hip_check(hipEventCreateWithFlags(&ev_f1_, hipEventDisableTiming), "event");
       hip_check(hipEventRecord(ev_f1_, ctx_.stream), "record f1");
     }
-    enqueue_f2_assemble(lv, dz, *st);
+    enqueue_f2_assemble(lv, dz, *st, with_f2);
     *pre = dz;
     if (ctx_.world == 1) wait_signal("sync f1");
     else hip_check(hipEventSynchronize(ev_f1_), "sync f1 event");
@@ -912,7 +933,23 @@
 
 static const double kSpecSteps[3] = {1.0, kBeta, kBeta * kBeta};
 
-void Amg::enqueue_spec_trials(Level& lv, Trial* spec, HostSignal sig) {
+bool Amg::dot_rides(const Level& lv) const {
+  return (step_fuse() & kFuseDot) && ctx_.world == 1 && spec_count() == 3 && trial_dot_rides(n_, lv.plan.N);
+}
+
+TrialDot Amg::step_dot(Level& lv) {
+  TrialDot D;
+  D.x = lv.g.p;
+  D.y = lv.nstep.p;
+  D.N = lv.plan.N;
+  D.flag_dev = lv.gchol.fail_flag();
+  D.flag_host = h_flag_.p;
+  D.out_dev = scal_.p + 3;
+  D.out_host = host_scal(scal_.p + 3);
+  return D;
+}
+
+void Amg::enqueue_spec_trials(Level& lv, Trial* spec, HostSignal sig, const TrialDot* dot) {
   const int ns = spec_count();
   if (ns == 3) {
     TrialSet T;
@@ -926,11 +963,12 @@
     }
     T.out_dev = scal_.p + 4;
     T.out_host = host_scal(scal_.p + 4);
-    timer_.begin(ctx_.stream, KC_F0, trial_bytes(lv, true) + 2.0 * n_ * (P_.K + P_.ncones) * 8);
+    timer_.begin(ctx_.stream, KC_F0, trial_bytes(lv, true) + 2.0 * n_ * (P_.K + P_.ncones) * 8 + (dot ? 2.0 * dot->N * 8 : 0.0));
     launch_trial_set(ctx_.stream, lv.B.view, n_, P_, lv.s.p, lv.nstep.p, T, Dz0_.p, w_.p, c_.p, phi_cur_.p, kFracToBoundary,
-                     partials_.p, sig);
+                     partials_.p, sig, dot);
     timer_.end(ctx_.stream);
   } else {
+    if (dot) throw InternalError("enqueue_spec_trials: the dot rides with three points only");
     enqueue_trial(lv, spec[0], kSpecSteps[0], 0);
     enqueue_trial(lv, spec[1], kSpecSteps[1], 1, sig);
   }
@@ -950,12 +988,15 @@
   hip_check(hipStreamBeginCapture(ctx_.stream, hipStreamCaptureModeThreadLocal), "hipStreamBeginCapture");
   try {
     lv.gchol.enqueue_chain(ctx_.stream, lv.avals.p, lv.g.p, lv.nstep.p);
-    launch_dot(ctx_.stream, lv.plan.N, lv.g.p, lv.nstep.p, partials_.p, scal_.p + 3, host_scal(scal_.p + 3), lv.gchol.fail_flag(),
-               h_flag_.p);
+    const bool rides = dot_rides(lv);
+    if (!rides)
+      launch_dot(ctx_.stream, lv.plan.N, lv.g.p, lv.nstep.p, partials_.p, scal_.p + 3, host_scal(scal_.p + 3), lv.gchol.fail_flag(),
+                 h_flag_.p);
     HostSignal sig;
     sig.seq_dev = seq_dev_.p;
     sig.seq_host = h_seq_.p;
-    enqueue_spec_trials(lv, spec, sig);
+    const TrialDot D = step_dot(lv);
+    enqueue_spec_trials(lv, spec, sig, rides ? &D : nullptr);
   } catch (...) {
     (void)hipStreamEndCapture(ctx_.stream, &graph);
     if (graph) (void)hipGraphDestroy(graph);
@@ -1035,21 +1076,24 @@
         hip_check(hipEventRecord(e0, ctx_.stream), "record");
       }
       const bool olocal = owner_local(lv);
+      const bool rides = flag_rides && !olocal && spec && dot_rides(lv);
       lv.gchol.factor_solve(ctx_.stream, lv.avals.p, lv.g.p, lv.nstep.p, tm, flag_rides && lv.flag_armed, false, olocal);
       if (time_chain) hip_check(hipEventRecord(e1, ctx_.stream), "record");
       if (olocal) {
         launch_dot_owned(ctx_.stream, N, lv.g.p, lv.nstep.p, lv.gchol.unknown_kind(), ctx_.rank == 0, partials_.p, scal_.p + 3);
         launch_flag_to_double(ctx_.stream, lv.gchol.fail_flag(), scal_.p + 10);
       } else if (flag_rides) {
-        launch_dot(ctx_.stream, N, lv.g.p, lv.nstep.p, partials_.p, scal_.p + 3, host_scal(scal_.p + 3), lv.gchol.fail_flag(),
-                   h_flag_.p, spec ? HostSignal() : next_signal());
+        if (!rides)
+          launch_dot(ctx_.stream, N, lv.g.p, lv.nstep.p, partials_.p, scal_.p + 3, host_scal(scal_.p + 3), lv.gchol.fail_flag(),
+                     h_flag_.p, spec ? HostSignal() : next_signal());
         lv.flag_armed = true;
       } else {
         launch_dot(ctx_.stream, N, lv.g.p, lv.nstep.p, partials_.p, scal_.p + 3);
         hip_check(hipMemcpyAsync(h_flag_.p, lv.gchol.fail_flag(), sizeof(int), hipMemcpyDeviceToHost, ctx_.stream), "D2H flag");
       }
       if (spec) {
-        enqueue_spec_trials(lv, spec, next_signal());
+        const TrialDot D = step_dot(lv);
+        enqueue_spec_trials(lv, spec, next_signal(), rides ? &D : nullptr);
         if (!olocal) ctx_.allreduce_sum(scal_.p + 4, 2 * spec_count());
         st.n_f0 += spec_count();
       }
diff --git a/multigridbarriermpi.jl_amd/csrc/amg.hpp b/multigridbarriermpi.jl_amd/csrc/amg.hpp
--- a/multigridbarriermpi.jl_amd/csrc/amg.hpp
+++ b/multigridbarriermpi.jl_amd/csrc/amg.hpp
@@ -325,7 +325,7 @@
   void enqueue_f0(Level& lv, const double* s_dev, double alpha, const double* nstep, double* s_out, double* dz,
                   const double* phi_ref, double* phi_out, double* out2, HostSignal sig = HostSignal());
   double dev_f1(Level& lv, const double* dz, double t, double* g_out, SolveStats* st = nullptr, const double** pre = nullptr);
-  void enqueue_f2_assemble(Level& lv, const double* dz, SolveStats& st);
+  void enqueue_f2_assemble(Level& lv, const double* dz, SolveStats& st, bool have_Y = false);
   bool values_stay_local(Level& lv);
   bool owner_local(Level& lv) { return in_solve_ && values_stay_local(lv); }
   bool in_solve_ = false;
@@ -348,7 +348,9 @@
                     const double* pre_assembled = nullptr);
   void enqueue_trial(Level& lv, Trial& T, double step, int slot, HostSignal sig = HostSignal());
   int spec_count() const { return n_ <= fused_trial_rows_ ? 3 : 2; }
-  void enqueue_spec_trials(Level& lv, Trial* spec, HostSignal sig);
+  void enqueue_spec_trials(Level& lv, Trial* spec, HostSignal sig, const TrialDot* dot = nullptr);
+  bool dot_rides(const Level& lv) const;
+  TrialDot step_dot(Level& lv);
   void launch_step_graph(Level& lv, Trial* spec);
   NewtonResult newton(int l, double t, bool finest, bool final, double lam_tol, int maxit, SolveStats& st, int verbose);
   bool amgb_step(double t, bool final, double lam_tol, int max_newton, std::vector<long long>& its, SolveStats& st, int verbose);
diff --git a/multigridbarriermpi.jl_amd/csrc/capi.cpp b/multigridbarriermpi.jl_amd/csrc/capi.cpp
--- a/multigridbarriermpi.jl_amd/csrc/capi.cpp
+++ b/multigridbarriermpi.jl_amd/csrc/capi.cpp
@@ -618,6 +618,100 @@
     hip_check(hipGetLastError(), "map_rows_barrier launch");
   });
 }
+int mgb_spmv_norm(mgb_csr A, mgb_vec x, mgb_vec y, double* out) {
+  return guard([&] {
+    need(A && x && y && out, "null argument");
+    need(A->A.view.cols == x->n && A->A.view.rows == y->n, "spmv_norm: shape mismatch");
+    need(spmv_norm_fits(A->A.view.rows), "spmv_norm: 1 to 256 * 2048 rows");
+    hip_check(hipSetDevice(A->ctx->ctx.device), "hipSetDevice");
+    *out = reduce_scalar(y, [&](hipStream_t st, double* parts, double* res) {
+      launch_spmv_norm(st, A->A.view, x->buf.p, nullptr, y->buf.p, parts, res);
+    });
+  });
+}
+int mgb_trial_dot(mgb_csr B, int K, int nterms, const int* kind, const int* nq, const int* idx_q, const int* idx_s,
+                  const int* idx_s2, const double* p, const double* coef, const double* off, int n, mgb_vec s, mgb_vec nstep,
+                  const double* alpha3, mgb_vec Dz0, mgb_vec w, mgb_vec c, mgb_vec g, int flag_in, int fused, mgb_vec out,
+                  double* sums7, int* flag_host, int* flag_dev, int* rode) {
+  return guard([&] {
+    need(B && s && nstep && alpha3 && Dz0 && w && c && g && out && sums7 && flag_host && flag_dev && rode, "trial_dot: null argument");
+    need(n >= 1 && K >= 1 && K <= 8, "trial_dot: bad arguments");
+    BarrierParams P = make_params_terms(K, nterms, kind, nq, idx_q, idx_s, idx_s2, p, coef, off);
+    const int N = B->A.view.cols;
+    const long long nK = (long long)n * K, per = N + nK + (long long)n * P.ncones;
+    need(B->A.view.rows == nK && N >= 1 && s->n == N && nstep->n == N && g->n == N && Dz0->n == nK && w->n == n && c->n == nK &&
+             out->n == 3 * per, "trial_dot: shape mismatch");
+    hipStream_t st = B->ctx->ctx.stream;
+    hip_check(hipSetDevice(B->ctx->ctx.device), "hipSetDevice");
+    DevBuf<double> scratch, res;
+    scratch.alloc((size_t)kReductionHeader + 7 * (size_t)std::max(f0_blocks(n), f0_blocks(N)) + 8);
+    hip_check(hipMemsetAsync(scratch.p, 0, kReductionHeader * sizeof(double), st), "memset ticket");
+    res.alloc(7);
+    DevBuf<int> fdev;
+    fdev.upload(&flag_in, 1);
+    PinnedBuf<int> fhost;
+    fhost.alloc(1);
+    fhost.p[0] = -1;
+    TrialSet T;
+    T.na = 3;
+    for (int a = 0; a < 3; ++a) {
+      T.alpha[a] = alpha3[a];
+      T.s_out[a] = out->buf.p + a * per;
+      T.dz[a] = T.s_out[a] + N;
+      T.phi_out[a] = T.dz[a] + nK;
+    }
+    T.out_dev = res.p + 1;
+    TrialDot D;
+    D.x = g->buf.p;
+    D.y = nstep->buf.p;
+    D.N = N;
+    D.flag_dev = fdev.p;
+    D.flag_host = fhost.p;
+    D.out_dev = res.p;
+    *rode = fused && trial_dot_rides(n, N);
+    if (!*rode) launch_dot(st, N, D.x, D.y, scratch.p, D.out_dev, nullptr, D.flag_dev, D.flag_host);
+    launch_trial_set(st, B->A.view, n, P, s->buf.p, nstep->buf.p, T, Dz0->buf.p, w->buf.p, c->buf.p, nullptr, 0.0, scratch.p,
+                     HostSignal(), *rode ? &D : nullptr);
+    hip_check(hipGetLastError(), "trial_dot launch");
+    hip_check(hipStreamSynchronize(st), "sync trial_dot");
+    res.download(sums7, 7);
+    fdev.download(flag_dev, 1);
+    *flag_host = fhost.p[0];
+  });
+}
+int mgb_barrier_f12(int K, int nterms, const int* kind, const int* nq, const int* idx_q, const int* idx_s, const int* idx_s2,
+                    const double* p, const double* coef, const double* off, int n, mgb_vec Dz, mgb_vec w, mgb_vec c, double t,
+                    const double* a_node, const double* mu_node, const unsigned char* mask, int fused, mgb_vec v, mgb_vec Y) {
+  return guard([&] {
+    need(Dz && w && c && v && Y && n >= 1 && K >= 1 && K <= 8, "barrier_f12: bad arguments");
+    need((a_node == nullptr) == (mu_node == nullptr), "barrier_f12: a_node and mu_node come together");
+    BarrierParams P = make_params_terms(K, nterms, kind, nq, idx_q, idx_s, idx_s2, p, coef, off);
+    const long long nK = (long long)n * K;
+    need(Dz->n == nK && w->n == n && c->n == nK && v->n == nK && Y->n == (long long)n * P.nY(), "barrier_f12: shape mismatch");
+    hipStream_t st = Dz->ctx->ctx.stream;
+    hip_check(hipSetDevice(Dz->ctx->ctx.device), "hipSetDevice");
+    DevBuf<double> an, mn;
+    DevBuf<unsigned char> mk;
+    if (a_node) {
+      an.upload(a_node, (size_t)n * P.ncones);
+      mn.upload(mu_node, (size_t)n * P.ncones);
+      P.a_node = an.p;
+      P.mu_node = mn.p;
+    }
+    if (mask) {
+      mk.upload(mask, (size_t)n * P.ncones);
+      P.term_mask = mk.p;
+    }
+    if (fused) {
+      launch_barrier_f12(st, n, P, Dz->buf.p, w->buf.p, c->buf.p, t, v->buf.p, Y->buf.p);
+    } else {
+      launch_barrier_f1(st, n, P, Dz->buf.p, w->buf.p, c->buf.p, t, v->buf.p);
+      launch_barrier_f2(st, n, P, Dz->buf.p, w->buf.p, Y->buf.p);
+    }
+    hip_check(hipGetLastError(), "barrier_f12 launch");
+    hip_check(hipStreamSynchronize(st), "sync barrier_f12");
+  });
+}
 int mgb_mul(mgb_vec x, mgb_vec y, mgb_vec out) {
   return guard([&] {
     need(x && y && out && x->n == y->n && x->n == out->n, "mul: shape mismatch");
diff --git a/multigridbarriermpi.jl_amd/csrc/devutil.hpp b/multigridbarriermpi.jl_amd/csrc/devutil.hpp
--- a/multigridbarriermpi.jl_amd/csrc/devutil.hpp
+++ b/multigridbarriermpi.jl_amd/csrc/devutil.hpp
@@ -9,7 +9,7 @@
 constexpr int kBlock = 256;
 constexpr int kMaxBlocks = 2048;
 
-inline int grid_for(long long work_items) {
+__host__ __device__ inline int grid_for(long long work_items) {
   long long b = (work_items + kBlock - 1) / kBlock;
   if (b < 1) b = 1;
   if (b > kMaxBlocks) b = kMaxBlocks;
@@ -63,9 +63,9 @@
 constexpr int kTicketDoubles = kReductionHeader;
 constexpr int kTicketStride = 32;
 static_assert(kReductionHeader * sizeof(double) >= 9 * kTicketStride * sizeof(unsigned), "ticket words");
-template <int NOUT>
-__device__ inline void grid_finish(const double (&r)[NOUT] , double* scratch, double* out_dev,
-                                   double* out_host, double* lds, HostSignal sig = HostSignal(), unsigned slot = 0xffffffffu) {
+template <int NOUT, class Store>
+__device__ inline void grid_finish_store(const double (&r)[NOUT] , double* scratch, HostSignal sig,
+                                         unsigned slot, Store&& store) {
   if (slot == 0xffffffffu) slot = blockIdx.x;
   __shared__ int is_last;
   unsigned* ticket = reinterpret_cast<unsigned*>(scratch);
@@ -105,20 +105,26 @@
   }
   double tot[NOUT];
   block_sum_n<NOUT>(acc, tot);
-  (void)lds;
-  if (threadIdx.x == 0) {
-#pragma unroll
-    for (int o = 0; o < NOUT; ++o) {
-      if (out_dev) out_dev[o] = tot[o];
-      if (out_host) __hip_atomic_store(&out_host[o], tot[o], __ATOMIC_RELAXED, __HIP_MEMORY_SCOPE_SYSTEM);
-    }
-  }
+  if (threadIdx.x == 0) store(tot);
   if (sig.seq_host && threadIdx.x == 0) {
     asm volatile("s_waitcnt vmcnt(0)" ::: "memory");
     const unsigned long long q = __hip_atomic_load(sig.seq_dev, __ATOMIC_RELAXED, __HIP_MEMORY_SCOPE_AGENT) + 1;
     __hip_atomic_store(sig.seq_dev, q, __ATOMIC_RELAXED, __HIP_MEMORY_SCOPE_AGENT);
     __hip_atomic_store(sig.seq_host, q, __ATOMIC_RELEASE, __HIP_MEMORY_SCOPE_SYSTEM);
   }
+}
+__device__ inline void store_result(double* out_dev, double* out_host, int o, double v) {
+  if (out_dev) out_dev[o] = v;
+  if (out_host) __hip_atomic_store(&out_host[o], v, __ATOMIC_RELAXED, __HIP_MEMORY_SCOPE_SYSTEM);
+}
+template <int NOUT>
+__device__ inline void grid_finish(const double (&r)[NOUT] , double* scratch, double* out_dev,
+                                   double* out_host, double* lds, HostSignal sig = HostSignal(), unsigned slot = 0xffffffffu) {
+  (void)lds;
+  grid_finish_store<NOUT>(r, scratch, sig, slot, [=](const double (&tot)[NOUT]) {
+#pragma unroll
+    for (int o = 0; o < NOUT; ++o) store_result(out_dev, out_host, o, tot[o]);
+  });
 }
 template <int NOUT, class Fn>
 __device__ inline void grid_finish_fn(const double (&r)[NOUT] , double* scratch, double* lds, Fn&& fn) {
diff --git a/multigridbarriermpi.jl_amd/csrc/kernels.hip b/multigridbarriermpi.jl_amd/csrc/kernels.hip
--- a/multigridbarriermpi.jl_amd/csrc/kernels.hip
+++ b/multigridbarriermpi.jl_amd/csrc/kernels.hip
@@ -1,5 +1,6 @@
 #include "kernels.hpp"
 #include "kernels_tpl.hpp"
+#include "errors.hpp"
 
 #include <algorithm>
 #include <cmath>
@@ -13,6 +14,71 @@
 void spmv_launch(hipStream_t st, const DevCsr& A, const double* x, const double* y0, double* y) {
   const int grid = grid_for((long long)A.rows * G);
   hipLaunchKernelGGL((spmv_kernel_t<G, double>), dim3(grid), dim3(kBlock), 0, st, A.rows, A.rowptr, A.colidx, A.vals, x, y0, y);
+}
+
+template <int G>
+__global__ __launch_bounds__(kBlock) void spmv_norm_kernel(int rows, const int* __restrict__ rowptr, const int* __restrict__ colidx,
+                                                            const double* __restrict__ vals, const double* __restrict__ x,
+                                                            const double* y0, double* y, double* scratch, double* out_dev,
+                                                            double* out_host, HostSignal sig) {
+  __shared__ double lds[kBlock / 64];
+  __shared__ double ys[kBlock];
+  constexpr int GR = kBlock / G;
+  const int lane = threadIdx.x % G, grp = threadIdx.x / G;
+  const unsigned blk = xcd_block(blockIdx.x, gridDim.x);
+  const long long r0 = (long long)blk * kBlock;
+  const int nrows = (int)min((long long)kBlock, (long long)rows - r0);
+  for (int rr0 = grp; rr0 < nrows; rr0 += kSpmvU * GR) {
+    int b[kSpmvU], e[kSpmvU];
+    double acc[kSpmvU], base[kSpmvU];
+#pragma unroll
+    for (int u = 0; u < kSpmvU; ++u) {
+      const int rr = rr0 + u * GR;
+      const bool ok = rr < nrows;
+      b[u] = ok ? rowptr[r0 + rr] : 0;
+      e[u] = ok ? rowptr[r0 + rr + 1] : 0;
+      base[u] = (ok && y0 && lane == 0) ? y0[r0 + rr] : 0.0;
+      acc[u] = 0.0;
+    }
+    int ci[kSpmvU];
+    double va[kSpmvU];
+#pragma unroll
+    for (int u = 0; u < kSpmvU; ++u) {
+      const int k = b[u] + lane;
+      const bool in = k < e[u];
+      ci[u] = in ? colidx[k] : -1;
+      va[u] = in ? vals[k] : 0.0;
+    }
+#pragma unroll
+    for (int u = 0; u < kSpmvU; ++u) acc[u] = (ci[u] >= 0) ? va[u] * x[ci[u]] : 0.0;
+#pragma unroll
+    for (int u = 0; u < kSpmvU; ++u)
+      for (int k = b[u] + lane + G; k < e[u]; k += G) acc[u] += vals[k] * x[colidx[k]];
+#pragma unroll
+    for (int u = 0; u < kSpmvU; ++u) {
+      double a = acc[u];
+#pragma unroll
+      for (int o = G / 2; o > 0; o >>= 1) a += __shfl_down(a, o, G);
+      const int rr = rr0 + u * GR;
+      if (lane == 0 && rr < nrows) {
+        const double v = base[u] + a;
+        y[r0 + rr] = v;
+        ys[rr] = v;
+      }
+    }
+  }
+  __syncthreads();
+  double acc2 = 0.0;
+  if ((int)threadIdx.x < nrows) acc2 += ys[threadIdx.x] * ys[threadIdx.x];
+  const double r[1] = {block_sum(acc2, lds)};
+  grid_finish<1>(r, scratch, out_dev, out_host, lds, sig, blk);
+}
+
+template <int G>
+void spmv_norm_launch(hipStream_t st, const DevCsr& A, const double* x, const double* y0, double* y, double* scratch, double* out,
+                      double* out_host, HostSignal sig) {
+  hipLaunchKernelGGL(spmv_norm_kernel<G>, dim3(grid_for(A.rows)), dim3(kBlock), 0, st, A.rows, A.rowptr, A.colidx, A.vals, x, y0, y,
+                     scratch, out, out_host, sig);
 }
 
 template <int G>
@@ -110,18 +176,33 @@
 
 
 constexpr int kTrialNodes = 64;
-template <int G, int NA>
+template <int G, int NA, bool DOT>
 __global__ __launch_bounds__(kBlock) void trial_f0_kernel(int n, int N, BarrierParams P, const int* __restrict__ rowptr,
                                                            const int* __restrict__ colidx, const double* __restrict__ vals,
                                                            const double* __restrict__ s, const double* __restrict__ nstep,
                                                            TrialSet T, const double* __restrict__ Dz0,
                                                            const double* __restrict__ w, const double* __restrict__ c,
                                                            const double* __restrict__ phi_ref, double frac, double* scratch,
-                                                           HostSignal sig) {
+                                                           HostSignal sig, TrialDot D) {
   __shared__ double lds[kBlock / 64];
   __shared__ double dzs[NA][kTrialNodes * kMaxK];
   constexpr int GR = kBlock / G;
   const int K = P.K, lane = threadIdx.x % G, grp = threadIdx.x / G;
+  double dot_part = 0.0;
+  if constexpr (DOT) {
+    if (D.flag_dev && blockIdx.x == 0 && threadIdx.x == 0) {
+      const int f = __hip_atomic_load(D.flag_dev, __ATOMIC_RELAXED, __HIP_MEMORY_SCOPE_AGENT);
+      __hip_atomic_store(D.flag_host, f, __ATOMIC_RELAXED, __HIP_MEMORY_SCOPE_SYSTEM);
+      __hip_atomic_store(D.flag_dev, 0, __ATOMIC_RELAXED, __HIP_MEMORY_SCOPE_AGENT);
+    }
+    const unsigned ds = xcd_block(blockIdx.x, gridDim.x);
+    const long long gd = grid_for(D.N);
+    if (ds < gd) {
+      double acc = 0.0;
+      for (long long i = (long long)ds * kBlock + threadIdx.x; i < D.N; i += gd * kBlock) acc += D.x[i] * D.y[i];
+      dot_part = block_sum(acc, lds);
+    }
+  }
 #pragma unroll
   for (int a = 0; a < NA; ++a)
     if (T.s_out[a])
@@ -212,7 +293,21 @@
     mine[2 * a + 1] = pa == a ? accL : 0.0;
   }
   block_sum_n<2 * NA>(mine, r);
-  grid_finish<2 * NA>(r, scratch, T.out_dev, T.out_host, lds, sig, xcd_block(blockIdx.x, gridDim.x));
+  if constexpr (DOT) {
+    double rd[2 * NA + 1];
+#pragma unroll
+    for (int o = 0; o < 2 * NA; ++o) rd[o] = r[o];
+    rd[2 * NA] = dot_part;
+    double* const out_dev = T.out_dev;
+    double* const out_host = T.out_host;
+    grid_finish_store<2 * NA + 1>(rd, scratch, sig, xcd_block(blockIdx.x, gridDim.x), [=](const double (&tot)[2 * NA + 1]) {
+#pragma unroll
+      for (int o = 0; o < 2 * NA; ++o) store_result(out_dev, out_host, o, tot[o]);
+      store_result(D.out_dev, D.out_host, 0, tot[2 * NA]);
+    });
+  } else {
+    grid_finish<2 * NA>(r, scratch, T.out_dev, T.out_host, lds, sig, xcd_block(blockIdx.x, gridDim.x));
+  }
 }
 
 inline int trial_grid(int n) {
@@ -223,10 +318,15 @@
 template <int G>
 void trial_launch(hipStream_t st, const DevCsr& B, int n, const BarrierParams& P, const double* s, const double* nstep,
                   const TrialSet& T, const double* Dz0, const double* w, const double* c, const double* phi_ref, double frac,
-                  double* scratch, HostSignal sig) {
+                  double* scratch, HostSignal sig, const TrialDot* dot) {
 #define MGB_TRIAL_NA(NA)                                                                                                    \
-  hipLaunchKernelGGL((trial_f0_kernel<G, NA>), dim3(trial_grid(n)), dim3(kBlock), 0, st, n, B.cols, P, B.rowptr, B.colidx,   \
-                     B.vals, s, nstep, T, Dz0, w, c, phi_ref, frac, scratch, sig)
+  hipLaunchKernelGGL((trial_f0_kernel<G, NA, false>), dim3(trial_grid(n)), dim3(kBlock), 0, st, n, B.cols, P, B.rowptr,     \
+                     B.colidx, B.vals, s, nstep, T, Dz0, w, c, phi_ref, frac, scratch, sig, TrialDot())
+  if (dot) {
+    hipLaunchKernelGGL((trial_f0_kernel<G, 3, true>), dim3(trial_grid(n)), dim3(kBlock), 0, st, n, B.cols, P, B.rowptr, B.colidx,
+                       B.vals, s, nstep, T, Dz0, w, c, phi_ref, frac, scratch, sig, *dot);
+    return;
+  }
   switch (T.na) {
     case 1: MGB_TRIAL_NA(1); break;
     case 2: MGB_TRIAL_NA(2); break;
@@ -391,10 +491,32 @@
 
 int f0_blocks(int n) { return std::max(grid_for(n), trial_grid(n)); }
 
+bool trial_dot_rides(int n, int N) { return N >= 1 && trial_grid(n) >= grid_for(N); }
+
+bool spmv_norm_fits(int rows) { return rows >= 1 && rows <= kBlock * kMaxBlocks; }
+
+void launch_spmv_norm(hipStream_t st, const DevCsr& A, const double* x, const double* y0, double* y, double* scratch, double* out,
+                      double* out_host, HostSignal sig) {
+  if (!spmv_norm_fits(A.rows)) throw InternalError("spmv_norm: more rows than one block per 256 can own");
+#define MGB_SPMV_NORM(G) spmv_norm_launch<G>(st, A, x, y0, y, scratch, out, out_host, sig)
+  switch (A.group) {
+    case 1: MGB_SPMV_NORM(1); break;
+    case 2: MGB_SPMV_NORM(2); break;
+    case 4: MGB_SPMV_NORM(4); break;
+    case 8: MGB_SPMV_NORM(8); break;
+    case 16: MGB_SPMV_NORM(16); break;
+    case 32: MGB_SPMV_NORM(32); break;
+    default: MGB_SPMV_NORM(64); break;
+  }
+#undef MGB_SPMV_NORM
+}
+
 void launch_trial_set(hipStream_t st, const DevCsr& B, int n, BarrierParams P, const double* s, const double* nstep,
                       const TrialSet& T, const double* Dz0, const double* w, const double* c, const double* phi_ref, double frac,
-                      double* scratch, HostSignal sig) {
-#define MGB_TRIAL(G) trial_launch<G>(st, B, n, P, s, nstep, T, Dz0, w, c, phi_ref, frac, scratch, sig)
+                      double* scratch, HostSignal sig, const TrialDot* dot) {
+  if (dot && !(T.na == 3 && trial_dot_rides(n, dot->N)))
+    throw InternalError("trial launch: the dot rides only with three points on a grid of at least grid_for(N) blocks");
+#define MGB_TRIAL(G) trial_launch<G>(st, B, n, P, s, nstep, T, Dz0, w, c, phi_ref, frac, scratch, sig, dot)
   switch (B.group) {
     case 1: MGB_TRIAL(1); break;
     case 2: MGB_TRIAL(2); break;
@@ -438,6 +560,11 @@
   hipLaunchKernelGGL(barrier_f2_kernel_t<double>, dim3(grid_for(n)), dim3(kBlock), 0, st, n, P, Dz, w, Y);
 }
 
+void launch_barrier_f12(hipStream_t st, int n, BarrierParams P, const double* Dz, const double* w, const double* c, double t,
+                        double* v, double* Y) {
+  hipLaunchKernelGGL(barrier_f12_kernel_t<double>, dim3(grid_for(n)), dim3(kBlock), 0, st, n, P, Dz, w, c, t, v, Y);
+}
+
 void launch_barrier_rows_F(hipStream_t st, int n, BarrierParams P, const double* Dz, double* out) {
   if (n == 0) return;
   hipLaunchKernelGGL(barrier_rows_F_kernel, dim3(grid_for(n)), dim3(kBlock), 0, st, n, P, Dz, out);
diff --git a/multigridbarriermpi.jl_amd/csrc/kernels.hpp b/multigridbarriermpi.jl_amd/csrc/kernels.hpp
--- a/multigridbarriermpi.jl_amd/csrc/kernels.hpp
+++ b/multigridbarriermpi.jl_amd/csrc/kernels.hpp
@@ -83,16 +83,31 @@
   double* out_dev = nullptr;
   double* out_host = nullptr;
 };
+struct TrialDot {
+  const double* x = nullptr;
+  const double* y = nullptr;
+  int N = 0;
+  int* flag_dev = nullptr;
+  int* flag_host = nullptr;
+  double* out_dev = nullptr;
+  double* out_host = nullptr;
+};
+bool trial_dot_rides(int n, int N);
 void launch_trial_set(hipStream_t st, const DevCsr& B, int n, BarrierParams P, const double* s, const double* nstep,
                       const TrialSet& T, const double* Dz0, const double* w, const double* c, const double* phi_ref, double frac,
-                      double* scratch, HostSignal sig = HostSignal());
+                      double* scratch, HostSignal sig = HostSignal(), const TrialDot* dot = nullptr);
 void launch_barrier_f1(hipStream_t st, int n, BarrierParams P, const double* Dz, const double* w, const double* c,
                        double t, double* v);
 void launch_barrier_f2(hipStream_t st, int n, BarrierParams P, const double* Dz, const double* w, double* Y);
+void launch_barrier_f12(hipStream_t st, int n, BarrierParams P, const double* Dz, const double* w, const double* c, double t,
+                        double* v, double* Y);
 void launch_barrier_rows_F(hipStream_t st, int n, BarrierParams P, const double* Dz, double* out);
 void launch_expand_hessian_rows(hipStream_t st, int n, BarrierParams P, const double* Y, double* out);
 void launch_dot(hipStream_t st, int n, const double* x, const double* y, double* scratch, double* out, double* out_host = nullptr,
                 int* flag_dev = nullptr, int* flag_host = nullptr, HostSignal sig = HostSignal());
+bool spmv_norm_fits(int rows);
+void launch_spmv_norm(hipStream_t st, const DevCsr& A, const double* x, const double* y0, double* y, double* scratch, double* out,
+                      double* out_host = nullptr, HostSignal sig = HostSignal());
 void launch_dot_owned(hipStream_t st, int n, const double* x, const double* y, const int* kind, int count_top, double* scratch,
                       double* out);
 void launch_gather_top(hipStream_t st, int ntop, const int* top, const double* g, double* buf);
diff --git a/multigridbarriermpi.jl_amd/csrc/kernels_tpl.hpp b/multigridbarriermpi.jl_amd/csrc/kernels_tpl.hpp
--- a/multigridbarriermpi.jl_amd/csrc/kernels_tpl.hpp
+++ b/multigridbarriermpi.jl_amd/csrc/kernels_tpl.hpp
@@ -133,100 +133,114 @@
 }
 
 template <class T>
+__device__ inline void barrier_f1_row(const BarrierParams& P, long long q, const T* dz, T wq, const T* cq, T t, T* vq) {
+  T vr[kMaxK];
+#pragma unroll
+  for (int j = 0; j < kMaxK; ++j) vr[j] = (j < P.K) ? wq * (t * cq[j]) : T(0);
+  for (int ci = 0; ci < P.ncones; ++ci) {
+    const ConeSpec& S = P.cone[ci];
+    if (!P.active(ci, q)) continue;
+    const ConeAM<T> am = cone_am<T>(P, ci, q);
+    const ConeT<T> k = load_cone<T>(S, dz, am.a);
+    if (S.kind == 1) {
+#pragma unroll
+      for (int j = 0; j < kMaxK; ++j) {
+        T add = T(0);
+#pragma unroll
+        for (int i = 0; i < 3; ++i) add += (i < S.nq && S.iq[i] == j) ? -wq * (T(S.coef[i]) / k.phi) : T(0);
+        vr[j] += add;
+      }
+      continue;
+    }
+    const T ds = am.a * pow_a<T>(k.s, am.a - T(1));
+    const T gs = wq * (-ds / k.phi - am.mu / k.s);
+#pragma unroll
+    for (int j = 0; j < kMaxK; ++j) {
+      T add = T(0);
+#pragma unroll
+      for (int i = 0; i < 3; ++i) add += (i < S.nq && S.iq[i] == j) ? wq * (T(2) * k.q[i] / k.phi) : T(0);
+      add += (S.is == j) ? gs : T(0);
+      add += (S.is2 == j) ? gs : T(0);
+      vr[j] += add;
+    }
+  }
+#pragma unroll
+  for (int j = 0; j < kMaxK; ++j)
+    if (j < P.K) vq[j] = vr[j];
+}
+
+template <class T>
+__device__ inline void barrier_f2_row(const BarrierParams& P, long long q, const T* dz, T wq, T* yq) {
+  int slot = 0;
+  for (int ci = 0; ci < P.ncones; ++ci) {
+    const ConeSpec& S = P.cone[ci];
+    if (!P.active(ci, q)) {
+      const int ns = S.nY();
+      for (int i = 0; i < ns; ++i) yq[slot++] = T(0);
+      continue;
+    }
+    const ConeAM<T> am = cone_am<T>(P, ci, q);
+    const ConeT<T> k = load_cone<T>(S, dz, am.a);
+    if (S.kind == 1) {
+      const T ip2l = T(1) / (k.phi * k.phi);
+#pragma unroll
+      for (int i = 0; i < 3; ++i)
+#pragma unroll
+        for (int j = 0; j < 3; ++j)
+          if (i < S.nq && j >= i && j < S.nq) yq[slot++] = wq * (T(S.coef[i]) * T(S.coef[j]) * ip2l);
+      continue;
+    }
+    const T a = am.a;
+    const T ds = a * pow_a<T>(k.s, a - T(1));
+    const T dds = (a == T(1)) ? T(0) : a * (a - T(1)) * pow_a<T>(k.s, a - T(2));
+    const T ip = T(1) / k.phi, ip2 = ip * ip;
+    const T hss = -dds * ip + ds * ds * ip2 + am.mu / (k.s * k.s);
+    const int nq = S.nq, nact = S.nact();
+#pragma unroll
+    for (int i = 0; i < 5; ++i)
+#pragma unroll
+      for (int j = 0; j < 5; ++j) {
+        if (i < nact && j >= i && j < nact) {
+          const int ai = min(i, nq), aj = min(j, nq);
+          T h;
+          if (aj < nq) h = T(4) * pick3<T>(k.q, ai) * pick3<T>(k.q, aj) * ip2 + (ai == aj ? T(2) * ip : T(0));
+          else if (ai < nq) h = T(-2) * pick3<T>(k.q, ai) * ds * ip2;
+          else h = hss;
+          yq[slot++] = wq * h;
+        }
+      }
+  }
+}
+
+template <class T>
 __global__ __launch_bounds__(kBlock) void barrier_f1_kernel_t(int n, BarrierParams P, const T* __restrict__ Dz,
                                                                const T* __restrict__ w, const T* __restrict__ c, T t,
                                                                T* __restrict__ v) {
-  for (long long q = (long long)blockIdx.x * kBlock + threadIdx.x; q < n; q += (long long)gridDim.x * kBlock) {
-    const T* dz = Dz + q * P.K;
-    const T* cq = c + q * P.K;
-    const T wq = w[q];
-    T vr[kMaxK];
-#pragma unroll
-    for (int j = 0; j < kMaxK; ++j) vr[j] = (j < P.K) ? wq * (t * cq[j]) : T(0);
-    for (int ci = 0; ci < P.ncones; ++ci) {
-      const ConeSpec& S = P.cone[ci];
-      if (!P.active(ci, q)) continue;
-      const ConeAM<T> am = cone_am<T>(P, ci, q);
-      const ConeT<T> k = load_cone<T>(S, dz, am.a);
-      if (S.kind == 1) {
-#pragma unroll
-        for (int j = 0; j < kMaxK; ++j) {
-          T add = T(0);
-#pragma unroll
-          for (int i = 0; i < 3; ++i) add += (i < S.nq && S.iq[i] == j) ? -wq * (T(S.coef[i]) / k.phi) : T(0);
-          vr[j] += add;
-        }
-        continue;
-      }
-      const T ds = am.a * pow_a<T>(k.s, am.a - T(1));
-      const T gs = wq * (-ds / k.phi - am.mu / k.s);
-#pragma unroll
-      for (int j = 0; j < kMaxK; ++j) {
-        T add = T(0);
-#pragma unroll
-        for (int i = 0; i < 3; ++i) add += (i < S.nq && S.iq[i] == j) ? wq * (T(2) * k.q[i] / k.phi) : T(0);
-        add += (S.is == j) ? gs : T(0);
-        add += (S.is2 == j) ? gs : T(0);
-        vr[j] += add;
-      }
-    }
-    T* vq = v + q * P.K;
-#pragma unroll
-    for (int j = 0; j < kMaxK; ++j)
-      if (j < P.K) vq[j] = vr[j];
-  }
+  for (long long q = (long long)blockIdx.x * kBlock + threadIdx.x; q < n; q += (long long)gridDim.x * kBlock)
+    barrier_f1_row<T>(P, q, Dz + q * P.K, w[q], c + q * P.K, t, v + q * P.K);
 }
 
 template <class T>
 __global__ __launch_bounds__(kBlock) void barrier_f2_kernel_t(int n, BarrierParams P, const T* __restrict__ Dz,
                                                                const T* __restrict__ w, T* __restrict__ Y) {
   const int nY = P.nY();
+  for (long long q = (long long)blockIdx.x * kBlock + threadIdx.x; q < n; q += (long long)gridDim.x * kBlock)
+    barrier_f2_row<T>(P, q, Dz + q * P.K, w[q], Y + q * nY);
+}
+
+template <class T>
+__global__ __launch_bounds__(kBlock) void barrier_f12_kernel_t(int n, BarrierParams P, const T* __restrict__ Dz,
+                                                                const T* __restrict__ w, const T* __restrict__ c, T t,
+                                                                T* __restrict__ v, T* __restrict__ Y) {
+  const int nY = P.nY();
   for (long long q = (long long)blockIdx.x * kBlock + threadIdx.x; q < n; q += (long long)gridDim.x * kBlock) {
     const T* dz = Dz + q * P.K;
-    T* yq = Y + q * nY;
     const T wq = w[q];
-    int slot = 0;
-    for (int ci = 0; ci < P.ncones; ++ci) {
-      const ConeSpec& S = P.cone[ci];
-      if (!P.active(ci, q)) {
-        const int ns = S.nY();
-        for (int i = 0; i < ns; ++i) yq[slot++] = T(0);
-        continue;
-      }
-      const ConeAM<T> am = cone_am<T>(P, ci, q);
-      const ConeT<T> k = load_cone<T>(S, dz, am.a);
-      if (S.kind == 1) {
-        const T ip2l = T(1) / (k.phi * k.phi);
-#pragma unroll
-        for (int i = 0; i < 3; ++i)
-#pragma unroll
-          for (int j = 0; j < 3; ++j)
-            if (i < S.nq && j >= i && j < S.nq) yq[slot++] = wq * (T(S.coef[i]) * T(S.coef[j]) * ip2l);
-        continue;
-      }
-      const T a = am.a;
-      const T ds = a * pow_a<T>(k.s, a - T(1));
-      const T dds = (a == T(1)) ? T(0) : a * (a - T(1)) * pow_a<T>(k.s, a - T(2));
-      const T ip = T(1) / k.phi, ip2 = ip * ip;
-      const T hss = -dds * ip + ds * ds * ip2 + am.mu / (k.s * k.s);
-      const int nq = S.nq, nact = S.nact();
-#pragma unroll
-      for (int i = 0; i < 5; ++i)
-#pragma unroll
-        for (int j = 0; j < 5; ++j) {
-          if (i < nact && j >= i && j < nact) {
-            const int ai = min(i, nq), aj = min(j, nq);
-            T h;
-            if (aj < nq) h = T(4) * pick3<T>(k.q, ai) * pick3<T>(k.q, aj) * ip2 + (ai == aj ? T(2) * ip : T(0));
-            else if (ai < nq) h = T(-2) * pick3<T>(k.q, ai) * ds * ip2;
-            else h = hss;
-            yq[slot++] = wq * h;
-          }
-        }
-    }
-  }
-}
-
-
-}
-}
+    barrier_f1_row<T>(P, q, dz, wq, c + q * P.K, t, v + q * P.K);
+    barrier_f2_row<T>(P, q, dz, wq, Y + q * nY);
+  }
+}
+
+
+}
+}
```
